# b-tudor/mpmcxx

Measured on AMD Instinct MI355X. Metric: energy-evals/sec (10k-atom LJ+Ewald+polar box); 1/2/4/8-GPU scaling, higher is better.
Workload: dtype f64

## Files before the change

mpmcxx_amd/csrc/context.h:

```cpp
#pragma once
#include <hip/hip_runtime.h>

#include <algorithm>
#include <atomic>
#include <chrono>
#include <mutex>
#include <cmath>
#include <cstdio>
#include <cstdlib>
#include <cstring>
#include <string>
#include <thread>
#include <vector>

#include "../../include/mpmc_energy.h"
#include "kernels.h"

using namespace mpmc;

namespace mpmc {
extern thread_local std::string g_create_error;
}

struct EvPair {
	hipEvent_t a, b;
	int cls;
};

#if defined(__SANITIZE_THREAD__)
extern "C" void AnnotateHappensBefore(const char *file, int line, const volatile void *tag);
extern "C" void AnnotateHappensAfter(const char *file, int line, const volatile void *tag);
inline char g_pinned_pool_tag;
#endif
template <class T>
inline hipError_t pinned_alloc(T **p, size_t bytes) {
	hipError_t e = hipHostMalloc((void **)p, bytes);
#if defined(__SANITIZE_THREAD__)
	AnnotateHappensAfter(__FILE__, __LINE__, &g_pinned_pool_tag);
#endif
	return e;
}
inline hipError_t pinned_free(void *p) {
#if defined(__SANITIZE_THREAD__)
	AnnotateHappensBefore(__FILE__, __LINE__, &g_pinned_pool_tag);
#endif
	return hipHostFree(p);
}

struct mpmc_ctx;
template <class T, bool kPinned = false>
struct DevBuf {
	T *p = nullptr;
	size_t cap = 0;
	DevBuf() = default;
	DevBuf(DevBuf &&o) noexcept : p(o.p), cap(o.cap) { o.p = nullptr, o.cap = 0; }
	DevBuf &operator=(DevBuf &&o) noexcept {
		std::swap(p, o.p), std::swap(cap, o.cap);
		return *this;
	}
	~DevBuf() { release(nullptr); }
	operator T *() const { return p; }
	void release(mpmc_ctx *c);
	int reserve(mpmc_ctx *c, size_t need, size_t grow_to = 0);
};
template <class T>
using PinnedBuf = DevBuf<T, true>;

struct mpmc_tuning {
	int stream_mode = -1;
	int pair_kernel = 0;
	int pair_waves = 0;
	int sort_grid = -1;
	int sort_nx = 0, sort_ny = 0;
	bool side_after_sweep = true;
	bool lazy_side_stream = true;
	bool poll_retire = true;
	bool poll_long = true;
	bool dense_symmetric = true;
	bool fast_geometry = true;
	int pair_split = -1;
	int pair_split_tail = -1;
	int sweep_order = 1;
	int sweep_lds_pad = 2048;
	bool use_panels = true;
	bool no_uniform = false;
	bool no_classes = false;
	bool single_launch = true;
	bool no_recip_tab = false;
	bool no_sort = false;
	bool no_order_carry = false;
	bool no_polar_delta = false;
	bool no_inline_move = false;
	int virtual_device = -1;
	int fail_next_wait = 0;
	bool trace_panel = false;
	bool dipoles_on_demand = true;
	long long tensor_budget_mb = 4096;
	long long direct_budget_mb = -1;
};

struct mpmc_kept {
	mpmc_tuning tune;
	bool prof = false;
	mpmc_timings tim{};
	long long n_poll_hits = 0, n_poll_timeouts = 0, n_stream_syncs = 0, n_poll_yields = 0;
	long long n_uploads_carried = 0, n_uploads_sorted = 0;
	bool tb_enabled = false, tb_mk = false;
	bool de_enabled = false;
	int de_flags = 0;
	bool pw_enabled = false;
	double pw_alpha = 0.0;
	bool palmo_enabled = false;
	bool on_demand = false;
};

struct mpmc_ctx {
	mpmc_kept kept;
	int device = 0;
	hipStream_t stream = nullptr;
	hipStream_t stream2 = nullptr;
	hipEvent_t ev_fork = nullptr, ev_join = nullptr;
	bool two_streams = true;
	int max_atoms = 0, max_pad = 0;
	int n = 0, n_pad = 0, n_tiles = 0, n_tile_pairs = 0, n_split = 1;
	int n_molecules = 0;
	double N_movable = 0;
	std::string err;

	std::vector<double> h_pos, h_q, h_alpha, h_eps, h_sigma, h_mass;
	std::vector<int32_t> h_mol, h_frozen, h_disp;

	std::vector<int32_t> perm, slot_of;
	int32_t *d_slot_of = nullptr, *d_perm = nullptr;
	bool atoms_dirty = true;

	DevBuf<char> d_atoms_blob;
	double4 *d_xyzq = nullptr;
	double2 *d_lj = nullptr;
	int2 *d_mf = nullptr;
	double *d_alpha = nullptr, *d_eps = nullptr, *d_inv_molmass = nullptr;

	DevBuf<int2> d_tile_pairs;
	DevBuf<double> d_block_part;
	DevBuf<int> d_block_cnt;
	DevBuf<int> d_cls;
	DevBuf<double> d_tile_bounds;
	DevBuf<double4> d_tp_shift;
	DevBuf<int4> d_panels;
	DevBuf<int> d_seg;
	DevBuf<double> d_gpart;
	DevBuf<long long> d_trace;
	int n_panel_entries = 0, seg_tiles = -1;
	bool panels_built = false;
	DevBuf<double2> d_erf_tab;
	DevBuf<int2> d_sweep_blocks;
	int n_sweep_blocks = 0, sweep_tiles = -1;
	DevBuf<int> d_generic_list;
	int n_generic = 0;
	std::vector<int> h_generic;
	int inflight_hint = 1;
	bool last_pair_was_sweep = false;
	FusedParams last_fp{};
	bool last_fp_valid = false;
	int debug_panel_replicas = 1;
	PinnedBuf<double4> h_xyzq;
	hipEvent_t ev_xyzq = nullptr;
	bool xyzq_in_flight = false;
	std::vector<double> h_pos_sorted;
	bool order_sorted = false;
	bool order_carried = false;
	bool atoms_dirty_order = false;
	int edits_since_sort = 0;
	double sort_origin_f[3] = {0, 0, 0};
	hipStream_t sync_stream = nullptr;
	std::vector<double> molmass_tmp;
	PinnedBuf<long long> static_cnt;
	PinnedBuf<char> h_kstage;
	hipEvent_t ev_kstage = nullptr;
	bool kstage_in_flight = false;
	int lvec_kmax = -1;
	PinnedBuf<char> h_stage;
	hipEvent_t ev_stage = nullptr;
	bool stage_in_flight = false;
	unsigned static_gen = 1, static_ride_gen = 0;

	bool static_dirty = true;
	double h_static[3] = {0, 0, 0};
	DevBuf<int> d_counter;
	bool scal_clean = false;
	int poll_budget_us = 1000;
	bool spin_on_post = false;
	bool last_was_single = false;
	double single_seq = 0;
	DevBuf<double> d_atom_part;
	DevBuf<double> d_scal;
	long long *d_cnt = nullptr;
	PinnedBuf<double> h_scal;
	long long *h_cnt = nullptr;
	DevBuf<int> d_flag;
	PinnedBuf<int> h_flag;

	int K = 0;
	DevBuf<double4> d_kvec, d_kw;
	DevBuf<double4> d_sf;
	DevBuf<int4> d_lvec;
	DevBuf<double4> d_sf_part;
	DevBuf<double> d_w_en;

	DevBuf<double> d_e_recip_part, d_part, d_e_static, d_mu[2], d_e_induced, d_rrms;
	DevBuf<double2> d_gs_blocks;
	DevBuf<double> d_gs_ul;
	int mu_cur = 0;
	DevBuf<double> d_dk_ring;
	enum { PEND_NONE = 0, PEND_OPEN = 1, PEND_DROPPED = 2 };
	int polar_pending = PEND_NONE;
	int pend_done = 0, pend_target = 0;
	DevBuf<double> d_arows;
	DevBuf<double> d_adense;
	DevBuf<double2> d_ab;
	int solver_used = MPMC_SOLVER_MATRIX_FREE;
	DevBuf<double> d_chol, d_chol_v, d_chol_info;
	PinnedBuf<double> h_chol_info;
	DevBuf<int> d_chol_list, d_chol_status;
	bool direct_ran = false;
	mpmc_direct_info direct{};

	Box box{};
	double box_in[20] = {0};
	bool box_in_has_recip = false;
	bool box_set = false, atoms_set = false, opts_set = false, k_dirty = true;
	mpmc_options opts{};
	double ewald_alpha = 0, polar_ewald_alpha = 0;

	bool pending = false;
	bool have_polar = false;
	int iters = 0, failed = 0;
	unsigned run_mask = 0;

	bool cache_valid = false;
	mpmc_result last_full{};
	mpmc_result trial_res{};
	int trial_last_kind = -1;
	bool trial_open = false, trial_evaluated = false, trial_was_full = false, trial_enqueued = false, trial_noop = false;
	mpmc_result trial_keep{};
	int trial_first = 0, trial_count = 0;
	std::vector<double> trial_new, trial_old;
	int *d_mv_slot = nullptr, *d_mv_orig = nullptr;
	double4 *d_mv_new = nullptr;
	DevBuf<int> d_moved_idx;
	DevBuf<double4> d_sf_trial;
	DevBuf<double> d_e_real, d_e_real_trial, d_dk_part;
	bool e_real_valid = false;
	bool trial_polar_delta = false;
	std::vector<int> store_dirty_tiles, trial_tiles;
	int touch_n = -1, touch[8] = {0};
	DevBuf<unsigned char> d_mv_blob;
	PinnedBuf<unsigned char> h_mv_blob;
	DevBuf<double> d_delta_out;
	PinnedBuf<double> h_delta_out;
	MvInline mv_inline{};
	bool trial_inline = false;
	double trial_seq = 0;
	long long *d_delta_cnt = nullptr, *h_delta_cnt = nullptr;

	bool tb_have = false;
	bool tb_dirty = false;
	std::vector<double> h_tb_au;
	DevBuf<double2> d_tb_au;
	DevBuf<double> d_tb_part;

	bool de_have = false;
	bool de_dirty = false;
	std::vector<double> h_de;
	std::vector<double> h_de_raw;
	bool de_lrc_valid = false;
	double de_lrc[2] = {0, 0}, de_lrc_volume = 0, de_lrc_cutoff = 0;
	int de_lrc_rd_lrc = 0;
	DevBuf<double4> d_de_co;
	DevBuf<double> d_de_t10;
	DevBuf<double> d_de_part;

	bool palmo_ran = false;
	double palmo_correction = 0.0;
	DevBuf<double> d_palmo_f, d_palmo_change;

	std::vector<EvPair> ev_free, ev_used;

	int64_t bytes_total = 0;
};

#define HIP_TRY(ctx, call)                                                                                        \
	do {                                                                                                          \
		hipError_t _e = (call);                                                                                   \
		if (_e != hipSuccess) {                                                                                   \
			(ctx)->err = std::string(#call) + ": " + hipGetErrorString(_e);                                       \
			return MPMC_ERR_HIP;                                                                                  \
		}                                                                                                         \
	} while (0)

template <class T, bool kPinned>
inline void DevBuf<T, kPinned>::release(mpmc_ctx *c) {
	if (p) (void)(kPinned ? pinned_free(p) : hipFree(p));
	if (p && c && !kPinned) c->bytes_total -= (int64_t)(cap * sizeof(T));
	p = nullptr, cap = 0;
}
template <class T, bool kPinned>
inline int DevBuf<T, kPinned>::reserve(mpmc_ctx *c, size_t need, size_t grow_to) {
	if (need <= cap) return MPMC_OK;
	release(c);
	const size_t count = std::max(need, grow_to), bytes = std::max<size_t>(count, 1) * sizeof(T);
	hipError_t e = kPinned ? pinned_alloc(&p, bytes) : hipMalloc((void **)&p, bytes);
	if (e != hipSuccess) p = nullptr;
	if (e == hipSuccess && !kPinned && (e = hipMemsetAsync(p, 0, bytes, c->stream)) == hipSuccess) e = hipStreamSynchronize(c->stream);
	if (e != hipSuccess) {
		release(nullptr);
		c->err = std::string(kPinned ? "pinned host" : "device") + " allocation of " + std::to_string(bytes) + " bytes: " + hipGetErrorString(e);
		return MPMC_ERR_HIP;
	}
	cap = count;
	if (!kPinned) c->bytes_total += (int64_t)(count * sizeof(T));
	return MPMC_OK;
}

namespace mpmc {

constexpr size_t kAtomRecordBytes = sizeof(double4) + sizeof(double2) + sizeof(int2) + 3 * sizeof(double) + 2 * sizeof(int32_t);
template <typename F>
inline void atom_block_layout(char *base, size_t P, F &&set) {
	double4 *xyzq = reinterpret_cast<double4 *>(base);
	double2 *lj = reinterpret_cast<double2 *>(xyzq + P);
	int2 *mf = reinterpret_cast<int2 *>(lj + P);
	double *al = reinterpret_cast<double *>(mf + P), *ep = al + P, *imm = ep + P;
	int32_t *perm = reinterpret_cast<int32_t *>(imm + P), *slot = perm + P;
	set(xyzq, lj, mf, al, ep, imm, perm, slot);
}
inline int mirror_guard(mpmc_ctx *c) {
	if (c->xyzq_in_flight) {
		HIP_TRY(c, hipEventSynchronize(c->ev_xyzq));
		c->xyzq_in_flight = false;
	}
	return MPMC_OK;
}

inline int fail(mpmc_ctx *c, int code, const std::string &msg) {
	if (c) c->err = msg;
	else g_create_error = msg;
	return code;
}

template <class Pred>
inline bool poll_posted(mpmc_ctx *c, Pred seen, std::chrono::microseconds budget) {
	const auto t0 = std::chrono::steady_clock::now();
	for (int spins = 0;; ++spins) {
		if (seen()) {
			std::atomic_thread_fence(std::memory_order_acquire);
			c->kept.n_poll_hits++;
			return true;
		}
		if ((spins & 255) == 255) {
			const auto dt = std::chrono::steady_clock::now() - t0;
			if (dt > budget) {
				c->kept.n_poll_timeouts++;
				return false;
			}
			if (dt > std::chrono::microseconds(50)) {
				c->kept.n_poll_yields++;
				std::this_thread::yield();
			}
		}
	}
}

inline void prof_begin(mpmc_ctx *c, int cls, int &cur, hipStream_t st) {
	cur = -1;
	if (!c->kept.prof) return;
	EvPair e;
	if (!c->ev_free.empty()) {
		e = c->ev_free.back();
		c->ev_free.pop_back();
	} else {
		if (hipEventCreate(&e.a) != hipSuccess || hipEventCreate(&e.b) != hipSuccess) return;
	}
	e.cls = cls;
	(void)hipEventRecord(e.a, st);
	c->ev_used.push_back(e);
	cur = (int)c->ev_used.size() - 1;
}
inline void prof_end(mpmc_ctx *c, int cur, hipStream_t st) {
	if (cur >= 0 && cur < (int)c->ev_used.size()) (void)hipEventRecord(c->ev_used[cur].b, st);
}
inline void prof_harvest(mpmc_ctx *c) {
	for (auto &e : c->ev_used) {
		float ms = 0;
		if (hipEventElapsedTime(&ms, e.a, e.b) == hipSuccess) {
			c->kept.tim.ms[e.cls] += ms;
			c->kept.tim.launches[e.cls] += 1;
		}
		c->ev_free.push_back(e);
	}
	c->ev_used.clear();
}
struct ProfScope {
	mpmc_ctx *c;
	int cur;
	hipStream_t st;
	ProfScope(mpmc_ctx *c_, int cls, hipStream_t st_ = nullptr) : c(c_), st(st_ ? st_ : c_->stream) { prof_begin(c, cls, cur, st); }
	~ProfScope() { prof_end(c, cur, st); }
};
inline hipStream_t fork_side(mpmc_ctx *c) {
	if (!c->two_streams) return c->stream;
	if (!c->stream2 && hipStreamCreateWithFlags(&c->stream2, hipStreamNonBlocking) != hipSuccess) {
		c->stream2 = nullptr;
		c->two_streams = false;
		return c->stream;
	}
	(void)hipEventRecord(c->ev_fork, c->stream);
	(void)hipStreamWaitEvent(c->stream2, c->ev_fork, 0);
	return c->stream2;
}
inline void join_side(mpmc_ctx *c) {
	if (!c->two_streams || !c->stream2) return;
	(void)hipEventRecord(c->ev_join, c->stream2);
	(void)hipStreamWaitEvent(c->stream, c->ev_join, 0);
}


enum : unsigned {
	RUN_PAIR = 1, RUN_PAIR_ES = 2, RUN_RECIP = 4, RUN_ATOMTERMS = 8, RUN_FIELD = 16, RUN_SOLVE = 32, RUN_WOLF = 64,
	RUN_STORE = 128,
	RUN_THREE_BODY = 256,
	RUN_DISP = 512
};
constexpr double kThreeBodyScale = 3.0 * (0.0032539449 / (3.166811429 * 0.000001));
int three_body_ready(mpmc_ctx *c);
int disp_ready(mpmc_ctx *c);
DispParams disp_params(const mpmc_ctx *c);
int prepare(mpmc_ctx *c, bool defer_static = false);
int enqueue(mpmc_ctx *c, unsigned mask, bool on_demand = false);
int wait_and_fill(mpmc_ctx *c, mpmc_result *out);
unsigned full_mask(const mpmc_ctx *c);
inline bool polar_moments_apply(const mpmc_ctx *c) {
	const mpmc_options &o = c->opts;
	return o.polarization && !o.rd_only && o.polar_iterative && o.polar_max_iter >= 1 && o.polar_max_iter <= kMomentsMaxIter && o.polar_gamma == 1.0 && o.polar_precision == 0.0 && !o.polar_rrms &&
	       !o.polar_gs;
}
inline int moments_half(int n) { return (n + 1) / 2; }
inline int reserve_dk_ring(mpmc_ctx *c) { return c->d_dk_ring.reserve(c, (size_t)(moments_half(c->opts.polar_max_iter) + 1) * 3 * (size_t)c->max_pad); }
int finish_pending_dipoles(mpmc_ctx *c);
inline void drop_pending_dipoles(mpmc_ctx *c) {
	if (c->polar_pending == mpmc_ctx::PEND_OPEN) c->polar_pending = mpmc_ctx::PEND_DROPPED;
}
inline bool direct_solve(const mpmc_ctx *c) { return c->opts.polarization && !c->opts.rd_only && !c->opts.polar_iterative; }
inline bool wolf_field_on(const mpmc_ctx *c) { return c->kept.pw_enabled && c->opts.polarization && !c->opts.rd_only && !c->opts.polar_ewald; }
void ext_params(const mpmc_ctx *c, FusedParams &fp, bool wolf_on);
AtomsDev atoms_view(const mpmc_ctx *c);
RecipDev recip_view(const mpmc_ctx *c);
int upload_atoms(mpmc_ctx *c);

}
```

mpmcxx_amd/csrc/evaluate.cpp:

```cpp
#include "context.h"


using namespace mpmc;

static int build_k_tables(mpmc_ctx *c) {
	const int kmax = c->opts.ewald_kmax;
	const double alpha = c->ewald_alpha, ea = c->polar_ewald_alpha;
	auto each_lvec = [kmax](auto &&visit) {
		int l[3];
		for (l[0] = 0; l[0] <= kmax; l[0]++)
			for (l[1] = (!l[0] ? 0 : -kmax); l[1] <= kmax; l[1]++)
				for (l[2] = ((!l[0] && !l[1]) ? 1 : -kmax); l[2] <= kmax; l[2]++)
					if (l[0] * l[0] + l[1] * l[1] + l[2] * l[2] <= kmax * kmax) visit(l);
	};
	int K = 0, rc;
	each_lvec([&K](const int *) { K++; });
	if ((size_t)K > c->d_lvec.cap) c->lvec_kmax = -1;
	if ((rc = c->d_kvec.reserve(c, (size_t)K)) != MPMC_OK) return rc;
	if ((rc = c->d_kw.reserve(c, (size_t)K)) != MPMC_OK) return rc;
	if ((rc = c->d_lvec.reserve(c, (size_t)K)) != MPMC_OK) return rc;
	if ((rc = c->d_w_en.reserve(c, (size_t)K)) != MPMC_OK) return rc;
	if ((rc = c->d_sf.reserve(c, (size_t)K)) != MPMC_OK) return rc;
	if (K > 0) {
		if (c->kstage_in_flight) {
			HIP_TRY(c, hipEventSynchronize(c->ev_kstage));
			c->kstage_in_flight = false;
		}
		if ((rc = c->h_kstage.reserve(c, (size_t)K * (2 * sizeof(double4) + sizeof(double) + sizeof(int4)))) != MPMC_OK) return rc;
		if (!c->ev_kstage) HIP_TRY(c, hipEventCreateWithFlags(&c->ev_kstage, hipEventDisableTiming));
		double4 *kvec = reinterpret_cast<double4 *>(c->h_kstage.p), *kw = kvec + K;
		int4 *lvec = reinterpret_cast<int4 *>(kw + K);
		double *wen = reinterpret_cast<double *>(lvec + K);
		int n = 0;
		each_lvec([&](const int *l) {
			double k[3];
			for (int p = 0; p < 3; p++) {
				k[p] = 0;
				for (int q = 0; q < 3; q++) k[p] += 2.0 * kPi * c->box.r[3 * p + q] * l[q];
			}
			const double k2 = k[0] * k[0] + k[1] * k[1] + k[2] * k[2];
			kvec[n] = make_double4(k[0], k[1], k[2], k2);
			lvec[n] = make_int4(l[0], l[1], l[2], 0);
			wen[n] = std::exp(-k2 / (4.0 * alpha * alpha)) / k2;
			const double g = std::exp(-k2 / (4.0 * ea * ea));
			kw[n] = make_double4(k[0] / k2 * g, k[1] / k2 * g, k[2] / k2 * g, 0.0);
			n++;
		});
		HIP_TRY(c, hipMemcpyAsync(c->d_kvec, kvec, K * sizeof(double4), hipMemcpyHostToDevice, c->stream));
		HIP_TRY(c, hipMemcpyAsync(c->d_kw, kw, K * sizeof(double4), hipMemcpyHostToDevice, c->stream));
		HIP_TRY(c, hipMemcpyAsync(c->d_w_en, wen, K * sizeof(double), hipMemcpyHostToDevice, c->stream));
		if (c->lvec_kmax != kmax) {
			HIP_TRY(c, hipMemcpyAsync(c->d_lvec, lvec, K * sizeof(int4), hipMemcpyHostToDevice, c->stream));
			c->lvec_kmax = kmax;
		}
		HIP_TRY(c, hipEventRecord(c->ev_kstage, c->stream));
		c->kstage_in_flight = true;
	}
	c->K = K;
	return MPMC_OK;
}

constexpr int kDenseChunks = 16;
constexpr int kOneStreamMinInflight = 4;
constexpr int kCheckEvery = 4;
constexpr int kSingleLaunchTiles = 32;

static int ensure_polar_buffers(mpmc_ctx *c) {
	const size_t np = (size_t)c->max_pad;
	int rc;
	if ((rc = c->d_e_static.reserve(c, 3 * np)) != MPMC_OK) return rc;
	if ((rc = c->d_mu[0].reserve(c, 3 * np)) != MPMC_OK) return rc;
	if ((rc = c->d_mu[1].reserve(c, 3 * np)) != MPMC_OK) return rc;
	if ((rc = c->d_e_induced.reserve(c, 3 * np)) != MPMC_OK) return rc;
	if ((rc = c->d_rrms.reserve(c, np)) != MPMC_OK) return rc;
	if ((rc = c->d_e_recip_part.reserve(c, recip_slices_capacity(np))) != MPMC_OK) return rc;
	if ((rc = c->d_e_real.reserve(c, 3 * np)) != MPMC_OK) return rc;
	if ((rc = c->d_e_real_trial.reserve(c, 3 * np)) != MPMC_OK) return rc;
	if ((rc = c->d_gs_ul.reserve(c, 6 * np)) != MPMC_OK) return rc;
	if ((rc = c->d_palmo_f.reserve(c, 3 * np)) != MPMC_OK) return rc;
	if ((rc = c->d_palmo_change.reserve(c, 3 * np)) != MPMC_OK) return rc;
	if (polar_moments_apply(c) && (rc = reserve_dk_ring(c)) != MPMC_OK) return rc;
	const size_t need = (size_t)std::max(c->n_tiles, kDenseChunks) * c->n_pad * 3;
	return c->d_part.reserve(c, need);
}

static int resolve_solver(mpmc_ctx *c) {
	const size_t need = (size_t)c->n_tile_pairs * (kTile * kTile);
	int want = c->opts.solver;
	if (direct_solve(c)) {
		c->solver_used = MPMC_SOLVER_MATRIX_FREE;
		return MPMC_OK;
	}
	if (c->opts.polar_gs) want = MPMC_SOLVER_MATRIX_FREE;
	if (want == MPMC_SOLVER_AUTO) {
		const size_t budget_mb = (size_t)c->kept.tune.tensor_budget_mb;
		want = (need * sizeof(double2) <= budget_mb * (size_t)1048576) ? MPMC_SOLVER_COMPACT : MPMC_SOLVER_MATRIX_FREE;
		if (c->opts.polar_precision == 0.0 && c->opts.polar_max_iter <= 3) want = MPMC_SOLVER_MATRIX_FREE;
	}
	if (want == MPMC_SOLVER_DENSE) {
		const int rc = c->d_adense.reserve(c, (size_t)3 * c->n_pad * (size_t)3 * c->n_pad);
		if (rc != MPMC_OK) return rc;
	}
	if (want == MPMC_SOLVER_COMPACT) {
		const int rc = c->d_ab.reserve(c, need);
		if (rc != MPMC_OK) {
			if (c->opts.solver == MPMC_SOLVER_COMPACT) return rc;
			(void)hipGetLastError();
			want = MPMC_SOLVER_MATRIX_FREE;
		}
	}
	c->solver_used = want;
	return MPMC_OK;
}

int mpmc::prepare(mpmc_ctx *c, bool defer_static) {
	if (!c->box_set) return fail(c, MPMC_ERR_BOX, "energy: no box set (mpmc_set_box)");
	if (!c->atoms_set) return fail(c, MPMC_ERR_INVALID_DATUM, "energy: no atoms set (mpmc_set_atoms)");
	HIP_TRY(c, hipSetDevice(c->device));
	if (c->opts.feynman_hibbs && c->h_mass.empty())
		return fail(c, MPMC_ERR_INVALID_DATUM, "energy: feynman_hibbs needs atom masses (mpmc_set_atoms was called without them)");
	if (c->atoms_dirty) {
		int rc = upload_atoms(c);
		if (rc != MPMC_OK) return rc;
	}
	if (c->k_dirty) {
		c->ewald_alpha = (c->opts.ewald_alpha > 0) ? c->opts.ewald_alpha : 3.5 / c->box.cutoff;
		c->polar_ewald_alpha = (c->opts.polar_ewald_alpha > 0) ? c->opts.polar_ewald_alpha : 3.5 / c->box.cutoff;
		int rc = build_k_tables(c);
		if (rc != MPMC_OK) return rc;
		c->k_dirty = false;
	}
	if (c->static_dirty && !defer_static) {
		c->scal_clean = false;
		launch_atom_terms(c->stream, atoms_view(c), c->box, c->ewald_alpha, c->opts.rd_lrc,  1, c->d_atom_part, c->d_scal);
		HIP_TRY(c, hipGetLastError());
		double tmp[S_COUNT];
		HIP_TRY(c, hipMemcpyAsync(tmp, c->d_scal, sizeof(tmp), hipMemcpyDeviceToHost, c->stream));
		HIP_TRY(c, hipStreamSynchronize(c->stream));
		c->h_static[0] = tmp[S_LRC_PAIR];
		c->h_static[1] = tmp[S_LRC_SELF];
		c->h_static[2] = tmp[S_ES_SELF];
		c->static_dirty = false;
	}
	return MPMC_OK;
}

AtomsDev mpmc::atoms_view(const mpmc_ctx *c) {
	AtomsDev a;
	a.xyzq = c->d_xyzq;
	a.lj = c->d_lj;
	a.mf = c->d_mf;
	a.alpha = c->d_alpha;
	a.eps = c->d_eps;
	a.inv_molmass = c->d_inv_molmass;
	a.n = c->n;
	a.n_pad = c->n_pad;
	return a;
}
RecipDev mpmc::recip_view(const mpmc_ctx *c) {
	RecipDev r;
	r.kvec = c->d_kvec;
	r.w_en = c->d_w_en;
	r.kw = c->d_kw;
	r.lvec = c->kept.tune.no_recip_tab ? nullptr : c->d_lvec;
	r.sf = c->d_sf;
	r.K = c->K;
	return r;
}

static inline const double4 *shift_view(const mpmc_ctx *c) { return (c->kept.tune.no_uniform || c->kept.tune.no_classes) ? nullptr : c->d_tp_shift.p; }

void mpmc::ext_params(const mpmc_ctx *c, FusedParams &fp, bool wolf_on) {
	const mpmc_options &o = c->opts;
	fp.wolf = wolf_on ? 1 : 0;
	fp.fh_order = o.feynman_hibbs ? ((o.feynman_hibbs_order == 4) ? 4 : 2) : 0;
	fp.fh_c2 = fp.fh_c4 = 0.0;
	if (fp.fh_order) {
		const double hBar2 = 1.11211999e-68, hBar4 = 1.23681087e-136, kB = 1.3806503e-23, kB2 = 1.90619525e-46, amu = 1.66053873e-27;
		fp.fh_c2 = 1.0e20 * (hBar2 / (24.0 * kB * o.temperature)) / amu;
		fp.fh_c4 = 1.0e40 * (hBar4 / (1152.0 * kB2 * o.temperature * o.temperature)) / (amu * amu);
	}
	fp.wolf_erfa_over_r = std::erf(c->ewald_alpha * c->box.cutoff) / c->box.cutoff;
	fp.wolf_inv_r2 = 1.0 / (c->box.cutoff * c->box.cutoff);
}

static inline int sweep_split_mode(const mpmc_ctx *c) { return c->kept.tune.pair_split < 0 ? 2 : (c->kept.tune.pair_split != 0 ? 1 : 0); }
static inline int sweep_split_tail(const mpmc_ctx *c) {
	const int permille = c->kept.tune.pair_split_tail >= 0 ? c->kept.tune.pair_split_tail : kSweepSplitTailPermille;
	return (int)((long long)c->n_sweep_blocks * permille / 1000);
}

static int enqueue_direct_solve(mpmc_ctx *c, const AtomsDev &at) {
	hipStream_t st = c->stream;
	int n_pol = 0;
	for (int i = 0; i < c->n; i++) n_pol += (c->h_alpha[i] != 0.0) ? 1 : 0;
	const int np = chol_padded(n_pol);
	const size_t elems = (size_t)np * (size_t)np, bytes = elems * sizeof(double);
	int rc;
	if ((rc = c->d_chol_status.reserve(c, 4)) != MPMC_OK) return rc;
	if ((rc = c->d_chol_info.reserve(c, 4)) != MPMC_OK) return rc;
	if ((rc = c->h_chol_info.reserve(c, 4)) != MPMC_OK) return rc;
	{
		size_t free_b = 0, total_b = 0;
		HIP_TRY(c, hipMemGetInfo(&free_b, &total_b));
		size_t avail = free_b + c->d_chol.cap * sizeof(double);
		if (c->kept.tune.direct_budget_mb >= 0) avail = std::min(avail, (size_t)c->kept.tune.direct_budget_mb * (size_t)1048576);
		if (bytes > avail) {
			char buf[256];
			std::snprintf(buf, sizeof buf, "direct dipole solve: the factor of %d unknowns needs %.1f MB (%d x %d doubles), %.1f MB are available", 3 * n_pol,
			              (double)bytes / 1048576.0, np, np, (double)avail / 1048576.0);
			return fail(c, MPMC_ERR_MEMORY, buf);
		}
	}
	if (c->d_chol.reserve(c, elems) != MPMC_OK) {
		(void)hipGetLastError();
		return fail(c, MPMC_ERR_MEMORY, "direct dipole solve: cannot allocate the factor (" + std::to_string(bytes) + " bytes): " + c->err);
	}
	if ((rc = c->d_chol_v.reserve(c, (size_t)2 * np, (size_t)2 * np + 1)) != MPMC_OK) return rc;
	if ((rc = c->d_chol_list.reserve(c, (size_t)n_pol, (size_t)c->max_pad)) != MPMC_OK) return rc;
	c->mu_cur = 0;
	double *mu = c->d_mu[0], *v0 = c->d_chol_v, *v1 = c->d_chol_v + np;
	HIP_TRY(c, hipMemsetAsync(c->d_chol_status, 0, sizeof(int), st));
	HIP_TRY(c, hipMemsetAsync(mu, 0, 3 * (size_t)at.n_pad * sizeof(double), st));
	if (n_pol > 0) {
		{
			ProfScope p(c, MPMC_K_TENSOR);
			launch_chol_build(st, at, c->box, c->opts.polar_damp, c->d_chol_list, n_pol, np, c->d_chol);
		}
		{
			ProfScope p(c, MPMC_K_DIPOLE_ITER);
			launch_chol_rhs(st, c->d_chol_list, n_pol, np, c->d_e_static, v0, c->d_chol_status);
			launch_chol_factor(st, c->d_chol, np, c->d_chol_status);
			launch_chol_solve(st, c->d_chol, np, v0, v1, c->d_chol_status);
			launch_chol_scatter(st, c->d_chol_list, n_pol, v0, mu, c->d_chol_status);
		}
	}
	{
		ProfScope p(c, MPMC_K_REDUCE);
		launch_dipole_iter_hybrid(st, at, c->box, mu, c->d_tile_pairs, c->d_cls, shift_view(c),
		                          c->n_tile_pairs, nullptr, c->d_part, c->opts.polar_damp, nullptr);
		launch_dipole_update(st, at, c->d_e_static, c->d_part, c->n_tiles, mu, c->d_mu[1], c->d_e_induced, 0, c->d_rrms, 0.0, nullptr, nullptr, 1);
		launch_chol_finish(st, at, mu, c->d_e_static, c->d_e_induced, c->d_chol_status, c->d_chol_info);
	}
	HIP_TRY(c, hipGetLastError());
	HIP_TRY(c, hipMemcpyAsync(c->h_chol_info, c->d_chol_info, 3 * sizeof(double), hipMemcpyDeviceToHost, st));
	c->direct.n_unknowns = 3 * (int64_t)n_pol;
	c->direct.factor_bytes = (int64_t)(c->d_chol.cap * sizeof(double));
	c->direct_ran = true;
	return MPMC_OK;
}


struct JacobiPlan {
	bool dense, dense_sym, compact;
	int iter_slots;
};
static JacobiPlan jacobi_plan(const mpmc_ctx *c) {
	JacobiPlan jp;
	jp.dense = (c->solver_used == MPMC_SOLVER_DENSE) && !c->opts.polar_gs;
	jp.dense_sym = jp.dense && c->kept.tune.dense_symmetric;
	jp.compact = c->solver_used == MPMC_SOLVER_COMPACT;
	jp.iter_slots = (jp.dense && !jp.dense_sym) ? kDenseChunks : c->n_tiles;
	return jp;
}
static void enqueue_jacobi_iteration(mpmc_ctx *c, const AtomsDev &at, const JacobiPlan &jp, int it, int want_rrms, double allowed, int *ctl, int *host_flag,
                                     double *dk) {
	hipStream_t st = c->stream;
	const mpmc_options &o = c->opts;
	const int *converged = ctl ? ctl + 1 : nullptr;
	if (jp.dense) {
		ProfScope p(c, MPMC_K_DIPOLE_ITER);
		if (jp.dense_sym) launch_dense_symv(st, c->d_adense, c->n_pad, c->d_mu[c->mu_cur], c->d_tile_pairs, c->n_tile_pairs, c->d_part);
		else launch_dense_matvec(st, c->d_adense, c->n_pad, c->d_mu[c->mu_cur], kDenseChunks, c->d_part);
	} else if (jp.compact) {
		ProfScope p(c, MPMC_K_DIPOLE_ITER);
		if (c->panels_built)
			launch_dipole_iter_panel(st, at, c->box, c->d_mu[c->mu_cur], c->d_tile_pairs, c->d_tp_shift, c->d_panels,
			                         c->n_panel_entries, c->d_ab, c->d_part, c->d_gpart, converged, c->d_trace);
		else
			launch_dipole_iter_hybrid(st, at, c->box, c->d_mu[c->mu_cur], c->d_tile_pairs, c->d_cls,
			                          shift_view(c), c->n_tile_pairs, c->d_ab, c->d_part, o.polar_damp,
			                          converged);
	} else {
		ProfScope p(c, MPMC_K_DIPOLE_ITER);
		launch_dipole_iter_hybrid(st, at, c->box, c->d_mu[c->mu_cur], c->d_tile_pairs, c->d_cls,
		                          shift_view(c), c->n_tile_pairs, nullptr, c->d_part, o.polar_damp,
		                          converged);
	}
	{
		ProfScope p(c, MPMC_K_REDUCE);
		if (jp.compact && c->panels_built && !jp.dense)
			launch_dipole_update_panel(st, at, c->d_e_static, c->d_part, c->d_gpart, c->d_seg, c->d_mu[c->mu_cur], c->d_mu[1 - c->mu_cur],
			                           c->d_e_induced, want_rrms, c->d_rrms, allowed, ctl, host_flag, it, dk);
		else
			launch_dipole_update(st, at, c->d_e_static, c->d_part, jp.iter_slots, c->d_mu[c->mu_cur], c->d_mu[1 - c->mu_cur], c->d_e_induced,
			                     want_rrms, c->d_rrms, allowed, ctl, host_flag, it, dk);
	}
	c->mu_cur = 1 - c->mu_cur;
}

int mpmc::finish_pending_dipoles(mpmc_ctx *c) {
	if (c->polar_pending == mpmc_ctx::PEND_NONE) return MPMC_OK;
	if (c->polar_pending == mpmc_ctx::PEND_DROPPED)
		return fail(c, MPMC_ERR_ARG, "the dipoles of the last evaluation were left to be computed on demand, and its positions, cell, options or buffers "
		                             "have been overwritten since: evaluate again (or mpmc_set_dipoles_on_demand(ctx, 0))");
	HIP_TRY(c, hipSetDevice(c->device));
	const AtomsDev at = atoms_view(c);
	const JacobiPlan jp = jacobi_plan(c);
	for (int it = c->pend_done + 1; it <= c->pend_target; it++) enqueue_jacobi_iteration(c, at, jp, it, 0, 0.0, nullptr, nullptr, nullptr);
	HIP_TRY(c, hipGetLastError());
	HIP_TRY(c, hipStreamSynchronize(c->stream));
	c->polar_pending = mpmc_ctx::PEND_NONE;
	c->pend_done = c->pend_target;
	if (!c->pending) prof_harvest(c);
	return MPMC_OK;
}

int mpmc::enqueue(mpmc_ctx *c, unsigned mask, bool on_demand) {
	if (c->pending) return fail(c, MPMC_ERR_ARG, "an evaluation of this context is still in flight (mpmc_energy_wait first)");
	drop_pending_dipoles(c);
	int rc = prepare(c, true);
	if (rc != MPMC_OK) return rc;
	if ((mask & RUN_THREE_BODY) && (rc = three_body_ready(c)) != MPMC_OK) return rc;
	if ((mask & RUN_DISP) && (rc = disp_ready(c)) != MPMC_OK) return rc;
	const bool static_ride = c->static_dirty;
	c->static_ride_gen = 0;
	const AtomsDev at = atoms_view(c);
	const RecipDev rcp = recip_view(c);
	const mpmc_options &o = c->opts;
	hipStream_t st = c->stream;
	c->run_mask = mask;
	c->have_polar = false;
	c->direct_ran = false;
	c->palmo_ran = false;
	c->iters = 0;
	c->failed = 0;

	c->last_was_single = false;
	c->spin_on_post = false;
	if (c->kept.tune.single_launch && mask == (RUN_PAIR | RUN_ATOMTERMS) && !o.feynman_hibbs && c->n_tiles <= kSingleLaunchTiles && !c->kept.prof && !static_ride) {
		FusedParams fp{};
		fp.rd_lrc = o.rd_lrc;
		c->single_seq += 1.0;
		launch_pair_lj_single(st, at, c->box, fp, c->d_tile_pairs, c->n_tile_pairs, c->d_block_part, c->d_block_cnt, c->d_counter, c->h_scal,
		                      c->single_seq);
		HIP_TRY(c, hipGetLastError());
		c->last_was_single = true;
		c->pending = true;
		return MPMC_OK;
	}
	if (!c->scal_clean) HIP_TRY(c, hipMemsetAsync(c->d_scal, 0, (S_COUNT + C_COUNT) * sizeof(double), st));
	c->scal_clean = false;
	if (static_ride) {
		launch_atom_terms(st, at, c->box, c->ewald_alpha, o.rd_lrc,  1, c->d_atom_part, c->d_scal);
		HIP_TRY(c, hipGetLastError());
		c->static_ride_gen = c->static_gen;
	}

	if (mask & (RUN_FIELD | RUN_SOLVE | RUN_STORE)) {
		if ((rc = ensure_polar_buffers(c)) != MPMC_OK) return rc;
		if ((rc = resolve_solver(c)) != MPMC_OK) return rc;
	}
	const bool compact = (mask & RUN_SOLVE) && c->solver_used == MPMC_SOLVER_COMPACT;

	const bool need_sf = (mask & RUN_RECIP) || ((mask & RUN_FIELD) && o.polar_ewald);
	const bool need_intra = (mask & RUN_PAIR) && (mask & RUN_PAIR_ES) && !(o.wolf && (mask & RUN_WOLF)) && (c->n_molecules != c->n);
	const bool side_work = need_sf || need_intra;
	c->two_streams = (c->kept.tune.stream_mode == 1) ||
	                 (c->kept.tune.stream_mode < 0 && c->n_tile_pairs > kOneStreamMaxPairs &&
	                  !((mask & RUN_SOLVE) && c->inflight_hint >= kOneStreamMinInflight));
	const bool side_fork = c->two_streams && (need_sf || need_intra);
	bool panel_side = false;
	int side_rc = MPMC_OK;
	auto enqueue_side_work = [&](hipStream_t s2) {
		if (need_intra) {
			ProfScope p(c, MPMC_K_PAIR, s2);
			launch_intra_terms(s2, at, c->d_slot_of, c->ewald_alpha, c->d_scal);
		}
		{
			ProfScope p(c, MPMC_K_RECIP, s2);
			if (need_sf) {
				const size_t need_part = (size_t)c->n_tiles * (size_t)c->K;
				if (rcp.lvec && o.ewald_kmax <= kRecipTabMaxK && (side_rc = c->d_sf_part.reserve(c, need_part)) != MPMC_OK) return;
				launch_recip_sf(s2, at, c->box, rcp, o.ewald_kmax, c->d_sf_part);
			}
			if (mask & RUN_RECIP) launch_recip_energy(s2, rcp, c->box, c->d_scal);
		}
		if ((mask & RUN_FIELD) && o.polar_ewald) {
			ProfScope p(c, MPMC_K_FIELD, s2);
			launch_field_recip(s2, at, c->box, rcp, o.ewald_kmax, c->d_e_recip_part);
		}
	};
	const bool side_deferred = side_work && side_fork && (mask & (RUN_PAIR | RUN_FIELD | RUN_STORE)) != 0 && c->kept.tune.side_after_sweep;
	if (side_work && !side_deferred) {
		enqueue_side_work(side_fork ? fork_side(c) : st);
		if (side_rc != MPMC_OK) return side_rc;
	}

	if (mask & (RUN_PAIR | RUN_FIELD | RUN_STORE)) {
		{
			ProfScope pc(c, MPMC_K_CLASSES);
			if (c->kept.tune.no_classes) HIP_TRY(c, hipMemsetAsync(c->d_cls, 0, (size_t)c->n_tile_pairs * sizeof(int), st));
			else launch_tile_classes(st, at, c->box, c->d_tile_pairs, c->n_tile_pairs, (o.polarization && !o.rd_only) ? o.polar_damp : 0.0,
			                         c->d_tile_bounds, c->d_cls, c->kept.tune.no_uniform ? nullptr : c->d_tp_shift, c->sort_origin_f, kTholeFarX);
		}
		FusedParams fp;
		fp.ewald_alpha = c->ewald_alpha;
		fp.polar_ewald_alpha = c->polar_ewald_alpha;
		fp.polar_damp = o.polar_damp;
		fp.rd_lrc = o.rd_lrc;
		fp.do_es = ((mask & RUN_PAIR_ES) || (mask & RUN_FIELD)) ? 1 : 0;
		fp.do_field = ((mask & RUN_FIELD) && !wolf_field_on(c)) ? (o.polar_ewald ? 1 : 2) : 0;
		fp.do_thole = compact ? 1 : 0;
		ext_params(c, fp, (o.wolf && (mask & RUN_WOLF)) != 0);
		fp.thole_far_x = kTholeFarX;
		fp.pair_waves = c->kept.tune.pair_waves ? c->kept.tune.pair_waves : (c->n_tile_pairs <= kPairSplitMax ? 4 : 1);
		fp.store_only = ((mask & RUN_STORE) && !(mask & (RUN_PAIR | RUN_FIELD))) ? 1 : 0;
		fp.touch_n = fp.store_only ? c->touch_n : -1;
		for (int k = 0; k < 8; k++) fp.touch[k] = c->touch[k];
		if (!fp.store_only && compact) c->store_dirty_tiles.clear();
		c->panels_built = false;
		if (compact && c->kept.tune.use_panels && !c->kept.tune.no_classes && !c->kept.tune.no_uniform && c->n_tiles >= 3) {
			if (c->seg_tiles != c->n_tiles) {
				std::vector<int> seg((size_t)c->n_tiles + 1, 0);
				for (int J = 0; J < c->n_tiles; J++) seg[J + 1] = seg[J] + panel_segment_entries(J);
				if ((rc = c->d_seg.reserve(c, seg.size())) != MPMC_OK) return rc;
				HIP_TRY(c, hipMemcpyAsync(c->d_seg, seg.data(), seg.size() * sizeof(int), hipMemcpyHostToDevice, st));
				HIP_TRY(c, hipStreamSynchronize(st));
				c->n_panel_entries = seg[c->n_tiles];
				c->seg_tiles = c->n_tiles;
			}
			const size_t need = (size_t)c->n_panel_entries;
			if ((rc = c->d_panels.reserve(c, need)) != MPMC_OK) return rc;
			if ((rc = c->d_gpart.reserve(c, need * kTile * 3)) != MPMC_OK) return rc;
			if (c->kept.tune.trace_panel && (rc = c->d_trace.reserve(c, need * 4)) != MPMC_OK) return rc;
			panel_side = c->two_streams;
			if (!panel_side) {
				ProfScope pc(c, MPMC_K_CLASSES, st);
				launch_build_panels(st, c->d_cls, c->n_tiles, c->d_seg, c->d_panels);
			}
			c->panels_built = true;
		}
		hipStream_t s_side = (side_deferred || panel_side) ? fork_side(c) : st;
		c->last_fp = fp;
		c->last_fp_valid = !fp.store_only;
		ProfScope p(c, MPMC_K_PAIR);
		const bool sweep = c->kept.tune.pair_kernel != 1 && c->d_sweep_blocks && (c->kept.tune.pair_kernel == 2 || c->n_tile_pairs > kSweepMinPairs) &&
		                   pair_sweep_covers(c->box, fp, c->ewald_alpha);
		c->last_pair_was_sweep = sweep;
		if (sweep) {
			launch_pair_sweep(st, at, c->box, fp, c->n_molecules != c->n, c->d_sweep_blocks, c->n_sweep_blocks, c->d_cls,
			                  shift_view(c), c->d_erf_tab, c->d_block_part, c->d_block_cnt, c->d_part,
			                  compact ? c->d_ab : nullptr, sweep_split_mode(c), sweep_split_tail(c), c->kept.tune.fast_geometry,
			                  (side_deferred || panel_side) ? c->kept.tune.sweep_lds_pad : 0);
			if (c->n_generic > 0)
				launch_pair_fused(st, at, c->box, fp, c->d_tile_pairs, c->d_cls, c->n_generic, c->d_block_part, c->d_block_cnt, c->d_part,
				                  compact ? c->d_ab : nullptr, c->d_generic_list);
		} else if (!(fp.store_only && !compact))
			launch_pair_fused(st, at, c->box, fp, c->d_tile_pairs, c->d_cls, c->n_tile_pairs, c->d_block_part, c->d_block_cnt, c->d_part,
			                  compact ? c->d_ab : nullptr);
		if (side_deferred) {
			enqueue_side_work(s_side);
			if (side_rc != MPMC_OK) return side_rc;
		}
		if (panel_side) {
			ProfScope pc(c, MPMC_K_CLASSES, s_side);
			launch_build_panels(s_side, c->d_cls, c->n_tiles, c->d_seg, c->d_panels);
		}
	}
	if ((side_work && side_fork) || panel_side) join_side(c);
	const bool reduce_in_tail = (mask & RUN_PAIR) && (mask & RUN_SOLVE);
	if ((mask & RUN_PAIR) && !reduce_in_tail) {
		ProfScope p(c, MPMC_K_REDUCE);
		launch_reduce_pairs(st, c->d_block_part, c->d_block_cnt, c->n_tile_pairs, c->d_scal, c->d_cnt);
	}

	if (mask & RUN_FIELD) {
		ProfScope p(c, MPMC_K_FIELD);
		c->mu_cur = 0;
		if (wolf_field_on(c))
			launch_wolf_field(st, at, c->box, wolf_field_params(c->kept.pw_alpha, c->box.cutoff), c->d_tile_pairs, c->d_cls, c->n_tile_pairs, c->d_part);
		launch_field_finalize(st, at, c->box, o.polar_ewald, c->d_e_recip_part, c->d_part, c->n_tiles, o.polar_gamma, c->d_e_static,
		                      c->d_mu[0], c->d_e_real, polar_moments_apply(c) ? c->d_dk_ring.p : nullptr);
		c->e_real_valid = (mask == full_mask(c));
	}

	if ((mask & RUN_SOLVE) && direct_solve(c)) {
		if ((rc = enqueue_direct_solve(c, at)) != MPMC_OK) return rc;
		{
			ProfScope p(c, MPMC_K_REDUCE);
			if (reduce_in_tail)
				launch_polar_energy_and_pairs(st, at, c->d_mu[c->mu_cur], c->d_e_static, nullptr, c->d_block_part, c->d_block_cnt, c->n_tile_pairs, c->d_scal,
				                              c->d_cnt);
			else launch_polar_energy(st, at, c->d_mu[c->mu_cur], c->d_e_static, nullptr, c->d_scal);
		}
		c->have_polar = true;
		c->polar_pending = mpmc_ctx::PEND_NONE;
	} else if (mask & RUN_SOLVE) {
		const bool by_precision = (o.polar_precision != 0.0);
		const int want_rrms = (o.polar_rrms || o.polar_precision > 0) ? 1 : 0;
		const double allowed = by_precision ? o.polar_precision * o.polar_precision * kDebye2SKA * kDebye2SKA : 0.0;
		const JacobiPlan jp = jacobi_plan(c);
		const bool dense = jp.dense, dense_sym = jp.dense_sym;
		const bool moments = polar_moments_apply(c);
		const int half = moments_half(o.polar_max_iter);
		const bool lazy = moments && on_demand && c->kept.tune.dipoles_on_demand && half < o.polar_max_iter;
		const int last_it = lazy ? half : o.polar_max_iter;
		const size_t dk_stride = 3 * (size_t)at.n_pad;
		if (dense) {
			ProfScope p(c, MPMC_K_TENSOR);
			launch_dense_build(st, at, c->box, o.polar_damp, c->d_adense, dense_sym);
		}
		int *ctl = (by_precision && !o.polar_gs) ? c->d_flag + 1 : nullptr;
		const int check_every = dense ? 1 : kCheckEvery;
		const int mu_start = c->mu_cur;
		int done_at = 0;
		int *host_flag = ctl ? c->h_flag + 2 : nullptr;
		if (ctl) {
			HIP_TRY(c, hipMemsetAsync(ctl, 0, 3 * sizeof(int), st));
			c->h_flag[2] = c->h_flag[3] = 0;
		}
		if (o.polar_gs) {
			if ((rc = c->d_gs_blocks.reserve(c, gs_block_store_elements(c->n_tiles))) != MPMC_OK) return rc;
			ProfScope p(c, MPMC_K_TENSOR);
			launch_gs_blocks(st, at, c->box, o.polar_damp, c->d_gs_blocks);
		}
		int it = 0;
		bool keep = true;
		while (keep) {
			it++;
			if (it >= kMaxIterationCount && by_precision) {
				launch_dipole_reset(st, at, c->d_e_static, c->d_mu[c->mu_cur]);
				c->failed = 1;
				break;
			}
			if (by_precision && o.polar_gs) HIP_TRY(c, hipMemsetAsync(c->d_flag, 0, sizeof(int), st));
			if (o.polar_gs) {
				double *mu = c->d_mu[c->mu_cur], *mu_old = c->d_mu[1 - c->mu_cur];
				if (want_rrms) HIP_TRY(c, hipMemcpyAsync(mu_old, mu, 3 * (size_t)at.n_pad * sizeof(double), hipMemcpyDeviceToDevice, st));
				{
					ProfScope p(c, MPMC_K_DIPOLE_ITER);
					launch_gs_sweep(st, at, c->box, o.polar_damp, c->d_e_static, mu, c->d_e_induced, c->d_part, c->d_tile_pairs, c->d_cls,
					                shift_view(c), c->n_tile_pairs, c->d_gs_ul, c->d_gs_ul + 3 * (size_t)c->max_pad, c->d_gs_blocks);
				}
				if (want_rrms) {
					ProfScope p(c, MPMC_K_REDUCE);
					launch_gs_finish(st, at, mu_old, mu, want_rrms, c->d_rrms, allowed, c->d_flag);
				}
				if (by_precision) {
					HIP_TRY(c, hipMemcpyAsync(c->h_flag, c->d_flag, sizeof(int), hipMemcpyDeviceToHost, st));
					HIP_TRY(c, hipStreamSynchronize(st));
					keep = (*c->h_flag != 0);
				} else {
					keep = (it != o.polar_max_iter);
				}
				continue;
			}
			enqueue_jacobi_iteration(c, at, jp, it, want_rrms, allowed, ctl, host_flag, (moments && it <= half) ? c->d_dk_ring + (size_t)it * dk_stride : nullptr);
			if (by_precision) {
				if (it % check_every == 0 || it + 1 >= kMaxIterationCount) {
					HIP_TRY(c, hipGetLastError());
					volatile const int *hf = host_flag;
					const bool seen = poll_posted(c, [&] { return hf[0] >= it || hf[1] != 0; }, std::chrono::microseconds(50000));
					if (seen) {
						done_at = hf[1];
					} else {
						c->kept.n_stream_syncs++;
						HIP_TRY(c, hipMemcpyAsync(c->h_flag, ctl + 1, sizeof(int), hipMemcpyDeviceToHost, st));
						HIP_TRY(c, hipStreamSynchronize(st));
						done_at = *c->h_flag;
					}
					keep = (done_at == 0);
				}
			} else {
				keep = (it != last_it);
			}
		}
		if (done_at > 0) {
			it = done_at;
			c->mu_cur = (mu_start + done_at) & 1;
		}
		c->iters = lazy ? o.polar_max_iter : it;
		c->polar_pending = lazy ? mpmc_ctx::PEND_OPEN : mpmc_ctx::PEND_NONE;
		c->pend_done = it, c->pend_target = o.polar_max_iter;
		if (moments) {
			ProfScope p(c, MPMC_K_REDUCE);
			if (reduce_in_tail)
				launch_polar_moments_and_pairs(st, at, c->d_dk_ring, c->d_e_static, o.polar_max_iter, c->d_block_part, c->d_block_cnt, c->n_tile_pairs, c->d_scal,
				                               c->d_cnt);
			else launch_polar_moments(st, at, c->d_dk_ring, c->d_e_static, o.polar_max_iter, c->d_scal);
		} else {
			ProfScope p(c, MPMC_K_REDUCE);
			if (reduce_in_tail)
				launch_polar_energy_and_pairs(st, at, c->d_mu[c->mu_cur], c->d_e_static, want_rrms ? c->d_rrms : nullptr, c->d_block_part, c->d_block_cnt,
				                              c->n_tile_pairs, c->d_scal, c->d_cnt);
			else launch_polar_energy(st, at, c->d_mu[c->mu_cur], c->d_e_static, want_rrms ? c->d_rrms : nullptr, c->d_scal);
		}
		if (c->kept.palmo_enabled && o.polar_gs && !c->failed) {
			double *mu = c->d_mu[c->mu_cur];
			{
				ProfScope p(c, MPMC_K_DIPOLE_ITER);
				launch_dipole_iter_hybrid(st, at, c->box, mu, c->d_tile_pairs, c->d_cls, shift_view(c),
				                          c->n_tile_pairs, nullptr, c->d_part, o.polar_damp, nullptr);
			}
			ProfScope p(c, MPMC_K_REDUCE);
			launch_dipole_update(st, at, c->d_e_static, c->d_part, c->n_tiles, mu, c->d_mu[1 - c->mu_cur], c->d_palmo_f, 0, c->d_rrms, 0.0, nullptr, nullptr, 1);
			launch_palmo_reduce(st, at, mu, c->d_palmo_f, c->d_e_induced, c->d_palmo_change, c->d_scal);
			c->palmo_ran = true;
		}
		c->have_polar = true;
	}
	if (mask & RUN_THREE_BODY) {
		ProfScope p(c, MPMC_K_THREE_BODY);
		launch_three_body(st, at, c->d_tb_au, c->box, kThreeBodyScale, c->d_tb_part, c->d_scal + S_THREE_BODY);
	}
	if (mask & RUN_DISP) {
		ProfScope p(c, MPMC_K_PAIR);
		launch_disp_expansion(st, at, c->d_de_co, c->d_de_t10, c->d_tile_pairs, c->n_tile_pairs, c->box, disp_params(c), c->de_lrc[0], c->de_lrc[1],
		                      c->d_de_part, c->d_scal + S_DISP);
	}
	HIP_TRY(c, hipGetLastError());
	c->single_seq += 1.0;
	launch_post_results(st, c->d_scal, c->h_scal, c->single_seq);
	HIP_TRY(c, hipGetLastError());
	c->scal_clean = true;
	c->spin_on_post = c->ev_used.empty() && (c->kept.tune.poll_long || c->n_tile_pairs <= kOneStreamMaxPairs);
	c->poll_budget_us = (c->n_tile_pairs <= kOneStreamMaxPairs) ? 1000 : 4000;
	c->pending = true;
	return MPMC_OK;
}


extern "C" int mpmc_debug_time_panel(mpmc_ctx *c, int reps, double *ms_per_launch) {
	if (!c || !ms_per_launch || reps <= 0) return MPMC_ERR_ARG;
	if (c->pending) return fail(c, MPMC_ERR_ARG, "mpmc_debug_time_panel: an evaluation is in flight");
	if (!c->have_polar || !c->panels_built || c->solver_used != MPMC_SOLVER_COMPACT)
		return fail(c, MPMC_ERR_ARG, "mpmc_debug_time_panel: the last evaluation did not run the panel kernel");
	HIP_TRY(c, hipSetDevice(c->device));
	{
		const int rc_f = finish_pending_dipoles(c);
		if (rc_f != MPMC_OK) return rc_f;
	}
	const AtomsDev at = atoms_view(c);
	hipEvent_t e0, e1;
	HIP_TRY(c, hipEventCreate(&e0));
	HIP_TRY(c, hipEventCreate(&e1));
	for (int r = 0; r < 3; r++)
		launch_dipole_iter_panel(c->stream, at, c->box, c->d_mu[c->mu_cur], c->d_tile_pairs, c->d_tp_shift, c->d_panels, c->n_panel_entries,
		                         c->d_ab, c->d_part, c->d_gpart);
	HIP_TRY(c, hipEventRecord(e0, c->stream));
	const int replicas = c->debug_panel_replicas;
	for (int r = 0; r < reps; r++)
		launch_dipole_iter_panel(c->stream, at, c->box, c->d_mu[c->mu_cur], c->d_tile_pairs, c->d_tp_shift, c->d_panels, c->n_panel_entries,
		                         c->d_ab, c->d_part, c->d_gpart, nullptr, nullptr, replicas);
	HIP_TRY(c, hipEventRecord(e1, c->stream));
	HIP_TRY(c, hipGetLastError());
	HIP_TRY(c, hipEventSynchronize(e1));
	float ms = 0;
	HIP_TRY(c, hipEventElapsedTime(&ms, e0, e1));
	(void)hipEventDestroy(e0);
	(void)hipEventDestroy(e1);
	*ms_per_launch = (double)ms / reps;
	return MPMC_OK;
}

extern "C" int mpmc_debug_time_pair(mpmc_ctx *c, int reps, double *ms_per_launch) {
	if (!c || !ms_per_launch || reps <= 0) return MPMC_ERR_ARG;
	if (c->pending) return fail(c, MPMC_ERR_ARG, "mpmc_debug_time_pair: an evaluation is in flight");
	if (!c->cache_valid || !c->last_fp_valid) return fail(c, MPMC_ERR_ARG, "mpmc_debug_time_pair: no complete evaluation has run");
	HIP_TRY(c, hipSetDevice(c->device));
	{
		const int rc_f = finish_pending_dipoles(c);
		if (rc_f != MPMC_OK) return rc_f;
	}
	const AtomsDev at = atoms_view(c);
	const FusedParams &fp = c->last_fp;
	const bool compact = c->solver_used == MPMC_SOLVER_COMPACT && fp.do_thole;
	bool timed = false;
	auto launch = [&] {
		if (c->last_pair_was_sweep) {
			launch_pair_sweep(c->stream, at, c->box, fp, c->n_molecules != c->n, c->d_sweep_blocks, c->n_sweep_blocks, c->d_cls,
			                  shift_view(c), c->d_erf_tab, c->d_block_part, c->d_block_cnt, c->d_part,
			                  compact ? c->d_ab : nullptr, sweep_split_mode(c), sweep_split_tail(c), c->kept.tune.fast_geometry,
			                  c->two_streams ? c->kept.tune.sweep_lds_pad : 0, timed ? c->debug_panel_replicas : 1);
			if (c->n_generic > 0)
				launch_pair_fused(c->stream, at, c->box, fp, c->d_tile_pairs, c->d_cls, c->n_generic, c->d_block_part, c->d_block_cnt, c->d_part,
				                  compact ? c->d_ab : nullptr, c->d_generic_list);
		} else {
			launch_pair_fused(c->stream, at, c->box, fp, c->d_tile_pairs, c->d_cls, c->n_tile_pairs, c->d_block_part, c->d_block_cnt, c->d_part,
			                  compact ? c->d_ab : nullptr);
		}
	};
	hipEvent_t e0, e1;
	HIP_TRY(c, hipEventCreate(&e0));
	HIP_TRY(c, hipEventCreate(&e1));
	for (int r = 0; r < 2; r++) launch();
	timed = true;
	HIP_TRY(c, hipEventRecord(e0, c->stream));
	for (int r = 0; r < reps; r++) launch();
	HIP_TRY(c, hipEventRecord(e1, c->stream));
	HIP_TRY(c, hipGetLastError());
	HIP_TRY(c, hipEventSynchronize(e1));
	float ms = 0;
	HIP_TRY(c, hipEventElapsedTime(&ms, e0, e1));
	(void)hipEventDestroy(e0);
	(void)hipEventDestroy(e1);
	*ms_per_launch = (double)ms / reps;
	return MPMC_OK;
}

int mpmc::wait_and_fill(mpmc_ctx *c, mpmc_result *out) {
	if (!c->pending) return fail(c, MPMC_ERR_ARG, "mpmc_energy_wait: nothing enqueued");
	auto abandon = [c](hipError_t e, const char *what) {
		(void)hipStreamSynchronize(c->stream);
		if (c->two_streams && c->stream2) (void)hipStreamSynchronize(c->stream2);
		c->sync_stream = nullptr;
		c->pending = false;
		c->scal_clean = false;
		c->static_ride_gen = 0;
		drop_pending_dipoles(c);
		return fail(c, MPMC_ERR_HIP, std::string(what) + ": " + hipGetErrorString(e));
	};
	hipError_t werr = c->kept.tune.fail_next_wait ? hipErrorUnknown : hipSetDevice(c->device);
	c->kept.tune.fail_next_wait = 0;
	if (werr != hipSuccess) return abandon(werr, "mpmc_energy_wait: hipSetDevice");
	bool seen = false;
	if (c->last_was_single || c->spin_on_post) {
		volatile const double *flag = c->h_scal + S_COUNT + C_COUNT;
		const double want = c->single_seq;
		seen = poll_posted(c, [&] { return *flag == want; }, std::chrono::microseconds(c->last_was_single ? 200 : c->poll_budget_us));
	}
	if (!seen) {
		c->kept.n_stream_syncs++;
		werr = hipStreamSynchronize(c->sync_stream ? c->sync_stream : c->stream);
		if (werr != hipSuccess) return abandon(werr, "mpmc_energy_wait: hipStreamSynchronize");
	} else if (c->kept.tune.poll_retire && c->n_tile_pairs > kOneStreamMaxPairs) {
		(void)hipStreamQuery(c->stream);
		if (c->two_streams && c->stream2) (void)hipStreamQuery(c->stream2);
	}
	c->sync_stream = nullptr;
	c->pending = false;
	prof_harvest(c);
	if (c->direct_ran) {
		c->direct.status = (int64_t)c->h_chol_info[0];
		c->direct.residual = (c->h_chol_info[2] > 0.0) ? c->h_chol_info[1] / c->h_chol_info[2] : 0.0;
		if (c->direct.status != 0) {
			c->failed = 1;
			c->err = "direct dipole solve: the matrix is not positive definite (pivot " + std::to_string((long long)c->direct.status) + " of " +
			         std::to_string((long long)c->direct.n_unknowns) + " is not positive): dipoles and polarization energy set to 0";
		}
	}
	if (!out) return MPMC_OK;
	std::memset(out, 0, sizeof(*out));
	const double *s = c->h_scal;
	if (c->static_ride_gen) {
		if (c->static_ride_gen == c->static_gen) {
			c->h_static[0] = s[S_LRC_PAIR];
			c->h_static[1] = s[S_LRC_SELF];
			c->h_static[2] = s[S_ES_SELF];
			c->static_dirty = false;
		}
		c->static_ride_gen = 0;
	}
	if (c->run_mask & RUN_DISP) {
		out->lj_pairs = s[S_DISP];
		out->lrc_pair = s[S_DISP_LRC_PAIR];
		out->lrc_self = s[S_DISP_LRC_SELF];
	} else {
		const bool lrc = (c->run_mask & RUN_ATOMTERMS) && c->opts.rd_lrc;
		out->lj_pairs = s[S_LJ];
		out->lrc_pair = lrc ? c->h_static[0] : 0.0;
		out->lrc_self = lrc ? c->h_static[1] : 0.0;
	}
	out->rd_energy = (out->lj_pairs + out->lrc_pair) + out->lrc_self;
	out->es_real = s[S_ES_REAL] - s[S_ES_INTRA];
	out->es_recip = s[S_ES_RECIP];
	out->es_self = (c->run_mask & RUN_RECIP) ? c->h_static[2] : 0.0;
	out->coulombic_energy = (out->es_real + out->es_recip) + out->es_self;
	out->polarization_energy = s[S_POLAR];
	if (c->run_mask & RUN_SOLVE) c->palmo_correction = c->palmo_ran ? s[S_PALMO] : 0.0;
	out->dipole_rrms = s[S_RRMS];
	out->three_body_energy = (c->run_mask & RUN_THREE_BODY) ? s[S_THREE_BODY] : 0.0;
	out->energy = out->rd_energy + out->coulombic_energy + out->polarization_energy + out->vdw_energy + out->three_body_energy;
	out->N = c->N_movable;
	out->NU = out->N * out->energy;
	out->n_pairs = (int64_t)c->n * (c->n - 1) / 2;
	out->n_lj_in_cutoff = c->h_cnt[C_LJ_IN];
	out->n_es_in_cutoff = c->h_cnt[C_ES_IN];
	out->n_intra = c->static_cnt[0];
	out->n_rd_excluded = c->static_cnt[1];
	out->n_es_excluded = c->static_cnt[2];
	out->n_frozen = c->static_cnt[3];
	out->polar_iterations = c->iters;
	out->iterator_failed = c->failed;
	if (c->run_mask == full_mask(c)) {
		c->last_full = *out;
		c->cache_valid = true;
	}
	return MPMC_OK;
}

unsigned mpmc::full_mask(const mpmc_ctx *c) {
	unsigned m = RUN_PAIR | RUN_ATOMTERMS;
	if (!c->opts.rd_only) {
		m |= RUN_PAIR_ES;
		m |= c->opts.wolf ? RUN_WOLF : RUN_RECIP;
		if (c->opts.polarization) m |= RUN_FIELD | RUN_SOLVE;
	}
	if (c->kept.tb_enabled) m |= RUN_THREE_BODY;
	if (c->kept.de_enabled) m |= RUN_DISP;
	return m;
}

extern "C" int mpmc_energy_async(mpmc_ctx *c) {
	if (!c) return MPMC_ERR_ARG;
	return enqueue(c, full_mask(c), c->kept.on_demand);
}
extern "C" int mpmc_set_dipoles_on_demand(mpmc_ctx *c, int enabled) {
	if (!c) return MPMC_ERR_ARG;
	c->kept.on_demand = enabled != 0;
	return MPMC_OK;
}
extern "C" int mpmc_hint_in_flight(mpmc_ctx *c, int n) {
	if (!c || n < 1) return MPMC_ERR_ARG;
	c->inflight_hint = n;
	return MPMC_OK;
}
extern "C" int mpmc_energy_wait(mpmc_ctx *c, mpmc_result *out) {
	if (!c) return MPMC_ERR_ARG;
	return wait_and_fill(c, out);
}
extern "C" int mpmc_energy(mpmc_ctx *c, mpmc_result *out) {
	if (!c || !out) return MPMC_ERR_ARG;
	c->inflight_hint = 1;
	int rc = enqueue(c, full_mask(c), c->kept.on_demand);
	if (rc != MPMC_OK) return rc;
	return wait_and_fill(c, out);
}


static int run_piece(mpmc_ctx *c, unsigned mask, mpmc_result *r) {
	if (!c) return MPMC_ERR_ARG;
	int rc = enqueue(c, mask);
	if (rc != MPMC_OK) return rc;
	return wait_and_fill(c, r);
}
extern "C" int mpmc_lj(mpmc_ctx *c, double *out) {
	mpmc_result r;
	int rc = run_piece(c, RUN_PAIR | RUN_ATOMTERMS, &r);
	if (rc == MPMC_OK && out) *out = r.rd_energy;
	return rc;
}
extern "C" int mpmc_coulombic_real(mpmc_ctx *c, double *out) {
	mpmc_result r;
	int rc = run_piece(c, RUN_PAIR | RUN_PAIR_ES, &r);
	if (rc == MPMC_OK && out) *out = r.es_real;
	return rc;
}
extern "C" int mpmc_coulombic_reciprocal(mpmc_ctx *c, double *out) {
	mpmc_result r;
	int rc = run_piece(c, RUN_RECIP, &r);
	if (rc == MPMC_OK && out) *out = r.es_recip;
	return rc;
}
extern "C" int mpmc_coulombic_self(mpmc_ctx *c, double *out) {
	mpmc_result r;
	int rc = run_piece(c, RUN_RECIP, &r);
	if (rc == MPMC_OK && out) *out = r.es_self;
	return rc;
}
extern "C" int mpmc_coulombic(mpmc_ctx *c, double *out) {
	if (!c) return MPMC_ERR_ARG;
	mpmc_result r;
	int rc = run_piece(c, RUN_PAIR | RUN_PAIR_ES | (c->opts.wolf ? RUN_WOLF : RUN_RECIP), &r);
	if (rc == MPMC_OK && out) *out = r.coulombic_energy;
	return rc;
}
extern "C" int mpmc_polar(mpmc_ctx *c, double *out) {
	if (!c) return MPMC_ERR_ARG;
	if (!c->opts.polarization) return fail(c, MPMC_ERR_INVALID_SETTING, "mpmc_polar: polarization is off");
	mpmc_result r;
	int rc = run_piece(c, RUN_FIELD | RUN_SOLVE, &r);
	if (rc == MPMC_OK && out) *out = r.polarization_energy;
	return rc;
}
extern "C" int mpmc_axilrod_teller(mpmc_ctx *c, double *out) {
	if (!c) return MPMC_ERR_ARG;
	if (!c->kept.tb_enabled) return fail(c, MPMC_ERR_INVALID_SETTING, "mpmc_axilrod_teller: the term is off (mpmc_set_axilrod_teller)");
	mpmc_result r;
	int rc = run_piece(c, RUN_THREE_BODY, &r);
	if (rc == MPMC_OK && out) *out = r.three_body_energy;
	return rc;
}
extern "C" int mpmc_disp_expansion(mpmc_ctx *c, double *out) {
	if (!c) return MPMC_ERR_ARG;
	if (!c->kept.de_enabled) return fail(c, MPMC_ERR_INVALID_SETTING, "mpmc_disp_expansion: the term is off (mpmc_set_disp_expansion)");
	mpmc_result r;
	int rc = run_piece(c, RUN_DISP, &r);
	if (rc == MPMC_OK && out) *out = r.rd_energy;
	return rc;
}
static int fetch_atoms3(mpmc_ctx *c, const double *d_src, double *out) {
	std::vector<double> tmp(3 * (size_t)c->n);
	HIP_TRY(c, hipMemcpyAsync(tmp.data(), d_src, tmp.size() * sizeof(double), hipMemcpyDeviceToHost, c->stream));
	HIP_TRY(c, hipStreamSynchronize(c->stream));
	for (int k = 0; k < c->n; k++) {
		const int i = c->perm[k];
		out[3 * (size_t)i] = tmp[3 * (size_t)k];
		out[3 * (size_t)i + 1] = tmp[3 * (size_t)k + 1];
		out[3 * (size_t)i + 2] = tmp[3 * (size_t)k + 2];
	}
	return MPMC_OK;
}

extern "C" int mpmc_thole_field(mpmc_ctx *c, double *ef_static) {
	if (!c) return MPMC_ERR_ARG;
	mpmc_result r;
	int rc = run_piece(c, RUN_FIELD, &r);
	if (rc != MPMC_OK) return rc;
	if (ef_static) return fetch_atoms3(c, c->d_e_static, ef_static);
	return MPMC_OK;
}

extern "C" int mpmc_thole_amatrix(mpmc_ctx *c, int row0, int nrows, double *a) {
	if (!c || !a || row0 < 0 || nrows <= 0) return MPMC_ERR_ARG;
	int rc = prepare(c);
	if (rc != MPMC_OK) return rc;
	if (row0 % 3 || nrows % 3 || row0 + nrows > 3 * c->n) return fail(c, MPMC_ERR_ARG, "mpmc_thole_amatrix: rows must cover whole atoms (multiples of 3) inside 3N");
	const size_t need = (size_t)nrows * 3 * c->n;
	if ((rc = c->d_arows.reserve(c, need)) != MPMC_OK) return rc;
	{
		ProfScope p(c, MPMC_K_TENSOR);
		launch_amatrix_rows(c->stream, atoms_view(c), c->d_slot_of, c->box, c->opts.polar_damp, row0, nrows, c->d_arows);
	}
	HIP_TRY(c, hipGetLastError());
	HIP_TRY(c, hipMemcpyAsync(a, c->d_arows, need * sizeof(double), hipMemcpyDeviceToHost, c->stream));
	HIP_TRY(c, hipStreamSynchronize(c->stream));
	prof_harvest(c);
	return MPMC_OK;
}

extern "C" int mpmc_polar_direct_info(mpmc_ctx *c, mpmc_direct_info *out) {
	if (!c || !out) return MPMC_ERR_ARG;
	if (c->pending) return fail(c, MPMC_ERR_ARG, "mpmc_polar_direct_info: an evaluation is in flight");
	*out = c->direct;
	return MPMC_OK;
}

extern "C" int mpmc_polar_palmo_info(mpmc_ctx *c, double *energy_correction, double *ef_induced_change) {
	if (!c) return MPMC_ERR_ARG;
	if (c->pending) return fail(c, MPMC_ERR_ARG, "mpmc_polar_palmo_info: an evaluation is in flight");
	if (energy_correction) *energy_correction = c->palmo_correction;
	if (ef_induced_change) {
		if (c->palmo_ran && c->d_palmo_change) {
			HIP_TRY(c, hipSetDevice(c->device));
			return fetch_atoms3(c, c->d_palmo_change, ef_induced_change);
		}
		std::fill(ef_induced_change, ef_induced_change + 3 * (size_t)c->n, 0.0);
	}
	return MPMC_OK;
}

extern "C" int mpmc_get_dipoles(mpmc_ctx *c, double *mu, double *ef_static, double *ef_induced) {
	if (!c) return MPMC_ERR_ARG;
	if (!c->d_e_static) return fail(c, MPMC_ERR_ARG, "mpmc_get_dipoles: no polarization evaluation has run");
	HIP_TRY(c, hipSetDevice(c->device));
	int rc = finish_pending_dipoles(c);
	if (rc != MPMC_OK) return rc;
	HIP_TRY(c, hipStreamSynchronize(c->stream));
	if (mu && rc == MPMC_OK) rc = fetch_atoms3(c, c->d_mu[c->mu_cur], mu);
	if (ef_static && rc == MPMC_OK) rc = fetch_atoms3(c, c->d_e_static, ef_static);
	if (ef_induced && rc == MPMC_OK) rc = fetch_atoms3(c, c->d_e_induced, ef_induced);
	return rc;
}

extern "C" int mpmc_update_com(mpmc_ctx *c, double *com, double *wrapped_com, double *wrapped_pos, int *n_molecules) {
	if (!c) return MPMC_ERR_ARG;
	if (!c->atoms_set || !c->box_set) return fail(c, MPMC_ERR_ARG, "mpmc_update_com: atoms and box must be set");
	if (c->h_mass.empty()) return fail(c, MPMC_ERR_ARG, "mpmc_update_com: mpmc_set_atoms was called without masses");
	if (n_molecules) *n_molecules = c->n_molecules;
	int m = 0;
	for (int i0 = 0; i0 < c->n;) {
		int i1 = i0;
		while (i1 + 1 < c->n && c->h_mol[i1 + 1] == c->h_mol[i0]) i1++;
		double cm[3] = {0, 0, 0}, mass = 0;
		for (int i = i0; i <= i1; i++) {
			mass += c->h_mass[i];
			for (int p = 0; p < 3; p++) cm[p] += c->h_mass[i] * c->h_pos[3 * i + p];
		}
		for (int p = 0; p < 3; p++) cm[p] /= mass;
		const bool mol_frozen = c->h_frozen[i1] != 0;
		double w[3] = {0, 0, 0};
		if (!mol_frozen) {
			double d[3];
			for (int p = 0; p < 3; p++) {
				d[p] = 0;
				for (int q = 0; q < 3; q++) d[p] += c->box.r[3 * q + p] * cm[q];
				d[p] = std::rint(d[p]);
			}
			for (int p = 0; p < 3; p++) {
				w[p] = 0;
				for (int q = 0; q < 3; q++) w[p] += c->box.b[3 * q + p] * d[q];
			}
		}
		if (com)
			for (int p = 0; p < 3; p++) com[3 * m + p] = cm[p];
		if (wrapped_com)
			for (int p = 0; p < 3; p++) wrapped_com[3 * m + p] = w[p];
		if (wrapped_pos)
			for (int i = i0; i <= i1; i++)
				for (int p = 0; p < 3; p++) wrapped_pos[3 * i + p] = mol_frozen ? c->h_pos[3 * i + p] : c->h_pos[3 * i + p] - w[p];
		m++;
		i0 = i1 + 1;
	}
	return MPMC_OK;
}
```

mpmcxx_amd/csrc/kernels.h:

```cpp
#pragma once

#include <hip/hip_runtime.h>
#include <stdint.h>

#include <algorithm>

#include "pair_math.h"

namespace mpmc {

constexpr int kTile = 64;
constexpr int kKSplit = 8;
constexpr int kKSplitMax = 64, kKSplitWaves = 1024;
inline int recip_ksplit(int n_pad) {
	const int nt = n_pad / kTile;
	int ks = kKSplit;
	while (ks < kKSplitMax && nt * ks < kKSplitWaves) ks *= 2;
	return ks;
}
inline size_t recip_slices_capacity(size_t max_pad) { return std::max((size_t)kKSplit * 3 * max_pad, (size_t)2 * kKSplitWaves * kTile * 3); }

struct AtomsDev {
	const double4 *xyzq;
	const double2 *lj;
	const int2 *mf;
	const double *alpha;
	const double *eps;
	const double *inv_molmass;
	int n, n_pad;
};

enum : int {
	S_LJ = 0, S_LRC_PAIR, S_ES_REAL, S_ES_INTRA,
	S_ES_RECIP, S_ES_SELF, S_LRC_SELF,
	S_POLAR, S_RRMS,
	S_THREE_BODY,
	S_DISP, S_DISP_LRC_PAIR, S_DISP_LRC_SELF,
	S_PALMO,
	S_COUNT = 16
};
enum : int { C_LJ_IN = 0, C_ES_IN, C_INTRA, C_RDX, C_ESX, C_FROZEN, C_COUNT = 8 };
enum : int {
	CLS_BEYOND_CUTOFF = 1,
	CLS_THOLE_FAR = 2,
	CLS_UNIFORM_X = 4,
	CLS_UNIFORM_Y = 8,
	CLS_UNIFORM_Z = 16
};
constexpr double kTholeFarX = 30.0;

struct RecipDev {
	const double4 *kvec;
	const double *w_en;
	const double4 *kw;
	const int4 *lvec;
	double4 *sf;
	int K;
};
constexpr int kRecipTabMaxK = 15;
void launch_recip_sf(hipStream_t st, const AtomsDev &at, const Box &bx, const RecipDev &rc, int kmax, double4 *sf_part);
constexpr size_t kAtomTermScratch = 64 * 34;
void launch_atom_terms(hipStream_t st, const AtomsDev &at, const Box &bx, double ewald_alpha, int rd_lrc, int do_es, double *part_scratch,
                       double *scal);

void launch_field_recip(hipStream_t st, const AtomsDev &at, const Box &bx, const RecipDev &rc, int kmax, double *e_recip );
void launch_field_finalize(hipStream_t st, const AtomsDev &at, const Box &bx, int polar_ewald, const double *e_recip,
                           const double *part, int n_split, double gamma, double *e_static, double *mu,
                           double *e_real_out = nullptr ,
                           double *mu_copy = nullptr );

void launch_dipole_update(hipStream_t st, const AtomsDev &at, const double *e_static, const double *part, int n_split,
                          const double *mu_old, double *mu_new, double *e_induced, int want_rrms, double *rrms_atom,
                          double allowed_sqerr, int *ctl, int *host_flag , int it,
                          double *dk = nullptr );
void launch_dipole_reset(hipStream_t st, const AtomsDev &at, const double *e_static, double *mu);
void launch_post_results(hipStream_t st, double *scal, double *out_host, double seq);
void launch_polar_energy(hipStream_t st, const AtomsDev &at, const double *mu, const double *e_static, const double *rrms_atom,
                         double *scal);
constexpr int kMomentsMaxIter = 64;
constexpr int kMomentsMaxHalf = (kMomentsMaxIter + 1) / 2;
void launch_polar_moments(hipStream_t st, const AtomsDev &at, const double *dk, const double *e_static, int n_iter, double *scal);
void launch_polar_moments_and_pairs(hipStream_t st, const AtomsDev &at, const double *dk, const double *e_static, int n_iter,
                                    const double *block_part, const int *block_cnt, int nb, double *scal, long long *cnt);

void launch_amatrix_rows(hipStream_t st, const AtomsDev &at, const int *slot_of, const Box &bx, double polar_damp, int row0, int nrows,
                         double *a );

struct FusedParams {
	double ewald_alpha, polar_ewald_alpha, polar_damp;
	int rd_lrc;
	int do_es;
	int do_field;
	int do_thole;
	int wolf;
	int fh_order;
	double fh_c2, fh_c4;
	double wolf_erfa_over_r, wolf_inv_r2;
	double thole_far_x;
	int store_only;
	int touch_n;
	int touch[8];
	int pair_waves;
};
constexpr int kOneStreamMaxPairs = 1536;
constexpr int kPairSplitMax = 8192;
void launch_pair_fused(hipStream_t st, const AtomsDev &at, const Box &bx, const FusedParams &fp, const int2 *tile_pairs,
                       const int *cls, int n_tile_pairs, double *block_part , int *block_cnt , double *fpart, double2 *ab,
                       const int *tp_list = nullptr);
struct PairSweepParams {
	double alpha_scaled_half, polar_damp_half, thole_far_x;
	int store;
	int nt;
	int have_shift;
	int split;
	int n_main;
	int fast;
};
constexpr int kSweepMinPairs = 2048;
constexpr int kSweepSplitTailPermille = 250;
constexpr int kErfTableDouble2 = 3 * 512;
void erfc_table_device_layout(double2 *out );
int pair_sweep_blocks(int n_tiles, int2 *out);
bool pair_sweep_covers(const Box &bx, const FusedParams &fp, double ewald_alpha);
void launch_pair_sweep(hipStream_t st, const AtomsDev &at, const Box &bx, const FusedParams &fp, bool intra ,
                       const int2 *blocks, int n_blocks, const int *cls, const double4 *tp_shift ,
                       const double2 *erf_tab, double *block_part, int *block_cnt, double *fpart, double2 *ab, int split_mode = 0 ,
                       int n_split_tail = 0 , bool fast_geometry = false, int lds_pad_bytes = 0 ,
                       int replicas = 1 );
void launch_reduce_pairs(hipStream_t st, const double *block_part, const int *block_cnt, int nb, double *scal, long long *cnt);
void launch_polar_energy_and_pairs(hipStream_t st, const AtomsDev &at, const double *mu, const double *e_static, const double *rrms_atom,
                                   const double *block_part, const int *block_cnt, int nb, double *scal, long long *cnt);
void launch_pair_lj_single(hipStream_t st, const AtomsDev &at, const Box &bx, const FusedParams &fp, const int2 *tile_pairs, int n_tile_pairs,
                           double *block_part, int *block_cnt, int *counter, double *out_host, double seq);
void launch_recip_energy(hipStream_t st, const RecipDev &rc, const Box &bx, double *scal);
void launch_static_counts(hipStream_t st, const AtomsDev &at, const int2 *tile_pairs, int n_tile_pairs, int *block_cnt ,
                          long long *cnt4);
void launch_intra_terms(hipStream_t st, const AtomsDev &at, const int *slot_of, double ewald_alpha, double *scal);
void launch_tile_classes(hipStream_t st, const AtomsDev &at, const Box &bx, const int2 *tile_pairs, int n_tile_pairs, double polar_damp,
                         double *tile_bounds , int *cls, double4 *tp_shift ,
                         const double origin_f[3] ,
                         double thole_far_x = kTholeFarX );
void launch_dipole_iter_hybrid(hipStream_t st, const AtomsDev &at, const Box &bx, const double *mu, const int2 *tile_pairs,
                               const int *cls, const double4 *tp_shift , int n_tile_pairs,
                               const double2 *ab ,
                               double *part, double polar_damp, const int *converged = nullptr);
int panel_segment_entries(int J);
void launch_build_panels(hipStream_t st, const int *cls, int n_tiles, const int *seg , int4 *panels);
void launch_dipole_iter_panel(hipStream_t st, const AtomsDev &at, const Box &bx, const double *mu, const int2 *tile_pairs,
                              const double4 *tp_shift, const int4 *panels, int n_entries, const double2 *ab, double *part, double *gpart,
                              const int *converged = nullptr, long long *trace = nullptr ,
                              int replicas = 1 );
void launch_dipole_update_panel(hipStream_t st, const AtomsDev &at, const double *e_static, const double *part, const double *gpart, const int *seg,
                                const double *mu_old, double *mu_new, double *e_induced, int want_rrms, double *rrms_atom, double allowed_sqerr,
                                int *ctl, int *host_flag, int it, double *dk = nullptr );
void launch_rot_selftest(hipStream_t st, int *out);

void launch_dense_build(hipStream_t st, const AtomsDev &at, const Box &bx, double polar_damp, double *a, bool upper_only = false);
void launch_dense_symv(hipStream_t st, const double *a, int n_pad, const double *x, const int2 *tile_pairs, int n_tile_pairs, double *part);
void launch_dense_matvec(hipStream_t st, const double *a, int n_pad, const double *x, int n_chunks, double *part);

constexpr int kCholNB = 64;
constexpr int kCholPanel = 192;
inline int chol_padded(int n_pol) { return (3 * n_pol + kCholPanel - 1) / kCholPanel * kCholPanel; }
void launch_chol_build(hipStream_t st, const AtomsDev &at, const Box &bx, double polar_damp, int *pol_list, int n_pol, int np, double *m);
void launch_chol_rhs(hipStream_t st, const int *pol_list, int n_pol, int np, const double *e_static, double *b, int *status);
void launch_chol_factor(hipStream_t st, double *m, int np, int *status);
void launch_chol_solve(hipStream_t st, const double *m, int np, double *v0, double *v1, const int *status);
void launch_chol_scatter(hipStream_t st, const int *pol_list, int n_pol, const double *x, double *mu , const int *status);
void launch_chol_finish(hipStream_t st, const AtomsDev &at, const double *mu, const double *e_static, double *e_induced, const int *status,
                        double *info);

size_t gs_block_store_elements(int n_tiles);
void launch_gs_blocks(hipStream_t st, const AtomsDev &at, const Box &bx, double polar_damp, double2 *blocks);
void launch_gs_sweep(hipStream_t st, const AtomsDev &at, const Box &bx, double polar_damp, const double *e_static, double *mu, double *e_induced,
                     double *part, const int2 *tile_pairs, const int *cls, const double4 *tp_shift, int n_tile_pairs, double *U, double *L,
                     const double2 *blocks);
void launch_gs_finish(hipStream_t st, const AtomsDev &at, const double *mu_old, const double *mu_new, int want_rrms, double *rrms_atom,
                      double allowed_sqerr, int *not_done_flag);

constexpr int kMvInline = 8;
struct MvInline {
	double nw[kMvInline][4];
	int slot[kMvInline], orig[kMvInline];
};
void launch_commit_positions_inline(hipStream_t st, double4 *xyzq, const MvInline &inl, int m);
void launch_delta(hipStream_t st, const AtomsDev &at, const int *slot_of, const Box &bx, const RecipDev &rc,
                  const FusedParams &fp , int do_es,
                  const int *mv_slot, const int *orig_of_mv, const double4 *mv_new, int m, int *moved_idx, double4 *sf_trial,
                  double *block_part, int *block_cnt, double *out4, long long *dcnt2,
                  double *host_out , double seq,
                  const MvInline *inl = nullptr );
void launch_commit_positions(hipStream_t st, double4 *xyzq, const int *mv_slot, const double4 *mv_new, int m);
void launch_delta_field(hipStream_t st, const AtomsDev &at, const Box &bx, double polar_ewald_alpha, int polar_ewald, const int *mv_slot,
                        const double4 *mv_new, int m, int *moved_idx, const double *e_real, double *e_real_trial, double *dk_part);
void launch_swap_positions(hipStream_t st, double4 *xyzq, const int *mv_slot, double4 *mv_new, int m);

constexpr int kThreeBodyBlocks = 8192;
long long three_body_tile_triples(int n_tiles);
int three_body_grid(long long work_items);
void launch_three_body(hipStream_t st, const AtomsDev &at, const double2 *au, const Box &bx, double scale, double *part, double *out);
void launch_three_body_delta(hipStream_t st, const AtomsDev &at, const double2 *au, const Box &bx, double scale, const int *mv_slot, const double4 *mv_new,
                             int m, int *moved_idx, double *part, double *out);

constexpr int kDispBlocks = 16384;
struct DispParams {
	int damp, schmidt;
};
int disp_grid(long long work_items);
void launch_disp_expansion(hipStream_t st, const AtomsDev &at, const double4 *co, const double *t10, const int2 *tile_pairs, int n_tile_pairs,
                           const Box &bx, const DispParams &dp, double lrc_pair, double lrc_self, double *part, double *out);
void launch_disp_expansion_delta(hipStream_t st, const AtomsDev &at, const double4 *co, const double *t10, const Box &bx, const DispParams &dp,
                                 const int *mv_slot, const double4 *mv_new, int m, int *moved_idx, double *part, double *out);

struct WolfFieldParams {
	double a;
	double c_gauss;
	double cutoff_term;
};
WolfFieldParams wolf_field_params(double polar_wolf_alpha, double cutoff);
void launch_wolf_field(hipStream_t st, const AtomsDev &at, const Box &bx, const WolfFieldParams &wp, const int2 *tile_pairs, const int *cls,
                       int n_tile_pairs, double *fpart);
void launch_wolf_field_delta(hipStream_t st, const AtomsDev &at, const Box &bx, const WolfFieldParams &wp, const int *mv_slot, const double4 *mv_new, int m,
                             int *moved_idx, const double *e_real, double *e_real_trial, double *dk_part);
void launch_palmo_reduce(hipStream_t st, const AtomsDev &at, const double *mu, const double *f_new, const double *e_induced, double *change, double *scal);

void launch_set_positions(hipStream_t st, const double *pos_dev, const int *perm, double4 *xyzq, int n);

}
```

mpmcxx_amd/csrc/kernels.hip:

```cpp
#include "kernels.h"

namespace mpmc {

__device__ __forceinline__ double wave_sum(double v) {
#pragma unroll
	for (int off = 32; off > 0; off >>= 1) v += __shfl_down(v, off, 64);
	return v;
}
__device__ __forceinline__ int wave_sum_i(int v) {
#pragma unroll
	for (int off = 32; off > 0; off >>= 1) v += __shfl_down(v, off, 64);
	return v;
}
__device__ __forceinline__ double block_sum_256(double v, double *sh) {
	v = wave_sum(v);
	__syncthreads();
	if ((threadIdx.x & 63) == 0) sh[threadIdx.x >> 6] = v;
	__syncthreads();
	return ((sh[0] + sh[1]) + sh[2]) + sh[3];
}

__device__ __forceinline__ void reduce_pairs_block(const double *__restrict__ block_part, const int *__restrict__ block_cnt, int nb,
                                                   double *__restrict__ scal, long long *__restrict__ cnt) {
	__shared__ double sh[4];
	__shared__ long long shc[256];
	double s0 = 0, s1 = 0;
	long long c0 = 0, c1 = 0;
#pragma unroll 4
	for (int b = threadIdx.x; b < nb; b += 256) {
		s0 += block_part[2 * (size_t)b];
		s1 += block_part[2 * (size_t)b + 1];
		c0 += block_cnt[2 * (size_t)b];
		c1 += block_cnt[2 * (size_t)b + 1];
	}
	s0 = block_sum_256(s0, sh);
	s1 = block_sum_256(s1, sh);
	if (threadIdx.x == 0) {
		scal[S_LJ] = s0;
		scal[S_ES_REAL] = s1;
	}
	for (int k = 0; k < 2; ++k) {
		__syncthreads();
		shc[threadIdx.x] = k ? c1 : c0;
		__syncthreads();
		for (int off = 128; off > 0; off >>= 1) {
			if (threadIdx.x < off) shc[threadIdx.x] += shc[threadIdx.x + off];
			__syncthreads();
		}
		if (threadIdx.x == 0) cnt[k ? C_ES_IN : C_LJ_IN] = shc[0];
	}
}
__global__ __launch_bounds__(256) void k_reduce_pairs(const double *__restrict__ block_part, const int *__restrict__ block_cnt, int nb,
                                                      double *__restrict__ scal, long long *__restrict__ cnt) {
	reduce_pairs_block(block_part, block_cnt, nb, scal, cnt);
}

__global__ __launch_bounds__(64) void k_static_counts(AtomsDev at, const int2 *__restrict__ tile_pairs, int *__restrict__ block_cnt) {
	__shared__ int2 s_mf[kTile];
	const int lane = threadIdx.x;
	const int2 IJ = tile_pairs[blockIdx.x];
	const int2 mi = at.mf[IJ.x * kTile + lane];
	s_mf[lane] = at.mf[IJ.y * kTile + lane];
	__syncthreads();
	int n_intra = 0, n_rdx = 0, n_esx = 0, n_fr = 0;
	const bool diag = (IJ.x == IJ.y);
	for (int jj = 0; jj < kTile; ++jj) {
		const int2 mj = s_mf[jj];
		if ((mi.y & AF_PAD) || (mj.y & AF_PAD) || (diag && jj <= lane)) continue;
		const PairFlags f = pair_flags(mi.x, mi.y, mj.x, mj.y);
		n_intra += f.intra;
		n_rdx += f.rd_excluded;
		n_esx += f.es_excluded;
		n_fr += f.frozen;
	}
	n_intra = wave_sum_i(n_intra);
	n_rdx = wave_sum_i(n_rdx);
	n_esx = wave_sum_i(n_esx);
	n_fr = wave_sum_i(n_fr);
	if (lane == 0) {
		int *bc = block_cnt + 4 * (size_t)blockIdx.x;
		bc[0] = n_intra;
		bc[1] = n_rdx;
		bc[2] = n_esx;
		bc[3] = n_fr;
	}
}
__global__ __launch_bounds__(256) void k_reduce_counts4(const int *__restrict__ block_cnt, int nb, long long *__restrict__ cnt4) {
	__shared__ long long shc[256];
	long long c[4] = {0, 0, 0, 0};
#pragma unroll 4
	for (int b = threadIdx.x; b < nb; b += 256)
		for (int k = 0; k < 4; ++k) c[k] += block_cnt[4 * (size_t)b + k];
	for (int k = 0; k < 4; ++k) {
		__syncthreads();
		shc[threadIdx.x] = c[k];
		__syncthreads();
		for (int off = 128; off > 0; off >>= 1) {
			if (threadIdx.x < off) shc[threadIdx.x] += shc[threadIdx.x + off];
			__syncthreads();
		}
		if (threadIdx.x == 0) cnt4[k] = shc[0];
	}
}
void launch_static_counts(hipStream_t st, const AtomsDev &at, const int2 *tile_pairs, int n_tile_pairs, int *block_cnt, long long *cnt4) {
	hipLaunchKernelGGL(k_static_counts, dim3(n_tile_pairs), dim3(kTile), 0, st, at, tile_pairs, block_cnt);
	hipLaunchKernelGGL(k_reduce_counts4, dim3(1), dim3(256), 0, st, block_cnt, n_tile_pairs, cnt4);
}

void launch_reduce_pairs(hipStream_t st, const double *block_part, const int *block_cnt, int nb, double *scal, long long *cnt) {
	hipLaunchKernelGGL(k_reduce_pairs, dim3(1), dim3(256), 0, st, block_part, block_cnt, nb, scal, cnt);
}

__global__ __launch_bounds__(256) void k_recip_sf(AtomsDev at, RecipDev rc) {
	__shared__ double sh[4];
	const double4 kv = rc.kvec[blockIdx.x];
	double re = 0, im = 0, C = 0, S = 0;
	for (int a = threadIdx.x; a < at.n; a += 256) {
		const double4 p = at.xyzq[a];
		const int fl = at.mf[a].y;
		const double ph = ((kv.x * p.x) + kv.y * p.y) + kv.z * p.z;
		double s, c;
		sincos(ph, &s, &c);
		const double qc = p.w * c, qs = p.w * s;
		C += qc;
		S += qs;
		if (!(fl & (AF_FROZEN | AF_ZERO_Q))) {
			re += qc;
			im += qs;
		}
	}
	re = block_sum_256(re, sh);
	im = block_sum_256(im, sh);
	C = block_sum_256(C, sh);
	S = block_sum_256(S, sh);
	if (threadIdx.x == 0) rc.sf[blockIdx.x] = make_double4(re, im, C, S);
}

__device__ const double kBinom6[7] = {1, 6, 15, 20, 15, 6, 1};
__device__ const double kBinom12[13] = {1, 12, 66, 220, 495, 792, 924, 792, 495, 220, 66, 12, 1};

constexpr int kAtomTermSums = 34, kAtomTermBlocks = 64;
static_assert((size_t)kAtomTermSums * kAtomTermBlocks <= kAtomTermScratch, "scratch of launch_atom_terms");
__global__ __launch_bounds__(256) void k_atom_terms_part(AtomsDev at, Box bx, double ewald_alpha, int rd_lrc, int do_es,
                                                         double *__restrict__ part ) {
	double self = 0, lrc = 0;
	double m[13], mf[13], d6 = 0, d12 = 0, df6 = 0, df12 = 0, na = 0, nfa = 0;
	for (int k = 0; k < 13; ++k) m[k] = mf[k] = 0;
	for (int a = blockIdx.x * 256 + threadIdx.x; a < at.n; a += gridDim.x * 256) {
		const int fl = at.mf[a].y;
		const double2 l = at.lj[a];
		if (rd_lrc && !(fl & (AF_NULL_RD | AF_NEG_SIGMA))) {
			double pw = l.y;
			const bool fr = (fl & AF_FROZEN) != 0;
			for (int k = 0; k < 13; ++k) {
				m[k] += pw;
				if (fr) mf[k] += pw;
				pw *= l.x;
			}
			const double t2 = 2.0 * l.x, t6 = (t2 * t2 * t2) * (t2 * t2 * t2), e2 = l.y * l.y;
			d6 += e2 * t6;
			d12 += e2 * t6 * t6;
			na += 1.0;
			if (fr) {
				df6 += e2 * t6;
				df12 += e2 * t6 * t6;
				nfa += 1.0;
			}
		}
		if (fl & AF_FROZEN) continue;
		const double q = at.xyzq[a].w;
		if (do_es) self -= ewald_alpha * q * q / sqrt(kPi);
		if (rd_lrc && !(fl & AF_NULL_RD)) lrc += lrc_term(l.x, at.eps[a], bx.cutoff, bx.volume);
	}
	__shared__ double s_w[4][kAtomTermSums];
	const int lane = threadIdx.x & 63, w = threadIdx.x >> 6;
	auto put = [&](int slot, double v) {
		v = wave_sum(v);
		if (lane == 0) s_w[w][slot] = v;
	};
	put(0, self);
	put(1, lrc);
	for (int k = 0; k < 13; ++k) {
		put(2 + k, m[k]);
		put(15 + k, mf[k]);
	}
	put(28, d6);
	put(29, d12);
	put(30, df6);
	put(31, df12);
	put(32, na);
	put(33, nfa);
	__syncthreads();
	if (threadIdx.x < kAtomTermSums)
		part[(size_t)blockIdx.x * kAtomTermSums + threadIdx.x] = ((s_w[0][threadIdx.x] + s_w[1][threadIdx.x]) + s_w[2][threadIdx.x]) + s_w[3][threadIdx.x];
}
__global__ __launch_bounds__(64) void k_atom_terms_finish(const double *__restrict__ part, int nb, Box bx, int rd_lrc, double *__restrict__ scal) {
	__shared__ double s[kAtomTermSums];
	if (threadIdx.x < kAtomTermSums) {
		double v = 0;
#pragma unroll 8
		for (int b = 0; b < nb; ++b) v += part[(size_t)b * kAtomTermSums + threadIdx.x];
		s[threadIdx.x] = v;
	}
	__syncthreads();
	if (threadIdx.x == 0) {
		const double *m = s + 2, *mf = s + 15;
		const double d6 = s[28], d12 = s[29], df6 = s[30], df12 = s[31];
		double s6 = 0, s12 = 0, f6 = 0, f12 = 0;
		for (int k = 0; k <= 6; ++k) {
			s6 += kBinom6[k] * m[k] * m[6 - k];
			f6 += kBinom6[k] * mf[k] * mf[6 - k];
		}
		for (int k = 0; k <= 12; ++k) {
			s12 += kBinom12[k] * m[k] * m[12 - k];
			f12 += kBinom12[k] * mf[k] * mf[12 - k];
		}
		const double p6 = (0.5 * (s6 - d6) - 0.5 * (f6 - df6)) / 64.0;
		const double p12 = (0.5 * (s12 - d12) - 0.5 * (f12 - df12)) / 4096.0;
		const double rc3 = bx.cutoff * bx.cutoff * bx.cutoff, rc9 = rc3 * rc3 * rc3;
		const bool no_pair = s[32] * (s[32] - 1.0) == s[33] * (s[33] - 1.0);
		scal[S_LRC_PAIR] = (rd_lrc && !no_pair) ? (16.0 / 3.0) * kPi * (p12 / (3.0 * rc9) - p6 / rc3) / bx.volume : 0.0;
		scal[S_ES_SELF] = s[0];
		scal[S_LRC_SELF] = s[1];
	}
}

__device__ __forceinline__ double2 cmul(double2 a, double2 b) { return make_double2(a.x * b.x - a.y * b.y, a.x * b.y + a.y * b.x); }
__device__ __forceinline__ double2 phase_base(const Box &bx, const double4 &p, int q) {
	const double g = (bx.r[q] * p.x + bx.r[3 + q] * p.y) + bx.r[6 + q] * p.z;
	double s, c;
	sincos(2.0 * kPi * g, &s, &c);
	return make_double2(c, s);
}

__global__ __launch_bounds__(256) void k_recip_sf_tab(AtomsDev at, Box bx, RecipDev rc, int kmax, double4 *__restrict__ part) {
	extern __shared__ double2 tab[];
	__shared__ double s_q[kTile], s_qe[kTile];
	const int KM1 = kmax + 1;
	const int tile = blockIdx.x, tid = threadIdx.x;
	for (int idx = tid; idx < 3 * kTile; idx += 256) {
		const int a = idx & 63, q = idx >> 6;
		const double2 base = phase_base(bx, at.xyzq[tile * kTile + a], q);
		double2 *row = tab + (size_t)(q * kTile + a) * KM1;
		double2 v = make_double2(1.0, 0.0);
		row[0] = v;
		for (int m = 1; m <= kmax; ++m) {
			v = cmul(v, base);
			row[m] = v;
		}
	}
	if (tid < kTile) {
		const int i = tile * kTile + tid;
		const int fl = at.mf[i].y;
		const double q = (fl & AF_PAD) ? 0.0 : at.xyzq[i].w;
		s_q[tid] = q;
		s_qe[tid] = (fl & (AF_FROZEN | AF_ZERO_Q | AF_PAD)) ? 0.0 : q;
	}
	__syncthreads();
	const int k = blockIdx.y * 256 + tid;
	if (k >= rc.K) return;
	const int4 l = rc.lvec[k];
	const int ay = abs(l.y), az = abs(l.z);
	const double sy = (l.y < 0) ? -1.0 : 1.0, sz = (l.z < 0) ? -1.0 : 1.0;
	double re = 0, im = 0, C = 0, S = 0;
	for (int a = 0; a < kTile; ++a) {
		const double2 ex = tab[(size_t)a * KM1 + l.x];
		double2 ey = tab[(size_t)(kTile + a) * KM1 + ay];
		double2 ez = tab[(size_t)(2 * kTile + a) * KM1 + az];
		ey.y *= sy;
		ez.y *= sz;
		const double2 e = cmul(cmul(ex, ey), ez);
		const double q = s_q[a], qe = s_qe[a];
		C += q * e.x;
		S += q * e.y;
		re += qe * e.x;
		im += qe * e.y;
	}
	part[(size_t)tile * rc.K + k] = make_double4(re, im, C, S);
}
__global__ __launch_bounds__(256) void k_recip_sf_reduce(RecipDev rc, const double4 *__restrict__ part, int n_tiles) {
	__shared__ double4 sh[16][16];
	const int kk = threadIdx.x & 15, g = threadIdx.x >> 4;
	const int k = blockIdx.x * 16 + kk;
	double4 acc = make_double4(0, 0, 0, 0);
	if (k < rc.K)
		for (int t = g; t < n_tiles; t += 16) {
			const double4 v = part[(size_t)t * rc.K + k];
			acc.x += v.x;
			acc.y += v.y;
			acc.z += v.z;
			acc.w += v.w;
		}
	sh[g][kk] = acc;
	__syncthreads();
	if (g == 0 && k < rc.K) {
		double4 r = sh[0][kk];
		for (int j = 1; j < 16; ++j) {
			r.x += sh[j][kk].x;
			r.y += sh[j][kk].y;
			r.z += sh[j][kk].z;
			r.w += sh[j][kk].w;
		}
		rc.sf[k] = r;
	}
}

void launch_recip_sf(hipStream_t st, const AtomsDev &at, const Box &bx, const RecipDev &rc, int kmax, double4 *sf_part) {
	if (rc.K <= 0) return;
	if (sf_part && rc.lvec && kmax <= kRecipTabMaxK) {
		const int nt = at.n_pad / kTile;
		const size_t lds = (size_t)3 * kTile * (kmax + 1) * sizeof(double2);
		hipLaunchKernelGGL(k_recip_sf_tab, dim3(nt, (rc.K + 255) / 256), dim3(256), lds, st, at, bx, rc, kmax, sf_part);
		hipLaunchKernelGGL(k_recip_sf_reduce, dim3((rc.K + 15) / 16), dim3(256), 0, st, rc, sf_part, nt);
		return;
	}
	hipLaunchKernelGGL(k_recip_sf, dim3(rc.K), dim3(256), 0, st, at, rc);
}
void launch_atom_terms(hipStream_t st, const AtomsDev &at, const Box &bx, double ewald_alpha, int rd_lrc, int do_es, double *part_scratch,
                       double *scal) {
	const int nb = std::max(1, std::min(kAtomTermBlocks, (at.n + 255) / 256));
	hipLaunchKernelGGL(k_atom_terms_part, dim3(nb), dim3(256), 0, st, at, bx, ewald_alpha, rd_lrc, do_es, part_scratch);
	hipLaunchKernelGGL(k_atom_terms_finish, dim3(1), dim3(64), 0, st, part_scratch, nb, bx, rd_lrc, scal);
}

__global__ __launch_bounds__(256) void k_recip_energy(RecipDev rc, Box bx, double *__restrict__ scal) {
	__shared__ double sh[4];
	double e = 0;
	for (int k = threadIdx.x; k < rc.K; k += 256) {
		const double4 sf = rc.sf[k];
		e += rc.w_en[k] * (sf.x * sf.x + sf.y * sf.y);
	}
	e = block_sum_256(e, sh);
	if (threadIdx.x == 0) scal[S_ES_RECIP] = e * (4.0 * kPi / bx.volume);
}
void launch_recip_energy(hipStream_t st, const RecipDev &rc, const Box &bx, double *scal) {
	hipLaunchKernelGGL(k_recip_energy, dim3(1), dim3(256), 0, st, rc, bx, scal);
}


__global__ __launch_bounds__(64) void k_field_recip(AtomsDev at, RecipDev rc, double *__restrict__ e_part ) {
	const int i = blockIdx.x * kTile + threadIdx.x;
	const int per = (rc.K + (int)gridDim.y - 1) / (int)gridDim.y;
	const int k0 = blockIdx.y * per, k1 = min(rc.K, k0 + per);
	const double4 p = at.xyzq[i];
	double ex = 0, ey = 0, ez = 0;
	for (int k = k0; k < k1; ++k) {
		const double4 kv = rc.kvec[k];
		const double4 sf = rc.sf[k];
		const double4 kw = rc.kw[k];
		const double ph = ((kv.x * p.x) + kv.y * p.y) + kv.z * p.z;
		double s, c;
		sincos(ph, &s, &c);
		const double g = s * sf.z - c * sf.w;
		ex += kw.x * g;
		ey += kw.y * g;
		ez += kw.z * g;
	}
	double *o = e_part + ((size_t)blockIdx.y * at.n_pad + i) * 3;
	o[0] = ex;
	o[1] = ey;
	o[2] = ez;
}

constexpr int kSlotGroups = 8;
__device__ __forceinline__ void slot_sum_64(const double *__restrict__ part, int n_slots, int n_pad, int i, int a, int g,
                                            double (*sh)[kTile][3], double out[3]) {
	double f[3] = {0, 0, 0};
	const int gs = __builtin_amdgcn_readfirstlane(g);
	const size_t tile0 = (size_t)__builtin_amdgcn_readfirstlane(i - a);
	const unsigned lane3 = 3u * (unsigned)a;
#pragma unroll 4
	for (int t = gs; t < n_slots; t += kSlotGroups) {
		const double *__restrict__ q = part + ((size_t)t * n_pad + tile0) * 3;
		f[0] += q[lane3];
		f[1] += q[lane3 + 1];
		f[2] += q[lane3 + 2];
	}
	sh[g][a][0] = f[0];
	sh[g][a][1] = f[1];
	sh[g][a][2] = f[2];
	__syncthreads();
	if (g == 0) {
		for (int p = 0; p < 3; ++p) {
			double v = sh[0][a][p];
			for (int k = 1; k < kSlotGroups; ++k) v += sh[k][a][p];
			out[p] = v;
		}
	}
}

__global__ __launch_bounds__(512) void k_field_finalize(AtomsDev at, Box bx, int polar_ewald, const double *__restrict__ e_recip_part,
                                                        const double *__restrict__ part, int n_split, double gamma,
                                                        double *__restrict__ e_static, double *__restrict__ mu, double *__restrict__ e_real_out, int n_kslices,
                                                        double *__restrict__ mu_copy) {
	__shared__ double sh[kSlotGroups][kTile][3];
	__shared__ double shk[kSlotGroups][kTile][3];
	const int a = threadIdx.x & 63, g = threadIdx.x >> 6;
	const int i = blockIdx.x * kTile + a;
	double real[3];
	double e[3] = {0, 0, 0};
	if (polar_ewald) slot_sum_64(e_recip_part, n_kslices, at.n_pad, i, a, g, shk, e);
	slot_sum_64(part, n_split, at.n_pad, i, a, g, sh, real);
	if (g != 0) return;
	if (e_real_out)
		for (int p = 0; p < 3; ++p) e_real_out[3 * (size_t)i + p] = real[p];
	if (polar_ewald) {
		const double sc = 8.0 * kPi / bx.volume;
		for (int p = 0; p < 3; ++p) e[p] *= sc;
	}
	for (int p = 0; p < 3; ++p) e[p] += real[p];
	const double al = at.alpha[i];
	for (int p = 0; p < 3; ++p) {
		e_static[3 * (size_t)i + p] = e[p];
		const double m0 = (al * e[p]) * gamma;
		mu[3 * (size_t)i + p] = m0;
		if (mu_copy) mu_copy[3 * (size_t)i + p] = m0;
	}
}

constexpr int kFieldRecipWaves = 4;
__global__ __launch_bounds__(64 * kFieldRecipWaves) void k_field_recip_tab(AtomsDev at, Box bx, RecipDev rc, int kmax, double *__restrict__ e_part) {
	extern __shared__ double2 tab[];
	__shared__ double s_e[kFieldRecipWaves][3][kTile];
	const int KM1 = kmax + 1;
	const int lane = threadIdx.x & 63, w = __builtin_amdgcn_readfirstlane(threadIdx.x >> 6), i = blockIdx.x * kTile + lane;
	if (w < 3) {
		const double2 base = phase_base(bx, at.xyzq[i], w);
		double2 v = make_double2(1.0, 0.0);
		tab[(size_t)(w * KM1) * kTile + lane] = v;
		for (int m = 1; m <= kmax; ++m) {
			v = cmul(v, base);
			tab[(size_t)(w * KM1 + m) * kTile + lane] = v;
		}
	}
	__syncthreads();
	const int per = (rc.K + (int)gridDim.y - 1) / (int)gridDim.y;
	const int s0 = blockIdx.y * per, s1 = min(rc.K, s0 + per);
	const int quarter = (s1 - s0 + kFieldRecipWaves - 1) / kFieldRecipWaves;
	const int k0 = min(s1, s0 + w * quarter), k1 = min(s1, k0 + quarter);
	double ex = 0, ey = 0, ez = 0;
#pragma unroll 8
	for (int k = k0; k < k1; ++k) {
		const int4 l = rc.lvec[k];
		const double4 sf = rc.sf[k];
		const double4 kw = rc.kw[k];
		const double2 a = tab[(size_t)l.x * kTile + lane];
		double2 b = tab[(size_t)(KM1 + abs(l.y)) * kTile + lane];
		double2 c = tab[(size_t)(2 * KM1 + abs(l.z)) * kTile + lane];
		if (l.y < 0) b.y = -b.y;
		if (l.z < 0) c.y = -c.y;
		const double2 e = cmul(cmul(a, b), c);
		const double g = e.y * sf.z - e.x * sf.w;
		ex += kw.x * g;
		ey += kw.y * g;
		ez += kw.z * g;
	}
	s_e[w][0][lane] = ex;
	s_e[w][1][lane] = ey;
	s_e[w][2][lane] = ez;
	__syncthreads();
	if (w == 0) {
		double *o = e_part + ((size_t)blockIdx.y * at.n_pad + i) * 3;
#pragma unroll
		for (int d = 0; d < 3; ++d) o[d] = ((s_e[0][d][lane] + s_e[1][d][lane]) + s_e[2][d][lane]) + s_e[3][d][lane];
	}
}

__global__ __launch_bounds__(64) void k_post_results(double *__restrict__ scal, double *__restrict__ out_host, double seq) {
	static_assert(S_COUNT + C_COUNT <= 64, "one wave posts the scalar block");
	const int t = threadIdx.x;
	if (t < S_COUNT + C_COUNT) {
		const double v = scal[t];
		out_host[t] = v;
		scal[t] = 0.0;
	}
	__threadfence_system();
	if (t == 0) __hip_atomic_store(out_host + S_COUNT + C_COUNT, seq, __ATOMIC_RELEASE, __HIP_MEMORY_SCOPE_SYSTEM);
}
void launch_post_results(hipStream_t st, double *scal, double *out_host, double seq) {
	hipLaunchKernelGGL(k_post_results, dim3(1), dim3(64), 0, st, scal, out_host, seq);
}

void launch_field_recip(hipStream_t st, const AtomsDev &at, const Box &bx, const RecipDev &rc, int kmax, double *e_recip_part) {
	if (rc.lvec && kmax <= kRecipTabMaxK) {
		const size_t lds = (size_t)3 * kTile * (kmax + 1) * sizeof(double2);
		hipLaunchKernelGGL(k_field_recip_tab, dim3(at.n_pad / kTile, recip_ksplit(at.n_pad)), dim3(kTile * kFieldRecipWaves), lds, st, at, bx, rc, kmax, e_recip_part);
		return;
	}
	hipLaunchKernelGGL(k_field_recip, dim3(at.n_pad / kTile, recip_ksplit(at.n_pad)), dim3(kTile), 0, st, at, rc, e_recip_part);
}

void launch_field_finalize(hipStream_t st, const AtomsDev &at, const Box &bx, int polar_ewald, const double *e_recip_part, const double *part,
                           int n_split, double gamma, double *e_static, double *mu, double *e_real_out, double *mu_copy) {
	hipLaunchKernelGGL(k_field_finalize, dim3(at.n_pad / kTile), dim3(kTile * kSlotGroups), 0, st, at, bx, polar_ewald, e_recip_part, part, n_split,
	                   gamma, e_static, mu, e_real_out, recip_ksplit(at.n_pad), mu_copy);
}

__device__ __forceinline__ void iteration_verdict(int *__restrict__ ctl, int *__restrict__ host_flag, int it, bool lane_broke) {
	const bool wave_broke = __any(lane_broke);
	if ((threadIdx.x & 63) != 0) return;
	if (wave_broke) atomicOr(&ctl[0], 1);
	__threadfence();
	const int ticket = atomicAdd(&ctl[2], 1);
	if (ticket != (int)gridDim.x - 1) return;
	__threadfence();
	const int broke = atomicOr(&ctl[0], 0);
	if (!broke) ctl[1] = it;
	ctl[0] = 0;
	ctl[2] = 0;
	if (host_flag) {
		__hip_atomic_store(host_flag + 1, broke ? 0 : it, __ATOMIC_RELAXED, __HIP_MEMORY_SCOPE_SYSTEM);
		__hip_atomic_store(host_flag, it, __ATOMIC_RELEASE, __HIP_MEMORY_SCOPE_SYSTEM);
	}
}

__device__ __forceinline__ void dipole_update_block(const AtomsDev &at, const double *__restrict__ e_static, const double *__restrict__ part,
                                                    int n_split, const double *__restrict__ mu_old, double *__restrict__ mu_new,
                                                    double *__restrict__ e_induced, int want_rrms, double *__restrict__ rrms_atom,
                                                    double allowed_sqerr, int *__restrict__ ctl, int *__restrict__ host_flag, int it,
                                                    double *__restrict__ dk) {
	__shared__ double sh[kSlotGroups][kTile][3];
	if (ctl && ctl[1] != 0) return;
	const int a = threadIdx.x & 63, g = threadIdx.x >> 6;
	const int i = blockIdx.x * kTile + a;
	double fsum[3];
	slot_sum_64(part, n_split, at.n_pad, i, a, g, sh, fsum);
	if (g != 0) return;
	const double al = at.alpha[i];
	const bool live = (i < at.n) && (al != 0.0);
	double f[3] = {0, 0, 0}, nm[3] = {0, 0, 0};
	if (live) {
		for (int p = 0; p < 3; ++p) {
			f[p] = fsum[p];
			nm[p] = al * (e_static[3 * (size_t)i + p] + f[p]);
		}
	}
	bool broke = false;
	double acc = 0, nn = 0;
	for (int p = 0; p < 3; ++p) {
		const double d = nm[p] - mu_old[3 * (size_t)i + p];
		acc += d * d;
		nn += nm[p] * nm[p];
		if (d * d > allowed_sqerr) broke = true;
		mu_new[3 * (size_t)i + p] = nm[p];
		e_induced[3 * (size_t)i + p] = f[p];
		if (dk) dk[3 * (size_t)i + p] = d;
	}
	if (want_rrms) {
		double r = sqrt(acc / nn);
		if (!isfinite(r)) r = 0.0;
		rrms_atom[i] = (i < at.n) ? r : 0.0;
	}
	if (ctl) iteration_verdict(ctl, host_flag, it, allowed_sqerr > 0.0 && broke && i < at.n);
}
__global__ __launch_bounds__(512) void k_dipole_update(AtomsDev at, const double *__restrict__ e_static, const double *__restrict__ part,
                                                       int n_split, const double *__restrict__ mu_old, double *__restrict__ mu_new,
                                                       double *__restrict__ e_induced, int want_rrms, double *__restrict__ rrms_atom,
                                                       double allowed_sqerr, int *__restrict__ ctl, int *__restrict__ host_flag, int it,
                                                       double *__restrict__ dk) {
	dipole_update_block(at, e_static, part, n_split, mu_old, mu_new, e_induced, want_rrms, rrms_atom, allowed_sqerr, ctl, host_flag, it, dk);
}

__global__ __launch_bounds__(256) void k_dipole_reset(AtomsDev at, const double *__restrict__ e_static, double *__restrict__ mu) {
	const int i = blockIdx.x * 256 + threadIdx.x;
	if (i >= at.n_pad) return;
	const double a = at.alpha[i];
	for (int p = 0; p < 3; ++p) mu[3 * (size_t)i + p] = a * e_static[3 * (size_t)i + p];
}

__device__ __forceinline__ void polar_energy_block(const AtomsDev &at, const double *__restrict__ mu, const double *__restrict__ e_static,
                                                   const double *__restrict__ rrms_atom, double *__restrict__ scal) {
	__shared__ double sh[4];
	double u = 0, rr = 0;
#pragma unroll 4
	for (int i = threadIdx.x; i < at.n; i += 256) {
		const size_t b = 3 * (size_t)i;
		u += ((mu[b] * e_static[b]) + mu[b + 1] * e_static[b + 1]) + mu[b + 2] * e_static[b + 2];
		if (rrms_atom) {
			const double r = rrms_atom[i];
			if (isfinite(r)) rr += r;
		}
	}
	u = block_sum_256(u, sh);
	rr = block_sum_256(rr, sh);
	if (threadIdx.x == 0) {
		scal[S_POLAR] = -0.5 * u;
		scal[S_RRMS] = rr / (double)at.n;
	}
}
__global__ __launch_bounds__(256) void k_polar_energy(AtomsDev at, const double *__restrict__ mu, const double *__restrict__ e_static,
                                                      const double *__restrict__ rrms_atom, double *__restrict__ scal) {
	polar_energy_block(at, mu, e_static, rrms_atom, scal);
}

constexpr int kMomentsMax = 2 * (kMomentsMaxHalf + 1);
constexpr int kMomentsOnePassHalf = 5;
template <int H>
__device__ __forceinline__ void polar_moments_one_pass(const AtomsDev &at, const double *__restrict__ dk, const double *__restrict__ e_static,
                                                       double *__restrict__ sh, double *__restrict__ s_m) {
	const size_t stride = 3 * (size_t)at.n_pad;
	double acc[2 * H + 1] = {};
#pragma unroll 2
	for (int i = threadIdx.x; i < at.n; i += 256) {
		const size_t b = 3 * (size_t)i;
		const double al = at.alpha[i];
		double d[H + 1][3], w[3];
#pragma unroll
		for (int a = 0; a <= H; ++a) {
			const double *__restrict__ q = dk + (size_t)a * stride + b;
			d[a][0] = q[0], d[a][1] = q[1], d[a][2] = q[2];
		}
		w[0] = e_static[b], w[1] = e_static[b + 1], w[2] = e_static[b + 2];
		const double inv = (al != 0.0) ? 1.0 / al : 0.0;
#pragma unroll
		for (int a = 0; a <= H; ++a) {
			if (a > 0) w[0] = d[a][0] * inv, w[1] = d[a][1] * inv, w[2] = d[a][2] * inv;
			acc[2 * a] += ((w[0] * d[a][0]) + w[1] * d[a][1]) + w[2] * d[a][2];
			if (a < H) acc[2 * a + 1] += ((w[0] * d[a + 1][0]) + w[1] * d[a + 1][1]) + w[2] * d[a + 1][2];
		}
	}
#pragma unroll
	for (int k = 0; k <= 2 * H; ++k) {
		const double v = block_sum_256(acc[k], sh);
		if (threadIdx.x == 0) s_m[k] = v;
	}
}
__device__ __forceinline__ void polar_moments_block(const AtomsDev &at, const double *__restrict__ dk, const double *__restrict__ e_static, int n_iter,
                                                    double *__restrict__ scal) {
	__shared__ double sh[4];
	__shared__ double s_m[kMomentsMax];
	const size_t stride = 3 * (size_t)at.n_pad;
	const int half = (n_iter + 1) / 2;
	switch (half <= kMomentsOnePassHalf ? half : 0) {
	case 1: polar_moments_one_pass<1>(at, dk, e_static, sh, s_m); break;
	case 2: polar_moments_one_pass<2>(at, dk, e_static, sh, s_m); break;
	case 3: polar_moments_one_pass<3>(at, dk, e_static, sh, s_m); break;
	case 4: polar_moments_one_pass<4>(at, dk, e_static, sh, s_m); break;
	case 5: polar_moments_one_pass<5>(at, dk, e_static, sh, s_m); break;
	default: break;
	}
	for (int a = 0; a <= (half <= kMomentsOnePassHalf ? -1 : half); ++a) {
		const double *__restrict__ da = dk + (size_t)a * stride;
		const bool odd = 2 * a + 1 <= n_iter;
		const double *__restrict__ db = odd ? da + stride : da;
		double m0 = 0, m1 = 0;
		if (a == 0) {
#pragma unroll 4
			for (int i = threadIdx.x; i < at.n; i += 256) {
				const size_t b = 3 * (size_t)i;
				const double w0 = e_static[b], w1 = e_static[b + 1], w2 = e_static[b + 2];
				m0 += ((w0 * da[b]) + w1 * da[b + 1]) + w2 * da[b + 2];
				m1 += ((w0 * db[b]) + w1 * db[b + 1]) + w2 * db[b + 2];
			}
		} else {
#pragma unroll 4
			for (int i = threadIdx.x; i < at.n; i += 256) {
				const size_t b = 3 * (size_t)i;
				const double al = at.alpha[i];
				const double inv = (al != 0.0) ? 1.0 / al : 0.0;
				const double w0 = da[b] * inv, w1 = da[b + 1] * inv, w2 = da[b + 2] * inv;
				m0 += ((w0 * da[b]) + w1 * da[b + 1]) + w2 * da[b + 2];
				m1 += ((w0 * db[b]) + w1 * db[b + 1]) + w2 * db[b + 2];
			}
		}
		m0 = block_sum_256(m0, sh);
		m1 = block_sum_256(m1, sh);
		if (threadIdx.x == 0) {
			s_m[2 * a] = m0;
			s_m[2 * a + 1] = odd ? m1 : 0.0;
		}
	}
	if (threadIdx.x == 0) {
		double u = 0;
		for (int k = 0; k <= n_iter; ++k) u += s_m[k];
		scal[S_POLAR] = -0.5 * u;
		scal[S_RRMS] = 0.0;
	}
}
__global__ __launch_bounds__(256) void k_polar_moments(AtomsDev at, const double *__restrict__ dk, const double *__restrict__ e_static, int n_iter,
                                                       double *__restrict__ scal) {
	polar_moments_block(at, dk, e_static, n_iter, scal);
}
__global__ __launch_bounds__(256) void k_polar_moments_and_pairs(AtomsDev at, const double *__restrict__ dk, const double *__restrict__ e_static, int n_iter,
                                                                 const double *__restrict__ block_part, const int *__restrict__ block_cnt, int nb,
                                                                 double *__restrict__ scal, long long *__restrict__ cnt) {
	if (blockIdx.x == 0) polar_moments_block(at, dk, e_static, n_iter, scal);
	else reduce_pairs_block(block_part, block_cnt, nb, scal, cnt);
}
void launch_polar_moments(hipStream_t st, const AtomsDev &at, const double *dk, const double *e_static, int n_iter, double *scal) {
	hipLaunchKernelGGL(k_polar_moments, dim3(1), dim3(256), 0, st, at, dk, e_static, n_iter, scal);
}
void launch_polar_moments_and_pairs(hipStream_t st, const AtomsDev &at, const double *dk, const double *e_static, int n_iter, const double *block_part,
                                    const int *block_cnt, int nb, double *scal, long long *cnt) {
	hipLaunchKernelGGL(k_polar_moments_and_pairs, dim3(2), dim3(256), 0, st, at, dk, e_static, n_iter, block_part, block_cnt, nb, scal, cnt);
}

__global__ __launch_bounds__(256) void k_polar_energy_and_pairs(AtomsDev at, const double *__restrict__ mu, const double *__restrict__ e_static,
                                                                const double *__restrict__ rrms_atom, const double *__restrict__ block_part,
                                                                const int *__restrict__ block_cnt, int nb, double *__restrict__ scal,
                                                                long long *__restrict__ cnt) {
	if (blockIdx.x == 0) polar_energy_block(at, mu, e_static, rrms_atom, scal);
	else reduce_pairs_block(block_part, block_cnt, nb, scal, cnt);
}

void launch_dipole_update(hipStream_t st, const AtomsDev &at, const double *e_static, const double *part, int n_split, const double *mu_old,
                          double *mu_new, double *e_induced, int want_rrms, double *rrms_atom, double allowed_sqerr, int *ctl, int *host_flag, int it,
                          double *dk) {
	hipLaunchKernelGGL(k_dipole_update, dim3(at.n_pad / kTile), dim3(kTile * kSlotGroups), 0, st, at, e_static, part, n_split, mu_old, mu_new,
	                   e_induced, want_rrms, rrms_atom, allowed_sqerr, ctl, host_flag, it, dk);
}
void launch_dipole_reset(hipStream_t st, const AtomsDev &at, const double *e_static, double *mu) {
	hipLaunchKernelGGL(k_dipole_reset, dim3((at.n_pad + 255) / 256), dim3(256), 0, st, at, e_static, mu);
}
void launch_polar_energy(hipStream_t st, const AtomsDev &at, const double *mu, const double *e_static, const double *rrms_atom, double *scal) {
	hipLaunchKernelGGL(k_polar_energy, dim3(1), dim3(256), 0, st, at, mu, e_static, rrms_atom, scal);
}
void launch_polar_energy_and_pairs(hipStream_t st, const AtomsDev &at, const double *mu, const double *e_static, const double *rrms_atom,
                                   const double *block_part, const int *block_cnt, int nb, double *scal, long long *cnt) {
	hipLaunchKernelGGL(k_polar_energy_and_pairs, dim3(2), dim3(256), 0, st, at, mu, e_static, rrms_atom, block_part, block_cnt, nb, scal, cnt);
}

template <bool ORTHO>
__global__ __launch_bounds__(256) void k_amatrix_rows(AtomsDev at, const int *__restrict__ slot_of, Box bx, double lambda, int atom0,
                                                      int natoms_rows, double *__restrict__ a) {
	const int j = blockIdx.x * 256 + threadIdx.x;
	const int ir = blockIdx.y;
	if (j >= at.n || ir >= natoms_rows) return;
	const int i = atom0 + ir;
	const size_t ld = 3 * (size_t)at.n;
	double *blk = a + (3 * (size_t)ir) * ld + 3 * (size_t)j;
	if (i == j) {
		const double al = at.alpha[slot_of[i]];
		for (int p = 0; p < 3; ++p)
			for (int q = 0; q < 3; ++q) blk[p * ld + q] = (p == q) ? ((al != 0.0) ? 1.0 / al : kMaxValue) : 0.0;
		return;
	}
	const int lo = min(i, j), hi = max(i, j);
	const double4 pl = at.xyzq[slot_of[lo]], ph = at.xyzq[slot_of[hi]];
	double d[3];
	const double r = min_image<ORTHO>(bx, pl.x - ph.x, pl.y - ph.y, pl.z - ph.z, d[0], d[1], d[2]);
	double ir3, ir5;
	if (r == 0.0)
		ir3 = ir5 = kMaxValue;
	else {
		const double inv = 1.0 / r;
		ir3 = inv * inv * inv;
		ir5 = ir3 * inv * inv;
	}
	const double r2 = r * r, l2 = lambda * lambda, l3 = l2 * lambda;
	const double explr = exp(-lambda * r);
	const double damp1 = 1.0 - explr * (0.5 * l2 * r2 + lambda * r + 1.0);
	const double damp2 = damp1 - explr * (l3 * r2 * r / 6.0);
	for (int p = 0; p < 3; ++p)
		for (int q = 0; q < 3; ++q) {
			double v = -3.0 * d[p] * d[q] * damp2 * ir5;
			if (p == q) v += damp1 * ir3;
			blk[p * ld + q] = v;
		}
}

void launch_amatrix_rows(hipStream_t st, const AtomsDev &at, const int *slot_of, const Box &bx, double polar_damp, int row0, int nrows, double *a) {
	const int atom0 = row0 / 3, nat = nrows / 3;
	dim3 grid((at.n + 255) / 256, nat), block(256);
	if (bx.ortho)
		hipLaunchKernelGGL(k_amatrix_rows<true>, grid, block, 0, st, at, slot_of, bx, polar_damp, atom0, nat, a);
	else
		hipLaunchKernelGGL(k_amatrix_rows<false>, grid, block, 0, st, at, slot_of, bx, polar_damp, atom0, nat, a);
}

__global__ __launch_bounds__(256) void k_set_positions(const double *__restrict__ pos, const int *__restrict__ perm, double4 *__restrict__ xyzq, int n) {
	const int k = blockIdx.x * 256 + threadIdx.x;
	if (k >= n) return;
	const int i = perm[k];
	double4 v = xyzq[k];
	v.x = pos[3 * (size_t)i + 0];
	v.y = pos[3 * (size_t)i + 1];
	v.z = pos[3 * (size_t)i + 2];
	xyzq[k] = v;
}
void launch_set_positions(hipStream_t st, const double *pos_dev, const int *perm, double4 *xyzq, int n) {
	if (n > 0) hipLaunchKernelGGL(k_set_positions, dim3((n + 255) / 256), dim3(256), 0, st, pos_dev, perm, xyzq, n);
}

}
```

mpmcxx_amd/csrc/kernels_panel.hip:

```cpp
#include "kernels.h"
#include "device_math.h"

namespace mpmc {

int panel_segment_entries(int J) { return J / 2 + 3; }
constexpr int kPanFar = 8, kPanDiag = 16;
#ifndef MPMC_PANEL_WAVES
#define MPMC_PANEL_WAVES 2
#endif
constexpr int kPanelWaves = MPMC_PANEL_WAVES;
#ifndef MPMC_PANEL_PIPE
#define MPMC_PANEL_PIPE 4
#endif
constexpr double kFarSumScale = 0.125;

__device__ __forceinline__ int tp_index(int I, int J, int nt) { return I * nt - (I * (I - 1)) / 2 + (J - I); }

__global__ __launch_bounds__(64) void k_build_panels(const int *__restrict__ cls, int nt, const int *__restrict__ seg, int4 *__restrict__ panels) {
	__shared__ int s_odd[16][33];
	const int J = blockIdx.x, lane = threadIdx.x;
	if (J >= nt) return;
	int4 *out = panels + seg[J];
	const int cap = seg[J + 1] - seg[J];
	int n = 0;
	if (lane == 0) out[0] = make_int4(tp_index(J, J, nt), -1, ((cls[tp_index(J, J, nt)] / CLS_UNIFORM_X) & 7) | kPanDiag, J);
	n = 1;
	int pend[16];
#pragma unroll
	for (int k = 0; k < 16; ++k) pend[k] = -1;
	const unsigned long long lt = (lane == 0) ? 0ull : (~0ull >> (64 - lane));
	for (int I0 = 0; I0 < J; I0 += 64) {
		const int I = I0 + lane;
		const bool live = I < J;
		const int tp = live ? tp_index(I, J, nt) : -1;
		const int c = live ? cls[tp] : 0;
		const int key = ((c & CLS_THOLE_FAR) ? 8 : 0) | ((c / CLS_UNIFORM_X) & 7);
#pragma unroll
		for (int k = 0; k < 16; ++k) {
			const unsigned long long mask = __ballot(live && key == k);
			if (mask == 0ull) continue;
			const int cnt = __popcll(mask);
			const bool mine = live && key == k;
			const int shift = (pend[k] >= 0) ? 1 : 0;
			const int rank = __popcll(mask & lt) + shift;
			const int total = cnt + shift;
			if (mine && (rank & 1)) s_odd[k][rank >> 1] = tp;
			__builtin_amdgcn_fence(__ATOMIC_RELEASE, "wavefront");
			__builtin_amdgcn_wave_barrier();
			if (mine && !(rank & 1) && rank + 1 < total) out[n + (rank >> 1)] = make_int4(tp, s_odd[k][rank >> 1], k, J);
			if (shift && lane == 0) out[n] = make_int4(pend[k], s_odd[k][0], k, J);
			int np = -1;
			if (total & 1) {
				const int top = 63 - __clzll(mask);
				np = __shfl(tp, top, 64);
			}
			n += total >> 1;
			pend[k] = np;
			__builtin_amdgcn_wave_barrier();
		}
	}
	if (lane == 0) {
		for (int far = 0; far < 2; ++far) {
			int prev = -1, prev_um = 0;
#pragma unroll
			for (int um = 7; um >= 0; --um) {
				const int p = pend[far * 8 + um];
				if (p < 0) continue;
				if (prev >= 0) {
					out[n++] = make_int4(prev, p, (prev_um & um) | (far ? kPanFar : 0), J);
					prev = -1;
				} else {
					prev = p;
					prev_um = um;
				}
			}
			if (prev >= 0) out[n++] = make_int4(prev, -1, prev_um | (far ? kPanFar : 0), J);
		}
		for (; n < cap; ++n) out[n] = make_int4(-1, -1, 0, J);
	}
}

template <int NI>
struct PanAcc {
	double f[NI][3];
	double g[3];
};

template <bool FAR, int NU, int NI, bool ROT, bool PAD, bool TRI>
__device__ __forceinline__ void pan_step(const Box &bx, const double2 *__restrict__ s_xy, const double2 *__restrict__ s_zm, const double2 *__restrict__ s_mm,
                                         const double *__restrict__ s_valid, const int jl, const int src4, const double (&L)[3],
                                         const double (&iL)[3], const double (&q)[NI][3], const double (&m)[NI][3], const double2 (&t)[NI],
                                         PanAcc<NI> &A) {
	const double2 xy = s_xy[jl], zm = s_zm[jl], mm = s_mm[jl];
	const double xj = xy.x, yj = xy.y, zj = zm.x, mjx = zm.y, mjy = mm.x, mjz = mm.y;
	double vj = 1.0;
	if (FAR && PAD) vj = s_valid[jl];
#pragma unroll
	for (int k = 0; k < NI; ++k) {
		double ox = q[k][0] - xj, oy = q[k][1] - yj, oz = q[k][2] - zj;
		if (TRI) {
			const double dx = ox, dy = oy, dz = oz;
			if (NU & 1) {
				const double n0 = rint(fma(bx.r[6], dz, fma(bx.r[3], dy, bx.r[0] * dx)));
				ox = fma(-n0, bx.b[0], ox), oy = fma(-n0, bx.b[1], oy), oz = fma(-n0, bx.b[2], oz);
			}
			if (NU & 2) {
				const double n1 = rint(fma(bx.r[7], dz, fma(bx.r[4], dy, bx.r[1] * dx)));
				ox = fma(-n1, bx.b[3], ox), oy = fma(-n1, bx.b[4], oy), oz = fma(-n1, bx.b[5], oz);
			}
			if (NU & 4) {
				const double n2 = rint(fma(bx.r[8], dz, fma(bx.r[5], dy, bx.r[2] * dx)));
				ox = fma(-n2, bx.b[6], ox), oy = fma(-n2, bx.b[7], oy), oz = fma(-n2, bx.b[8], oz);
			}
		} else {
			if (NU > 0) ox = fma(-L[0], rint(iL[0] * ox), ox);
			if (NU > 1) oy = fma(-L[1], rint(iL[1] * oy), oy);
			if (NU > 2) oz = fma(-L[2], rint(iL[2] * oz), oz);
		}
		double ta, tb;
		if (FAR) {
			const double r2 = fma(oz, oz, fma(oy, oy, ox * ox));
			const double y0 = __builtin_amdgcn_rsq(r2);
			const double y2 = y0 * fma(-(r2 * y0), y0, 3.0);
			const double i4 = y2 * y2;
			ta = i4 * y2;
			if (PAD) ta *= vj;
			tb = 0.75 * i4;
			const double sj = tb * fma(oz, mjz, fma(oy, mjy, ox * mjx));
			const double si = tb * fma(oz, m[k][2], fma(oy, m[k][1], ox * m[k][0]));
			A.f[k][0] = fma(ta, fma(sj, ox, -mjx), A.f[k][0]);
			A.f[k][1] = fma(ta, fma(sj, oy, -mjy), A.f[k][1]);
			A.f[k][2] = fma(ta, fma(sj, oz, -mjz), A.f[k][2]);
			A.g[0] = fma(ta, fma(si, ox, -m[k][0]), A.g[0]);
			A.g[1] = fma(ta, fma(si, oy, -m[k][1]), A.g[1]);
			A.g[2] = fma(ta, fma(si, oz, -m[k][2]), A.g[2]);
		} else {
			ta = t[k].x;
			tb = t[k].y;
			const double dj = tb * fma(oz, mjz, fma(oy, mjy, ox * mjx));
			const double di = tb * fma(oz, m[k][2], fma(oy, m[k][1], ox * m[k][0]));
			A.f[k][0] = fma(-ta, mjx, fma(dj, ox, A.f[k][0]));
			A.f[k][1] = fma(-ta, mjy, fma(dj, oy, A.f[k][1]));
			A.f[k][2] = fma(-ta, mjz, fma(dj, oz, A.f[k][2]));
			A.g[0] = fma(-ta, m[k][0], fma(di, ox, A.g[0]));
			A.g[1] = fma(-ta, m[k][1], fma(di, oy, A.g[1]));
			A.g[2] = fma(-ta, m[k][2], fma(di, oz, A.g[2]));
		}
	}
	if (ROT) {
		A.g[0] = rot_from_next(A.g[0]);
		A.g[1] = rot_from_next(A.g[1]);
		A.g[2] = rot_from_next(A.g[2]);
	}
}

template <bool FAR, int NU, int NI, int PIPE, bool TRI>
__device__ __forceinline__ void pan_walk(const Box &bx, const double2 *__restrict__ s_xy, const double2 *__restrict__ s_zm, const double2 *__restrict__ s_mm,
                                         const double *__restrict__ s_valid, const bool pad, const int lane, const int src4,
                                         const double (&L)[3], const double (&iL)[3], const double (&q)[NI][3], const double (&m)[NI][3],
                                         const double2 *__restrict__ ab, const size_t (&ab_tile)[NI], const int s_first, const int n_steps,
                                         PanAcc<NI> &A) {
	int jb = lane + s_first;
	if (FAR) {
		const double2 none[NI] = {};
#define MPMC_FAR_LOOP(P)                                                                                                               \
	for (int kc = 0; kc < n_steps - 4; kc += 4, jb += 4) {                                                                             \
		_Pragma("unroll") for (int u = 0; u < 4; ++u)                                                                                  \
		    pan_step<true, NU, NI, true, P, TRI>(bx, s_xy, s_zm, s_mm, s_valid, jb + u, src4, L, iL, q, m, none, A);                      \
	}                                                                                                                                  \
	_Pragma("unroll") for (int u = 0; u < 3; ++u) pan_step<true, NU, NI, true, P, TRI>(bx, s_xy, s_zm, s_mm, s_valid, jb + u, src4, L, iL, q, m, none, A); \
	pan_step<true, NU, NI, false, P, TRI>(bx, s_xy, s_zm, s_mm, s_valid, jb + 3, src4, L, iL, q, m, none, A);
		if (pad) {
			MPMC_FAR_LOOP(true)
		} else {
			MPMC_FAR_LOOP(false)
		}
#undef MPMC_FAR_LOOP
		return;
	}
	double2 buf[NI][PIPE];
	int voff = s_first * kTile + lane;
#pragma unroll
	for (int k = 0; k < NI; ++k) {
#pragma unroll
		for (int u = 0; u < PIPE; ++u) buf[k][u] = ld_stream<true>(ab + ab_tile[k] + voff + u * kTile);
	}
	for (int kc = 0; kc < n_steps - PIPE; kc += PIPE, jb += PIPE) {
		voff += PIPE * kTile;
#pragma unroll
		for (int u = 0; u < PIPE; ++u) {
			double2 t[NI];
#pragma unroll
			for (int k = 0; k < NI; ++k) t[k] = buf[k][u];
			pan_step<false, NU, NI, true, false, TRI>(bx, s_xy, s_zm, s_mm, s_valid, jb + u, src4, L, iL, q, m, t, A);
#pragma unroll
			for (int k = 0; k < NI; ++k) buf[k][u] = ld_stream<true>(ab + ab_tile[k] + voff + u * kTile);
			__builtin_amdgcn_sched_barrier(0);
		}
	}
#pragma unroll
	for (int u = 0; u < PIPE; ++u) {
		double2 t[NI];
#pragma unroll
		for (int k = 0; k < NI; ++k) t[k] = buf[k][u];
		if (u != PIPE - 1) pan_step<false, NU, NI, true, false, TRI>(bx, s_xy, s_zm, s_mm, s_valid, jb + u, src4, L, iL, q, m, t, A);
		else pan_step<false, NU, NI, false, false, TRI>(bx, s_xy, s_zm, s_mm, s_valid, jb + u, src4, L, iL, q, m, t, A);
		__builtin_amdgcn_sched_barrier(0);
	}
}

template <int PIPE, int NI, bool ORTHO>
__device__ __forceinline__ void panel_block(const AtomsDev &at, const Box &bx, const double *__restrict__ mu, const int2 *__restrict__ tile_pairs,
                                            const double4 *__restrict__ tp_shift, const double2 *__restrict__ ab, double *__restrict__ part,
                                            double *__restrict__ gslot, const int tpA, const int tpB, const int flags, const int J,
                                            double2 *__restrict__ s_xy, double2 *__restrict__ s_zm, double2 *__restrict__ s_mm,
                                            double *__restrict__ s_valid, double (*__restrict__ s_F)[2][3][kTile], double (*__restrict__ s_G)[3][kTile]) {
	const int lane = threadIdx.x & 63, w = threadIdx.x >> 6;
	const int src4 = ((lane + 1) & 63) * 4;
	const int tps[2] = {tpA, tpB};
	const int um = flags & 7;
	const bool far = (flags & kPanFar) != 0, diag = (flags & kPanDiag) != 0;
	const int j0 = J * kTile;
	const int nonuni = (~um) & 7;
	const int nu = __popc(nonuni);
	unsigned packed = 0x24;
	switch (ORTHO ? nonuni : 7) {
	case 2: packed = 0x21; break;
	case 4: packed = 0x12; break;
	case 5: packed = 0x18; break;
	case 6: packed = 0x09; break;
	default: break;
	}
	const int p0 = packed & 3, p1 = (packed >> 2) & 3, p2 = (packed >> 4) & 3;
	auto pick = [](const double x, const double y, const double z, const int p) { return p == 0 ? x : (p == 1 ? y : z); };
	const double L[3] = {pick(bx.b[0], bx.b[4], bx.b[8], p0), pick(bx.b[0], bx.b[4], bx.b[8], p1), pick(bx.b[0], bx.b[4], bx.b[8], p2)};
	const double iL[3] = {pick(bx.r[0], bx.r[4], bx.r[8], p0), pick(bx.r[0], bx.r[4], bx.r[8], p1), pick(bx.r[0], bx.r[4], bx.r[8], p2)};

	const double *__restrict__ xyz = reinterpret_cast<const double *>(at.xyzq);
	const double *__restrict__ xp[3] = {xyz + p0, xyz + p1, xyz + p2}, *__restrict__ mp[3] = {mu + p0, mu + p1, mu + p2};
	if (w == 0) {
		const unsigned a4 = 4u * (unsigned)(j0 + lane), a3 = 3u * (unsigned)(j0 + lane);
		const double2 xy = make_double2(xp[0][a4], xp[1][a4]);
		const double2 zm = make_double2(xp[2][a4], mp[0][a3]);
		const double2 mm = make_double2(mp[1][a3], mp[2][a3]);
		s_xy[lane] = s_xy[lane + kTile] = xy;
		s_zm[lane] = s_zm[lane + kTile] = zm;
		s_mm[lane] = s_mm[lane + kTile] = mm;
		s_valid[lane] = s_valid[lane + kTile] = (at.mf[j0 + lane].y & AF_PAD) ? 0.0 : 1.0;
	}
	double q[NI][3], m[NI][3];
	size_t ab_tile[NI];
	int Is[NI];
#pragma unroll
	for (int k = 0; k < NI; ++k) {
		const int I = tile_pairs[tps[k]].x;
		Is[k] = I;
		const unsigned a4 = 4u * (unsigned)(I * kTile + lane), a3 = 3u * (unsigned)(I * kTile + lane);
		const double4 sh = tp_shift[tps[k]];
		const bool whole = !ORTHO;
		const double sx = (whole || (um & 1)) ? sh.x : 0.0, sy = (whole || (um & 2)) ? sh.y : 0.0, sz = (whole || (um & 4)) ? sh.z : 0.0;
		q[k][0] = xp[0][a4] - pick(sx, sy, sz, p0);
		q[k][1] = xp[1][a4] - pick(sx, sy, sz, p1);
		q[k][2] = xp[2][a4] - pick(sx, sy, sz, p2);
		m[k][0] = mp[0][a3];
		m[k][1] = mp[1][a3];
		m[k][2] = mp[2][a3];
		ab_tile[k] = (size_t)tps[k] * (kTile * kTile);
	}
	__syncthreads();
	const bool pad = (at.n != at.n_pad) && (J == at.n_pad / kTile - 1);
	const int n_steps = (diag ? 32 : 64) / kPanelWaves, s_first = (diag ? 1 : 0) + w * n_steps;
	PanAcc<NI> A = {};
#define MPMC_PWALK(F, N) pan_walk<F, N, NI, PIPE, false>(bx, s_xy, s_zm, s_mm, s_valid, pad, lane, src4, L, iL, q, m, ab, ab_tile, s_first, n_steps, A)
#define MPMC_PWALK_TRI(F, M) pan_walk<F, M, NI, PIPE, true>(bx, s_xy, s_zm, s_mm, s_valid, pad, lane, src4, L, iL, q, m, ab, ab_tile, s_first, n_steps, A)
	if (!ORTHO && nu > 0) {
		if (far) {
			switch (nonuni) {
			case 1: MPMC_PWALK_TRI(true, 1); break;
			case 2: MPMC_PWALK_TRI(true, 2); break;
			case 3: MPMC_PWALK_TRI(true, 3); break;
			case 4: MPMC_PWALK_TRI(true, 4); break;
			case 5: MPMC_PWALK_TRI(true, 5); break;
			case 6: MPMC_PWALK_TRI(true, 6); break;
			default: MPMC_PWALK_TRI(true, 7); break;
			}
		} else MPMC_PWALK_TRI(false, 7);
	} else if (!ORTHO) {
		if (far) MPMC_PWALK(true, 0);
		else MPMC_PWALK(false, 0);
	} else if (far) {
		switch (nu) {
		case 0: MPMC_PWALK(true, 0); break;
		case 1: MPMC_PWALK(true, 1); break;
		case 2: MPMC_PWALK(true, 2); break;
		default: MPMC_PWALK(true, 3); break;
		}
	} else {
		switch (nu) {
		case 0: MPMC_PWALK(false, 0); break;
		case 1: MPMC_PWALK(false, 1); break;
		case 2: MPMC_PWALK(false, 2); break;
		default: MPMC_PWALK(false, 3); break;
		}
	}
#undef MPMC_PWALK
#undef MPMC_PWALK_TRI
	if (far) {
#pragma unroll
		for (int d = 0; d < 3; ++d) {
#pragma unroll
			for (int k = 0; k < NI; ++k) A.f[k][d] *= kFarSumScale;
			A.g[d] *= kFarSumScale;
		}
	}
	{
		const int jl_last = (lane + s_first + n_steps - 1) & 63;
#pragma unroll
		for (int d = 0; d < 3; ++d) {
#pragma unroll
			for (int k = 0; k < NI; ++k) s_F[w][k][d][lane] = A.f[k][d];
			s_G[w][d][jl_last] = A.g[d];
		}
	}
	__syncthreads();
	if (w != 0) return;
	const int nt_pad3 = at.n_pad * 3;
	double g[3];
#pragma unroll
	for (int d = 0; d < 3; ++d) {
		g[d] = s_G[0][d][lane];
#pragma unroll
		for (int v = 1; v < kPanelWaves; ++v) g[d] += s_G[v][d][lane];
	}
#pragma unroll
	for (int k = 0; k < NI; ++k) {
		double f[3];
#pragma unroll
		for (int d = 0; d < 3; ++d) {
			f[d] = s_F[0][k][d][lane];
#pragma unroll
			for (int v = 1; v < kPanelWaves; ++v) f[d] += s_F[v][k][d][lane];
		}
		if (NI == 1 && diag) {
#pragma unroll
			for (int d = 0; d < 3; ++d) {
				f[d] += g[d];
				g[d] = 0.0;
			}
		}
		double *oi = part + (size_t)J * nt_pad3 + 3 * (size_t)(Is[k] * kTile) + lane;
		oi[p0 * kTile] = f[0];
		oi[p1 * kTile] = f[1];
		oi[p2 * kTile] = f[2];
	}
	*(gslot + p0 * kTile + lane) = g[0];
	*(gslot + p1 * kTile + lane) = g[1];
	*(gslot + p2 * kTile + lane) = g[2];
}

constexpr int kUpdGroups = 16;
constexpr int kUpdWaves = 4;
constexpr int kUpdRounds = 2;
struct PanelUpdate {
	const double *e_static;
	const int *seg;
	double *mu_new, *e_induced , *rrms_atom, *dk ;
	double allowed_sqerr;
	int *ctl, *host_flag;
	int nt, it, want_rrms;
};

__device__ __forceinline__ void panel_update_tile(const AtomsDev &at, const PanelUpdate &u, const double *__restrict__ part, const double *__restrict__ gpart,
                                                  const double *__restrict__ mu_old, const int X, double (*__restrict__ sh)[kTile][3]) {
	constexpr int GW = kUpdGroups / kUpdWaves;
	const int a = threadIdx.x & 63, w = __builtin_amdgcn_readfirstlane(threadIdx.x >> 6);
	const int i = X * kTile + a;
	const int nF = u.nt - X, wg0 = u.seg[X], nG = u.seg[X + 1] - wg0;
	double al = 0.0, es[3] = {0, 0, 0}, mo[3] = {0, 0, 0};
	if (w == 0) {
		al = at.alpha[i];
		for (int p = 0; p < 3; ++p) {
			es[p] = u.e_static[3 * (size_t)i + p];
			mo[p] = mu_old[3 * (size_t)i + p];
		}
	}
	double f[GW][3] = {};
	const size_t n_pad = (size_t)at.n_pad;
	const int T = nF + nG;
	const double *__restrict__ pX = part + ((size_t)X * n_pad + (size_t)X * kTile) * 3 + a;
	const double *__restrict__ gX = gpart + (size_t)wg0 * (kTile * 3) + a;
	for (int t0 = 0; t0 < T; t0 += kUpdRounds * kUpdGroups) {
		double v[kUpdRounds][GW][3];
#pragma unroll
		for (int r = 0; r < kUpdRounds; ++r) {
#pragma unroll
			for (int c = 0; c < GW; ++c) {
				const int t = t0 + r * kUpdGroups + w * GW + c;
				const int tc = t < T ? t : T - 1;
				const double *__restrict__ q = tc < nF ? pX + (size_t)tc * n_pad * 3 : gX + (size_t)(tc - nF) * (kTile * 3);
				v[r][c][0] = q[0];
				v[r][c][1] = q[kTile];
				v[r][c][2] = q[2 * kTile];
			}
		}
#pragma unroll
		for (int r = 0; r < kUpdRounds; ++r) {
#pragma unroll
			for (int c = 0; c < GW; ++c) {
				const bool ok = t0 + r * kUpdGroups + w * GW + c < T;
#pragma unroll
				for (int p = 0; p < 3; ++p) f[c][p] += ok ? v[r][c][p] : 0.0;
			}
		}
	}
#pragma unroll
	for (int c = 0; c < GW; ++c) {
		sh[w * GW + c][a][0] = f[c][0];
		sh[w * GW + c][a][1] = f[c][1];
		sh[w * GW + c][a][2] = f[c][2];
	}
	__syncthreads();
	if (w != 0) return;
	double fsum[3];
	for (int p = 0; p < 3; ++p) {
		double v = sh[0][a][p];
		for (int k = 1; k < kUpdGroups; ++k) v += sh[k][a][p];
		fsum[p] = v;
	}
	const bool live = (i < at.n) && (al != 0.0);
	double fo[3] = {0, 0, 0}, nm[3] = {0, 0, 0};
	if (live) {
		for (int p = 0; p < 3; ++p) {
			fo[p] = fsum[p];
			nm[p] = al * (es[p] + fo[p]);
		}
	}
	bool broke = false;
	double acc = 0, nn = 0;
	for (int p = 0; p < 3; ++p) {
		const double d = nm[p] - mo[p];
		acc += d * d;
		nn += nm[p] * nm[p];
		if (d * d > u.allowed_sqerr) broke = true;
		u.mu_new[3 * (size_t)i + p] = nm[p];
		if (u.e_induced) u.e_induced[3 * (size_t)i + p] = fo[p];
		if (u.dk) u.dk[3 * (size_t)i + p] = d;
	}
	if (u.want_rrms) {
		double r = sqrt(acc / nn);
		if (!isfinite(r)) r = 0.0;
		u.rrms_atom[i] = (i < at.n) ? r : 0.0;
	}
	if (u.ctl) {
		int *ctl = u.ctl;
		const bool wave_broke = __any(u.allowed_sqerr > 0.0 && broke && i < at.n);
		if (a != 0) return;
		if (wave_broke) atomicOr(&ctl[0], 1);
		__threadfence();
		const int ticket = atomicAdd(&ctl[2], 1);
		if (ticket != u.nt - 1) return;
		__threadfence();
		const int any_broke = atomicOr(&ctl[0], 0);
		if (!any_broke) ctl[1] = u.it;
		ctl[0] = 0;
		ctl[2] = 0;
		if (u.host_flag) {
			__hip_atomic_store(u.host_flag + 1, any_broke ? 0 : u.it, __ATOMIC_RELAXED, __HIP_MEMORY_SCOPE_SYSTEM);
			__hip_atomic_store(u.host_flag, u.it, __ATOMIC_RELEASE, __HIP_MEMORY_SCOPE_SYSTEM);
		}
	}
}

constexpr int kPanelLdsDouble2 = 6 * kTile + kTile + (kPanelWaves * 2 * 3 * kTile + kPanelWaves * 3 * kTile) / 2;
template <int PIPE, bool ORTHO>
__global__ __launch_bounds__(64 * kPanelWaves) void k_dipole_iter_panel(AtomsDev at, Box bx, const double *__restrict__ mu,
                                                                        const int2 *__restrict__ tile_pairs, const double4 *__restrict__ tp_shift,
                                                                        const int4 *__restrict__ panels, const double2 *__restrict__ ab,
                                                                        double *__restrict__ part, double *__restrict__ gpart ,
                                                                        const int *__restrict__ converged ,
                                                                        long long *__restrict__ trace ) {
	long long t_start = 0;
	if (trace) t_start = wall_clock64();
	__shared__ double2 s_all[kPanelLdsDouble2];
	if (converged && *converged != 0) return;
	double2 *s_xy = s_all, *s_zm = s_all + 2 * kTile, *s_mm = s_all + 4 * kTile;
	double *s_valid = reinterpret_cast<double *>(s_all + 6 * kTile);
	double(*s_F)[2][3][kTile] = reinterpret_cast<double(*)[2][3][kTile]>(s_all + 7 * kTile);
	double(*s_G)[3][kTile] = reinterpret_cast<double(*)[3][kTile]>(s_all + 7 * kTile + kPanelWaves * 2 * 3 * kTile / 2);
	const int ent = (int)gridDim.x - 1 - (int)blockIdx.x;
	const int4 e = panels[ent];
	const int tpA = __builtin_amdgcn_readfirstlane(e.x), tpB = __builtin_amdgcn_readfirstlane(e.y);
	const int flags = __builtin_amdgcn_readfirstlane(e.z), J = __builtin_amdgcn_readfirstlane(e.w);
	double *gslot = gpart + (size_t)ent * kTile * 3;
	if (tpA < 0) {
		if (threadIdx.x < kTile) {
			*(gslot + threadIdx.x) = 0.0;
			*(gslot + kTile + threadIdx.x) = 0.0;
			*(gslot + 2 * kTile + threadIdx.x) = 0.0;
		}
		if (trace && threadIdx.x == 0) trace[4 * (size_t)ent + 1] = 0;
		return;
	}
	if (tpB >= 0) panel_block<PIPE, 2, ORTHO>(at, bx, mu, tile_pairs, tp_shift, ab, part, gslot, tpA, tpB, flags, J, s_xy, s_zm, s_mm, s_valid, s_F, s_G);
	else panel_block<PIPE, 1, ORTHO>(at, bx, mu, tile_pairs, tp_shift, ab, part, gslot, tpA, tpB, flags, J, s_xy, s_zm, s_mm, s_valid, s_F, s_G);
	if (trace && threadIdx.x == 0) {
		long long *o = trace + 4 * (size_t)ent;
		o[0] = t_start;
		o[1] = wall_clock64();
		o[2] = __builtin_amdgcn_s_getreg((4 ) | (0 << 6) | (31 << 11));
		o[3] = __builtin_amdgcn_s_getreg((20 ) | (0 << 6) | (3 << 11));
	}
}

__global__ __launch_bounds__(64 * kUpdWaves) void k_dipole_update_panel(AtomsDev at, const double *__restrict__ part, const double *__restrict__ gpart,
                                                                        const double *__restrict__ mu_old, const PanelUpdate u) {
	__shared__ double sh[kUpdGroups][kTile][3];
	if (u.ctl && u.ctl[1] != 0) return;
	panel_update_tile(at, u, part, gpart, mu_old, blockIdx.x, sh);
}

void launch_build_panels(hipStream_t st, const int *cls, int n_tiles, const int *seg, int4 *panels) {
	hipLaunchKernelGGL(k_build_panels, dim3(n_tiles), dim3(64), 0, st, cls, n_tiles, seg, panels);
}

void launch_dipole_iter_panel(hipStream_t st, const AtomsDev &at, const Box &bx, const double *mu, const int2 *tile_pairs,
                              const double4 *tp_shift, const int4 *panels, int n_entries, const double2 *ab, double *part, double *gpart,
                              const int *converged, long long *trace, int replicas) {
	if (n_entries <= 0) return;
	dim3 grid(n_entries, replicas > 1 ? replicas : 1), block(kTile * kPanelWaves);
	if (bx.ortho)
		hipLaunchKernelGGL((k_dipole_iter_panel<MPMC_PANEL_PIPE, true>), grid, block, 0, st, at, bx, mu, tile_pairs, tp_shift, panels, ab, part, gpart, converged, trace);
	else
		hipLaunchKernelGGL((k_dipole_iter_panel<MPMC_PANEL_PIPE, false>), grid, block, 0, st, at, bx, mu, tile_pairs, tp_shift, panels, ab, part, gpart, converged, trace);
}

void launch_dipole_update_panel(hipStream_t st, const AtomsDev &at, const double *e_static, const double *part, const double *gpart, const int *seg,
                                const double *mu_old, double *mu_new, double *e_induced, int want_rrms, double *rrms_atom, double allowed_sqerr,
                                int *ctl, int *host_flag, int it, double *dk) {
	PanelUpdate u{};
	u.dk = dk;
	u.e_static = e_static, u.seg = seg, u.mu_new = mu_new, u.e_induced = e_induced, u.rrms_atom = rrms_atom, u.allowed_sqerr = allowed_sqerr;
	u.ctl = ctl, u.host_flag = host_flag, u.nt = at.n_pad / kTile, u.it = it, u.want_rrms = want_rrms;
	hipLaunchKernelGGL(k_dipole_update_panel, dim3(at.n_pad / kTile), dim3(kTile * kUpdWaves), 0, st, at, part, gpart, mu_old, u);
}

}
```

mpmcxx_amd/csrc/trial.cpp:

```cpp
#include <atomic>
#include <chrono>

#include "context.h"


using namespace mpmc;

constexpr size_t kMvBlobBytes = MPMC_TRIAL_MAX_ATOMS * (2 * sizeof(int) + sizeof(double4));
static int ensure_trial_buffers(mpmc_ctx *c) {
	int rc;
	if (!c->h_mv_blob) {
		if ((rc = c->d_mv_blob.reserve(c, kMvBlobBytes)) != MPMC_OK) return rc;
		c->d_mv_new = reinterpret_cast<double4 *>(c->d_mv_blob.p);
		c->d_mv_slot = reinterpret_cast<int *>(c->d_mv_blob + MPMC_TRIAL_MAX_ATOMS * sizeof(double4));
		c->d_mv_orig = c->d_mv_slot + MPMC_TRIAL_MAX_ATOMS;
		if ((rc = c->d_moved_idx.reserve(c, (size_t)c->max_pad)) != MPMC_OK) return rc;
		if ((rc = c->d_delta_out.reserve(c, 9)) != MPMC_OK) return rc;
		c->d_delta_cnt = reinterpret_cast<long long *>(c->d_delta_out + 5);
		HIP_TRY(c, hipMemsetAsync(c->d_moved_idx, 0xff, (size_t)c->max_pad * sizeof(int), c->stream));
		if ((rc = c->h_delta_out.reserve(c, 10)) != MPMC_OK) return rc;
		c->h_delta_out[8] = c->h_delta_out[9] = 0.0;
		c->h_delta_cnt = reinterpret_cast<long long *>(c->h_delta_out + 5);
		if ((rc = c->h_mv_blob.reserve(c, kMvBlobBytes)) != MPMC_OK) return rc;
	}
	return c->d_sf_trial.reserve(c, (size_t)c->K);
}

extern "C" int mpmc_trial_begin(mpmc_ctx *c, int first, int count, const double *new_pos) {
	if (!c || !new_pos || first < 0 || count <= 0) return MPMC_ERR_ARG;
	if (!c->atoms_set || first + count > c->n) return fail(c, MPMC_ERR_ARG, "mpmc_trial_begin: range outside the atom list");
	if (c->trial_open) return fail(c, MPMC_ERR_ARG, "mpmc_trial_begin: a trial move is already open (accept or reject it first)");
	if (!c->cache_valid) return fail(c, MPMC_ERR_ARG, "mpmc_trial_begin: no accepted configuration (call mpmc_energy first)");
	for (int t = 0; t < 3 * count; t++)
		if (!std::isfinite(new_pos[t])) return fail(c, MPMC_ERR_INVALID_DATUM, "mpmc_trial_begin: non-finite position");
	c->trial_first = first;
	c->trial_count = count;
	c->trial_new.assign(new_pos, new_pos + 3 * (size_t)count);
	c->trial_old.assign(c->h_pos.begin() + 3 * (size_t)first, c->h_pos.begin() + 3 * (size_t)(first + count));
	c->trial_open = true;
	c->trial_evaluated = false;
	c->trial_enqueued = false;
	c->trial_noop = (std::memcmp(new_pos, c->h_pos.data() + 3 * (size_t)first, 3 * (size_t)count * sizeof(double)) == 0);
	return MPMC_OK;
}

extern "C" int mpmc_trial_energy_async(mpmc_ctx *c) {
	if (!c) return MPMC_ERR_ARG;
	if (!c->trial_open) return fail(c, MPMC_ERR_ARG, "mpmc_trial_energy: no trial move is open");
	if (c->trial_enqueued) return fail(c, MPMC_ERR_ARG, "mpmc_trial_energy_async: already enqueued");
	if (c->trial_noop) {
		c->trial_was_full = false;
		c->trial_enqueued = true;
		return MPMC_OK;
	}
	const mpmc_options &o = c->opts;
	const bool polar = o.polarization && !o.rd_only;
	const int m = c->trial_count;
	c->trial_polar_delta = false;
	const bool no_polar_delta = c->kept.tune.no_polar_delta;
	const bool polar_delta = polar && c->e_real_valid && !no_polar_delta && m <= MPMC_TRIAL_MAX_ATOMS && !o.wolf && !direct_solve(c);
	if ((polar && !polar_delta) || m > MPMC_TRIAL_MAX_ATOMS) {
		c->trial_keep = c->last_full;
		int rc = mpmc_update_positions(c, c->trial_first, m, c->trial_new.data());
		if (rc != MPMC_OK) return rc;
		if ((rc = enqueue(c, full_mask(c))) != MPMC_OK) return rc;
		c->trial_was_full = true;
		c->trial_last_kind = 1;
		c->trial_enqueued = true;
		return MPMC_OK;
	}
	drop_pending_dipoles(c);
	int rc = prepare(c);
	if (rc != MPMC_OK) return rc;
	if ((rc = ensure_trial_buffers(c)) != MPMC_OK) return rc;
	hipStream_t st = c->stream;
	const bool no_inline = c->kept.tune.no_inline_move;
	c->trial_inline = !polar_delta && m <= kMvInline && !no_inline && !c->kept.tb_enabled && !c->kept.de_enabled;
	if (c->trial_inline) {
		for (int t = 0; t < m; t++) {
			const int i = c->trial_first + t;
			c->mv_inline.orig[t] = i;
			c->mv_inline.slot[t] = c->slot_of[i];
			for (int d = 0; d < 3; d++) c->mv_inline.nw[t][d] = c->trial_new[3 * t + d];
			c->mv_inline.nw[t][3] = c->h_q[i];
		}
		for (int t = m; t < kMvInline; t++) {
			c->mv_inline.orig[t] = c->mv_inline.slot[t] = 0;
			for (int d = 0; d < 4; d++) c->mv_inline.nw[t][d] = 0.0;
		}
	} else {
		double4 *nw = reinterpret_cast<double4 *>(c->h_mv_blob.p);
		int *slots = reinterpret_cast<int *>(c->h_mv_blob + MPMC_TRIAL_MAX_ATOMS * sizeof(double4));
		int *origs = slots + MPMC_TRIAL_MAX_ATOMS;
		for (int t = 0; t < m; t++) {
			const int i = c->trial_first + t;
			origs[t] = i;
			slots[t] = c->slot_of[i];
			nw[t] = make_double4(c->trial_new[3 * t], c->trial_new[3 * t + 1], c->trial_new[3 * t + 2], c->h_q[i]);
		}
		HIP_TRY(c, hipMemcpyAsync(c->d_mv_blob, c->h_mv_blob, kMvBlobBytes, hipMemcpyHostToDevice, st));
	}
	const int do_es = o.rd_only ? 0 : 1;
	if (c->kept.tb_enabled) {
		if ((rc = three_body_ready(c)) != MPMC_OK) return rc;
		ProfScope p(c, MPMC_K_THREE_BODY);
		launch_three_body_delta(st, atoms_view(c), c->d_tb_au, c->box, kThreeBodyScale, c->d_mv_slot, c->d_mv_new, m, c->d_moved_idx, c->d_tb_part,
		                        c->d_delta_out + 7);
	}
	if (c->kept.de_enabled) {
		if ((rc = disp_ready(c)) != MPMC_OK) return rc;
		ProfScope p(c, MPMC_K_PAIR);
		launch_disp_expansion_delta(st, atoms_view(c), c->d_de_co, c->d_de_t10, c->box, disp_params(c), c->d_mv_slot, c->d_mv_new, m, c->d_moved_idx,
		                            c->d_de_part, c->d_delta_out + 8);
	}
	{
		FusedParams fp{};
		fp.ewald_alpha = c->ewald_alpha;
		ext_params(c, fp, o.wolf && do_es);
		ProfScope p(c, MPMC_K_PAIR);
		launch_delta(st, atoms_view(c), c->d_slot_of, c->box, recip_view(c), fp, do_es, c->d_mv_slot, c->d_mv_orig, c->d_mv_new, m,
		             c->d_moved_idx, c->d_sf_trial, c->d_block_part, c->d_block_cnt, c->d_delta_out, c->d_delta_cnt, c->h_delta_out,
		             (c->trial_seq += 1.0), c->trial_inline ? &c->mv_inline : nullptr);
	}
	HIP_TRY(c, hipGetLastError());
	c->trial_was_full = false;
	c->trial_last_kind = 0;
	if (polar_delta) {
		if ((rc = c->d_dk_part.reserve(c, (size_t)c->n_tiles * (size_t)m * 3, (size_t)c->n_tiles * MPMC_TRIAL_MAX_ATOMS * 3)) != MPMC_OK) return rc;
		const AtomsDev at = atoms_view(c);
		{
			ProfScope p(c, MPMC_K_FIELD);
			if (wolf_field_on(c))
				launch_wolf_field_delta(st, at, c->box, wolf_field_params(c->kept.pw_alpha, c->box.cutoff), c->d_mv_slot, c->d_mv_new, m, c->d_moved_idx, c->d_e_real,
				                        c->d_e_real_trial, c->d_dk_part);
			else
				launch_delta_field(st, at, c->box, c->polar_ewald_alpha, o.polar_ewald, c->d_mv_slot, c->d_mv_new, m, c->d_moved_idx, c->d_e_real,
				                   c->d_e_real_trial, c->d_dk_part);
			launch_swap_positions(st, c->d_xyzq, c->d_mv_slot, c->d_mv_new, m);
			if (o.polar_ewald) {
				RecipDev rt = recip_view(c);
				rt.sf = c->d_sf_trial;
				launch_field_recip(st, at, c->box, rt, o.ewald_kmax, c->d_e_recip_part);
			}
			c->mu_cur = 0;
			if (polar_moments_apply(c) && (rc = reserve_dk_ring(c)) != MPMC_OK) return rc;
			launch_field_finalize(st, at, c->box, o.polar_ewald, c->d_e_recip_part, c->d_e_real_trial, 1, o.polar_gamma, c->d_e_static, c->d_mu[0], nullptr,
			                      polar_moments_apply(c) ? c->d_dk_ring.p : nullptr);
		}
		HIP_TRY(c, hipGetLastError());
		c->trial_polar_delta = true;
		c->trial_tiles.clear();
		for (int t = 0; t < m; t++) {
			const int tile = c->slot_of[c->trial_first + t] / kTile;
			if (std::find(c->trial_tiles.begin(), c->trial_tiles.end(), tile) == c->trial_tiles.end()) c->trial_tiles.push_back(tile);
		}
		std::vector<int> touch = c->trial_tiles;
		for (int tile : c->store_dirty_tiles)
			if (std::find(touch.begin(), touch.end(), tile) == touch.end()) touch.push_back(tile);
		c->touch_n = (touch.size() <= 8) ? (int)touch.size() : -1;
		for (int k = 0; k < c->touch_n; k++) c->touch[k] = touch[k];
		rc = enqueue(c, RUN_STORE | RUN_SOLVE);
		c->touch_n = -1;
		if (rc != MPMC_OK) return rc;
		c->store_dirty_tiles = c->trial_tiles;
	}
	c->trial_enqueued = true;
	return MPMC_OK;
}

extern "C" int mpmc_trial_energy_wait(mpmc_ctx *c, mpmc_result *out) {
	if (!c || !out) return MPMC_ERR_ARG;
	if (!c->trial_open || !c->trial_enqueued) return fail(c, MPMC_ERR_ARG, "mpmc_trial_energy_wait: nothing enqueued");
	c->trial_enqueued = false;
	if (c->trial_noop) {
		c->trial_res = c->last_full;
		c->trial_evaluated = true;
		*out = c->trial_res;
		return MPMC_OK;
	}
	if (c->trial_was_full) {
		int rc = mpmc_energy_wait(c, out);
		if (rc != MPMC_OK) return rc;
		c->trial_res = *out;
		c->last_full = c->trial_keep;
		c->trial_evaluated = true;
		return MPMC_OK;
	}
	HIP_TRY(c, hipSetDevice(c->device));
	mpmc_result solved{};
	if (c->trial_polar_delta) {
		const mpmc_result keep = c->last_full;
		int rc = wait_and_fill(c, &solved);
		c->last_full = keep;
		if (rc != MPMC_OK) return rc;
	} else {
		bool seen = false;
		if (c->ev_used.empty()) {
			volatile const double *flag = c->h_delta_out + 8;
			const double want = c->trial_seq;
			seen = poll_posted(c, [&] { return *flag == want; }, std::chrono::microseconds(1000));
		}
		if (!seen) {
			c->kept.n_stream_syncs++;
			HIP_TRY(c, hipStreamSynchronize(c->stream));
		}
		prof_harvest(c);
	}
	const int do_es = c->opts.rd_only ? 0 : 1;
	const mpmc_result &a = c->last_full;
	mpmc_result r = a;
	r.lj_pairs = a.lj_pairs + (c->kept.de_enabled ? c->h_delta_out[9] : c->h_delta_out[0]);
	r.rd_energy = (r.lj_pairs + r.lrc_pair) + r.lrc_self;
	r.n_lj_in_cutoff = a.n_lj_in_cutoff + c->h_delta_cnt[0];
	if (do_es) {
		r.es_real = a.es_real + (c->h_delta_out[1] - c->h_delta_out[2]);
		r.es_recip = c->h_delta_out[3];
		r.coulombic_energy = (r.es_real + r.es_recip) + r.es_self;
		r.n_es_in_cutoff = a.n_es_in_cutoff + c->h_delta_cnt[1];
	}
	if (c->trial_polar_delta) {
		r.polarization_energy = solved.polarization_energy;
		r.dipole_rrms = solved.dipole_rrms;
		r.polar_iterations = solved.polar_iterations;
		r.iterator_failed = solved.iterator_failed;
	}
	if (c->kept.tb_enabled) r.three_body_energy = a.three_body_energy + c->h_delta_out[7];
	r.energy = r.rd_energy + r.coulombic_energy + r.polarization_energy + r.vdw_energy + r.three_body_energy;
	r.NU = r.N * r.energy;
	c->trial_res = r;
	c->trial_evaluated = true;
	*out = r;
	return MPMC_OK;
}

extern "C" int mpmc_trial_energy(mpmc_ctx *c, mpmc_result *out) {
	if (!c || !out) return MPMC_ERR_ARG;
	int rc = mpmc_trial_energy_async(c);
	if (rc != MPMC_OK) return rc;
	return mpmc_trial_energy_wait(c, out);
}

extern "C" int mpmc_trial_accept(mpmc_ctx *c) {
	if (!c) return MPMC_ERR_ARG;
	if (!c->trial_open || !c->trial_evaluated) return fail(c, MPMC_ERR_ARG, "mpmc_trial_accept: no evaluated trial move");
	HIP_TRY(c, hipSetDevice(c->device));
	const int m = c->trial_count;
	if (c->trial_noop) {
		c->trial_open = false;
		return MPMC_OK;
	}
	if (!c->trial_was_full) {
		if (c->trial_polar_delta) {
			std::swap(c->d_e_real, c->d_e_real_trial);
			c->store_dirty_tiles.clear();
		} else {
			if (c->trial_inline) launch_commit_positions_inline(c->stream, c->d_xyzq, c->mv_inline, m);
			else launch_commit_positions(c->stream, c->d_xyzq, c->d_mv_slot, c->d_mv_new, m);
		}
		HIP_TRY(c, hipGetLastError());
		std::swap(c->d_sf, c->d_sf_trial);
		for (int t = 0; t < 3 * m; t++) c->h_pos[3 * (size_t)c->trial_first + t] = c->trial_new[t];
		{
			const int rc_g = mirror_guard(c);
			if (rc_g != MPMC_OK) return rc_g;
		}
		for (int t = 0; t < m; t++) {
			double4 &v = c->h_xyzq[c->slot_of[c->trial_first + t]];
			v.x = c->trial_new[3 * t], v.y = c->trial_new[3 * t + 1], v.z = c->trial_new[3 * t + 2];
		}
	}
	c->last_full = c->trial_res;
	c->cache_valid = true;
	c->trial_open = false;
	c->trial_polar_delta = false;
	return MPMC_OK;
}

extern "C" int mpmc_trial_reject(mpmc_ctx *c) {
	if (!c) return MPMC_ERR_ARG;
	if (!c->trial_open) return fail(c, MPMC_ERR_ARG, "mpmc_trial_reject: no trial move is open");
	if (c->trial_enqueued) {
		mpmc_result drop;
		int rc = mpmc_trial_energy_wait(c, &drop);
		if (rc != MPMC_OK) return rc;
	}
	c->trial_open = false;
	if (c->trial_polar_delta) {
		HIP_TRY(c, hipSetDevice(c->device));
		launch_swap_positions(c->stream, c->d_xyzq, c->d_mv_slot, c->d_mv_new, c->trial_count);
		HIP_TRY(c, hipGetLastError());
		c->trial_polar_delta = false;
		return MPMC_OK;
	}
	if (c->trial_evaluated && c->trial_was_full) {
		const mpmc_result keep = c->last_full;
		int rc = mpmc_update_positions(c, c->trial_first, c->trial_count, c->trial_old.data());
		if (rc != MPMC_OK) return rc;
		c->last_full = keep;
		c->cache_valid = true;
		c->e_real_valid = false;
		const bool polar = c->opts.polarization && !c->opts.rd_only;
		if (!polar && !c->opts.wolf) {
			mpmc_result tmp;
			if ((rc = mpmc_energy(c, &tmp)) != MPMC_OK) return rc;
		}
	}
	return MPMC_OK;
}
```

Before: 1953.

## Compute polarization moments per tile inside update kernels and fuse tail with result posting

Each Jacobi dipole-update kernel (and the field-finalize kernel) now reduces its tile's moment terms in-wave and writes per-tile partials. A single tail kernel then folds those partials, reduces the pair blocks, and posts results to the host. This replaces a single-block pass that re-read the whole dk ring over all atoms, and drops a separate post-results launch. Field finalize also moves to a four-wave slot sum. The cost is extra loads and shuffles in each update kernel, plus a new per-tile buffer.

```diff
diff --git a/mpmcxx_amd/csrc/context.h b/mpmcxx_amd/csrc/context.h
--- a/mpmcxx_amd/csrc/context.h
+++ b/mpmcxx_amd/csrc/context.h
@@ -212,6 +212,7 @@
 	DevBuf<double> d_gs_ul;
 	int mu_cur = 0;
 	DevBuf<double> d_dk_ring;
+	DevBuf<double> d_moment_part;
 	enum { PEND_NONE = 0, PEND_OPEN = 1, PEND_DROPPED = 2 };
 	int polar_pending = PEND_NONE;
 	int pend_done = 0, pend_target = 0;
@@ -445,7 +446,11 @@
 	       !o.polar_gs;
 }
 inline int moments_half(int n) { return (n + 1) / 2; }
-inline int reserve_dk_ring(mpmc_ctx *c) { return c->d_dk_ring.reserve(c, (size_t)(moments_half(c->opts.polar_max_iter) + 1) * 3 * (size_t)c->max_pad); }
+inline int reserve_dk_ring(mpmc_ctx *c) {
+	const int rc = c->d_moment_part.reserve(c, (size_t)(c->max_pad / kTile) * kMomentsMax);
+	if (rc != MPMC_OK) return rc;
+	return c->d_dk_ring.reserve(c, (size_t)(moments_half(c->opts.polar_max_iter) + 1) * 3 * (size_t)c->max_pad);
+}
 int finish_pending_dipoles(mpmc_ctx *c);
 inline void drop_pending_dipoles(mpmc_ctx *c) {
 	if (c->polar_pending == mpmc_ctx::PEND_OPEN) c->polar_pending = mpmc_ctx::PEND_DROPPED;
diff --git a/mpmcxx_amd/csrc/evaluate.cpp b/mpmcxx_amd/csrc/evaluate.cpp
--- a/mpmcxx_amd/csrc/evaluate.cpp
+++ b/mpmcxx_amd/csrc/evaluate.cpp
@@ -264,7 +264,7 @@
 	return jp;
 }
 static void enqueue_jacobi_iteration(mpmc_ctx *c, const AtomsDev &at, const JacobiPlan &jp, int it, int want_rrms, double allowed, int *ctl, int *host_flag,
-                                     double *dk) {
+                                     double *dk, const MomentOut &mo = MomentOut()) {
 	hipStream_t st = c->stream;
 	const mpmc_options &o = c->opts;
 	const int *converged = ctl ? ctl + 1 : nullptr;
@@ -291,10 +291,10 @@
 		ProfScope p(c, MPMC_K_REDUCE);
 		if (jp.compact && c->panels_built && !jp.dense)
 			launch_dipole_update_panel(st, at, c->d_e_static, c->d_part, c->d_gpart, c->d_seg, c->d_mu[c->mu_cur], c->d_mu[1 - c->mu_cur],
-			                           c->d_e_induced, want_rrms, c->d_rrms, allowed, ctl, host_flag, it, dk);
+			                           c->d_e_induced, want_rrms, c->d_rrms, allowed, ctl, host_flag, it, dk, mo);
 		else
 			launch_dipole_update(st, at, c->d_e_static, c->d_part, jp.iter_slots, c->d_mu[c->mu_cur], c->d_mu[1 - c->mu_cur], c->d_e_induced,
-			                     want_rrms, c->d_rrms, allowed, ctl, host_flag, it, dk);
+			                     want_rrms, c->d_rrms, allowed, ctl, host_flag, it, dk, mo);
 	}
 	c->mu_cur = 1 - c->mu_cur;
 }
@@ -470,6 +470,7 @@
 	}
 	if ((side_work && side_fork) || panel_side) join_side(c);
 	const bool reduce_in_tail = (mask & RUN_PAIR) && (mask & RUN_SOLVE);
+	bool posted = false;
 	if ((mask & RUN_PAIR) && !reduce_in_tail) {
 		ProfScope p(c, MPMC_K_REDUCE);
 		launch_reduce_pairs(st, c->d_block_part, c->d_block_cnt, c->n_tile_pairs, c->d_scal, c->d_cnt);
@@ -481,7 +482,7 @@
 		if (wolf_field_on(c))
 			launch_wolf_field(st, at, c->box, wolf_field_params(c->kept.pw_alpha, c->box.cutoff), c->d_tile_pairs, c->d_cls, c->n_tile_pairs, c->d_part);
 		launch_field_finalize(st, at, c->box, o.polar_ewald, c->d_e_recip_part, c->d_part, c->n_tiles, o.polar_gamma, c->d_e_static,
-		                      c->d_mu[0], c->d_e_real, polar_moments_apply(c) ? c->d_dk_ring.p : nullptr);
+		                      c->d_mu[0], c->d_e_real, polar_moments_apply(c) ? c->d_dk_ring.p : nullptr, polar_moments_apply(c) ? c->d_moment_part.p : nullptr);
 		c->e_real_valid = (mask == full_mask(c));
 	}
 
@@ -556,7 +557,9 @@
 				}
 				continue;
 			}
-			enqueue_jacobi_iteration(c, at, jp, it, want_rrms, allowed, ctl, host_flag, (moments && it <= half) ? c->d_dk_ring + (size_t)it * dk_stride : nullptr);
+			MomentOut mo;
+			if (moments && it <= half) mo.part = c->d_moment_part, mo.d_prev = c->d_dk_ring + (size_t)(it - 1) * dk_stride, mo.k = it, mo.n_iter = o.polar_max_iter;
+			enqueue_jacobi_iteration(c, at, jp, it, want_rrms, allowed, ctl, host_flag, (moments && it <= half) ? c->d_dk_ring + (size_t)it * dk_stride : nullptr, mo);
 			if (by_precision) {
 				if (it % check_every == 0 || it + 1 >= kMaxIterationCount) {
 					HIP_TRY(c, hipGetLastError());
@@ -585,10 +588,10 @@
 		c->pend_done = it, c->pend_target = o.polar_max_iter;
 		if (moments) {
 			ProfScope p(c, MPMC_K_REDUCE);
-			if (reduce_in_tail)
-				launch_polar_moments_and_pairs(st, at, c->d_dk_ring, c->d_e_static, o.polar_max_iter, c->d_block_part, c->d_block_cnt, c->n_tile_pairs, c->d_scal,
-				                               c->d_cnt);
-			else launch_polar_moments(st, at, c->d_dk_ring, c->d_e_static, o.polar_max_iter, c->d_scal);
+			posted = !(mask & (RUN_THREE_BODY | RUN_DISP));
+			if (posted) c->single_seq += 1.0;
+			launch_moments_tail(st, c->d_moment_part, c->n_tiles, o.polar_max_iter, reduce_in_tail ? c->d_block_part.p : nullptr, c->d_block_cnt, c->n_tile_pairs,
+			                    c->d_scal, posted ? c->h_scal.p : nullptr, c->single_seq);
 		} else {
 			ProfScope p(c, MPMC_K_REDUCE);
 			if (reduce_in_tail)
@@ -620,8 +623,10 @@
 		                      c->d_de_part, c->d_scal + S_DISP);
 	}
 	HIP_TRY(c, hipGetLastError());
-	c->single_seq += 1.0;
-	launch_post_results(st, c->d_scal, c->h_scal, c->single_seq);
+	if (!posted) {
+		c->single_seq += 1.0;
+		launch_post_results(st, c->d_scal, c->h_scal, c->single_seq);
+	}
 	HIP_TRY(c, hipGetLastError());
 	c->scal_clean = true;
 	c->spin_on_post = c->ev_used.empty() && (c->kept.tune.poll_long || c->n_tile_pairs <= kOneStreamMaxPairs);
diff --git a/mpmcxx_amd/csrc/kernels.h b/mpmcxx_amd/csrc/kernels.h
--- a/mpmcxx_amd/csrc/kernels.h
+++ b/mpmcxx_amd/csrc/kernels.h
@@ -67,21 +67,57 @@
 void launch_field_finalize(hipStream_t st, const AtomsDev &at, const Box &bx, int polar_ewald, const double *e_recip,
                            const double *part, int n_split, double gamma, double *e_static, double *mu,
                            double *e_real_out = nullptr ,
-                           double *mu_copy = nullptr );
-
-void launch_dipole_update(hipStream_t st, const AtomsDev &at, const double *e_static, const double *part, int n_split,
-                          const double *mu_old, double *mu_new, double *e_induced, int want_rrms, double *rrms_atom,
-                          double allowed_sqerr, int *ctl, int *host_flag , int it,
-                          double *dk = nullptr );
+                           double *mu_copy = nullptr ,
+                           double *moment_part = nullptr );
+
 void launch_dipole_reset(hipStream_t st, const AtomsDev &at, const double *e_static, double *mu);
 void launch_post_results(hipStream_t st, double *scal, double *out_host, double seq);
 void launch_polar_energy(hipStream_t st, const AtomsDev &at, const double *mu, const double *e_static, const double *rrms_atom,
                          double *scal);
 constexpr int kMomentsMaxIter = 64;
 constexpr int kMomentsMaxHalf = (kMomentsMaxIter + 1) / 2;
-void launch_polar_moments(hipStream_t st, const AtomsDev &at, const double *dk, const double *e_static, int n_iter, double *scal);
-void launch_polar_moments_and_pairs(hipStream_t st, const AtomsDev &at, const double *dk, const double *e_static, int n_iter,
-                                    const double *block_part, const int *block_cnt, int nb, double *scal, long long *cnt);
+constexpr int kMomentsMax = 2 * (kMomentsMaxHalf + 1);
+struct MomentOut {
+	double *part = nullptr;
+	const double *d_prev = nullptr;
+	int k = 0, n_iter = 0;
+};
+__device__ __forceinline__ double moment_term(bool live, const double w[3], const double d[3]) {
+	return live ? ((w[0] * d[0]) + w[1] * d[1]) + w[2] * d[2] : 0.0;
+}
+__device__ __forceinline__ double moment_lane_sum(double v) {
+#pragma unroll
+	for (int off = 32; off > 0; off >>= 1) v += __shfl_down(v, off, 64);
+	return v;
+}
+__device__ __forceinline__ void moment_pair_store(const MomentOut &mo, bool live, double al, const double es[3], const double dp[3],
+                                                  const double dn[3], int lane, int tile) {
+	const double inv = (al != 0.0) ? 1.0 / al : 0.0;
+	const bool even = 2 * mo.k <= mo.n_iter;
+	double w[3], wn[3];
+	for (int p = 0; p < 3; ++p) {
+		w[p] = (mo.k == 1) ? es[p] : dp[p] * inv;
+		wn[p] = dn[p] * inv;
+	}
+	double m_odd = moment_term(live, w, dn), m_even = even ? moment_term(live, wn, dn) : 0.0;
+#pragma unroll
+	for (int off = 32; off > 0; off >>= 1) {
+		m_odd += __shfl_down(m_odd, off, 64);
+		m_even += __shfl_down(m_even, off, 64);
+	}
+	if (lane == 0) {
+		double *o = mo.part + (size_t)tile * kMomentsMax + 2 * mo.k - 1;
+		o[0] = m_odd;
+		if (even) o[1] = m_even;
+	}
+}
+void launch_dipole_update(hipStream_t st, const AtomsDev &at, const double *e_static, const double *part, int n_split,
+                          const double *mu_old, double *mu_new, double *e_induced, int want_rrms, double *rrms_atom,
+                          double allowed_sqerr, int *ctl, int *host_flag , int it,
+                          double *dk = nullptr ,
+                          const MomentOut &mo = MomentOut() );
+void launch_moments_tail(hipStream_t st, const double *moment_part, int n_tiles, int n_iter, const double *block_part, const int *block_cnt, int nb,
+                         double *scal, double *out_host, double seq);
 
 void launch_amatrix_rows(hipStream_t st, const AtomsDev &at, const int *slot_of, const Box &bx, double polar_damp, int row0, int nrows,
                          double *a );
@@ -152,7 +188,8 @@
                               int replicas = 1 );
 void launch_dipole_update_panel(hipStream_t st, const AtomsDev &at, const double *e_static, const double *part, const double *gpart, const int *seg,
                                 const double *mu_old, double *mu_new, double *e_induced, int want_rrms, double *rrms_atom, double allowed_sqerr,
-                                int *ctl, int *host_flag, int it, double *dk = nullptr );
+                                int *ctl, int *host_flag, int it, double *dk = nullptr ,
+                                const MomentOut &mo = MomentOut() );
 void launch_rot_selftest(hipStream_t st, int *out);
 
 void launch_dense_build(hipStream_t st, const AtomsDev &at, const Box &bx, double polar_damp, double *a, bool upper_only = false);
diff --git a/mpmcxx_amd/csrc/kernels.hip b/mpmcxx_amd/csrc/kernels.hip
--- a/mpmcxx_amd/csrc/kernels.hip
+++ b/mpmcxx_amd/csrc/kernels.hip
@@ -389,19 +389,63 @@
 	}
 }
 
-__global__ __launch_bounds__(512) void k_field_finalize(AtomsDev at, Box bx, int polar_ewald, const double *__restrict__ e_recip_part,
-                                                        const double *__restrict__ part, int n_split, double gamma,
-                                                        double *__restrict__ e_static, double *__restrict__ mu, double *__restrict__ e_real_out, int n_kslices,
-                                                        double *__restrict__ mu_copy) {
+constexpr int kSlotWaves = 4;
+__device__ __forceinline__ void slot_sum_64_four_waves(const double *__restrict__ part, int n_slots, int n_pad, int i, int a, int w,
+                                                       double (*sh)[kTile][3], double out[3]) {
+	constexpr int GW = kSlotGroups / kSlotWaves;
+	static_assert(GW == 2, "the walk below is written for two groups per wave");
+	double f[GW][3] = {};
+	const int g0 = __builtin_amdgcn_readfirstlane(w) * GW;
+	const size_t tile0 = (size_t)__builtin_amdgcn_readfirstlane(i - a);
+	const unsigned lane3 = 3u * (unsigned)a;
+	const size_t slot = (size_t)n_pad * 3;
+	int t = g0;
+#pragma unroll 4
+	for (; t + 1 < n_slots; t += kSlotGroups) {
+		const double *__restrict__ q = part + ((size_t)t * n_pad + tile0) * 3;
+		f[0][0] += q[lane3];
+		f[0][1] += q[lane3 + 1];
+		f[0][2] += q[lane3 + 2];
+		f[1][0] += q[slot + lane3];
+		f[1][1] += q[slot + lane3 + 1];
+		f[1][2] += q[slot + lane3 + 2];
+	}
+	if (t < n_slots) {
+		const double *__restrict__ q = part + ((size_t)t * n_pad + tile0) * 3;
+		f[0][0] += q[lane3];
+		f[0][1] += q[lane3 + 1];
+		f[0][2] += q[lane3 + 2];
+	}
+#pragma unroll
+	for (int c = 0; c < GW; ++c) {
+		sh[g0 + c][a][0] = f[c][0];
+		sh[g0 + c][a][1] = f[c][1];
+		sh[g0 + c][a][2] = f[c][2];
+	}
+	__syncthreads();
+	if (w == 0) {
+		for (int p = 0; p < 3; ++p) {
+			double v = sh[0][a][p];
+			for (int k = 1; k < kSlotGroups; ++k) v += sh[k][a][p];
+			out[p] = v;
+		}
+	}
+}
+
+__global__ __launch_bounds__(64 * kSlotWaves) void k_field_finalize(AtomsDev at, Box bx, int polar_ewald, const double *__restrict__ e_recip_part,
+                                                                    const double *__restrict__ part, int n_split, double gamma,
+                                                                    double *__restrict__ e_static, double *__restrict__ mu, double *__restrict__ e_real_out, int n_kslices,
+                                                                    double *__restrict__ mu_copy, double *__restrict__ moment_part) {
 	__shared__ double sh[kSlotGroups][kTile][3];
 	__shared__ double shk[kSlotGroups][kTile][3];
-	const int a = threadIdx.x & 63, g = threadIdx.x >> 6;
+	const int a = threadIdx.x & 63, w = threadIdx.x >> 6;
 	const int i = blockIdx.x * kTile + a;
 	double real[3];
 	double e[3] = {0, 0, 0};
-	if (polar_ewald) slot_sum_64(e_recip_part, n_kslices, at.n_pad, i, a, g, shk, e);
-	slot_sum_64(part, n_split, at.n_pad, i, a, g, sh, real);
-	if (g != 0) return;
+	const double al = (w == 0) ? at.alpha[i] : 0.0;
+	if (polar_ewald) slot_sum_64_four_waves(e_recip_part, n_kslices, at.n_pad, i, a, w, shk, e);
+	slot_sum_64_four_waves(part, n_split, at.n_pad, i, a, w, sh, real);
+	if (w != 0) return;
 	if (e_real_out)
 		for (int p = 0; p < 3; ++p) e_real_out[3 * (size_t)i + p] = real[p];
 	if (polar_ewald) {
@@ -409,12 +453,17 @@
 		for (int p = 0; p < 3; ++p) e[p] *= sc;
 	}
 	for (int p = 0; p < 3; ++p) e[p] += real[p];
-	const double al = at.alpha[i];
+	double d0[3];
 	for (int p = 0; p < 3; ++p) {
 		e_static[3 * (size_t)i + p] = e[p];
 		const double m0 = (al * e[p]) * gamma;
 		mu[3 * (size_t)i + p] = m0;
 		if (mu_copy) mu_copy[3 * (size_t)i + p] = m0;
+		d0[p] = m0;
+	}
+	if (moment_part) {
+		const double m = moment_lane_sum(moment_term(i < at.n && al != 0.0, e, d0));
+		if (a == 0) moment_part[(size_t)blockIdx.x * kMomentsMax] = m;
 	}
 }
 
@@ -466,7 +515,7 @@
 	}
 }
 
-__global__ __launch_bounds__(64) void k_post_results(double *__restrict__ scal, double *__restrict__ out_host, double seq) {
+__device__ __forceinline__ void post_results_wave(double *scal, double *out_host, double seq) {
 	static_assert(S_COUNT + C_COUNT <= 64, "one wave posts the scalar block");
 	const int t = threadIdx.x;
 	if (t < S_COUNT + C_COUNT) {
@@ -477,6 +526,9 @@
 	__threadfence_system();
 	if (t == 0) __hip_atomic_store(out_host + S_COUNT + C_COUNT, seq, __ATOMIC_RELEASE, __HIP_MEMORY_SCOPE_SYSTEM);
 }
+__global__ __launch_bounds__(64) void k_post_results(double *__restrict__ scal, double *__restrict__ out_host, double seq) {
+	post_results_wave(scal, out_host, seq);
+}
 void launch_post_results(hipStream_t st, double *scal, double *out_host, double seq) {
 	hipLaunchKernelGGL(k_post_results, dim3(1), dim3(64), 0, st, scal, out_host, seq);
 }
@@ -491,9 +543,9 @@
 }
 
 void launch_field_finalize(hipStream_t st, const AtomsDev &at, const Box &bx, int polar_ewald, const double *e_recip_part, const double *part,
-                           int n_split, double gamma, double *e_static, double *mu, double *e_real_out, double *mu_copy) {
-	hipLaunchKernelGGL(k_field_finalize, dim3(at.n_pad / kTile), dim3(kTile * kSlotGroups), 0, st, at, bx, polar_ewald, e_recip_part, part, n_split,
-	                   gamma, e_static, mu, e_real_out, recip_ksplit(at.n_pad), mu_copy);
+                           int n_split, double gamma, double *e_static, double *mu, double *e_real_out, double *mu_copy, double *moment_part) {
+	hipLaunchKernelGGL(k_field_finalize, dim3(at.n_pad / kTile), dim3(kTile * kSlotWaves), 0, st, at, bx, polar_ewald, e_recip_part, part, n_split,
+	                   gamma, e_static, mu, e_real_out, recip_ksplit(at.n_pad), mu_copy, moment_part);
 }
 
 __device__ __forceinline__ void iteration_verdict(int *__restrict__ ctl, int *__restrict__ host_flag, int it, bool lane_broke) {
@@ -518,7 +570,7 @@
                                                     int n_split, const double *__restrict__ mu_old, double *__restrict__ mu_new,
                                                     double *__restrict__ e_induced, int want_rrms, double *__restrict__ rrms_atom,
                                                     double allowed_sqerr, int *__restrict__ ctl, int *__restrict__ host_flag, int it,
-                                                    double *__restrict__ dk) {
+                                                    double *__restrict__ dk, const MomentOut mo) {
 	__shared__ double sh[kSlotGroups][kTile][3];
 	if (ctl && ctl[1] != 0) return;
 	const int a = threadIdx.x & 63, g = threadIdx.x >> 6;
@@ -535,8 +587,14 @@
 			nm[p] = al * (e_static[3 * (size_t)i + p] + f[p]);
 		}
 	}
+	double dp[3] = {0, 0, 0}, es[3] = {0, 0, 0};
+	if (mo.part) {
+		for (int p = 0; p < 3; ++p) es[p] = e_static[3 * (size_t)i + p];
+		if (mo.k > 1)
+			for (int p = 0; p < 3; ++p) dp[p] = mo.d_prev[3 * (size_t)i + p];
+	}
 	bool broke = false;
-	double acc = 0, nn = 0;
+	double acc = 0, nn = 0, dn[3];
 	for (int p = 0; p < 3; ++p) {
 		const double d = nm[p] - mu_old[3 * (size_t)i + p];
 		acc += d * d;
@@ -545,7 +603,9 @@
 		mu_new[3 * (size_t)i + p] = nm[p];
 		e_induced[3 * (size_t)i + p] = f[p];
 		if (dk) dk[3 * (size_t)i + p] = d;
-	}
+		dn[p] = d;
+	}
+	if (mo.part) moment_pair_store(mo, live, al, es, dp, dn, a, blockIdx.x);
 	if (want_rrms) {
 		double r = sqrt(acc / nn);
 		if (!isfinite(r)) r = 0.0;
@@ -557,8 +617,8 @@
                                                        int n_split, const double *__restrict__ mu_old, double *__restrict__ mu_new,
                                                        double *__restrict__ e_induced, int want_rrms, double *__restrict__ rrms_atom,
                                                        double allowed_sqerr, int *__restrict__ ctl, int *__restrict__ host_flag, int it,
-                                                       double *__restrict__ dk) {
-	dipole_update_block(at, e_static, part, n_split, mu_old, mu_new, e_induced, want_rrms, rrms_atom, allowed_sqerr, ctl, host_flag, it, dk);
+                                                       double *__restrict__ dk, const MomentOut mo) {
+	dipole_update_block(at, e_static, part, n_split, mu_old, mu_new, e_induced, want_rrms, rrms_atom, allowed_sqerr, ctl, host_flag, it, dk, mo);
 }
 
 __global__ __launch_bounds__(256) void k_dipole_reset(AtomsDev at, const double *__restrict__ e_static, double *__restrict__ mu) {
@@ -593,83 +653,27 @@
 	polar_energy_block(at, mu, e_static, rrms_atom, scal);
 }
 
-constexpr int kMomentsMax = 2 * (kMomentsMaxHalf + 1);
-constexpr int kMomentsOnePassHalf = 5;
-template <int H>
-__device__ __forceinline__ void polar_moments_one_pass(const AtomsDev &at, const double *__restrict__ dk, const double *__restrict__ e_static,
-                                                       double *__restrict__ sh, double *__restrict__ s_m) {
-	const size_t stride = 3 * (size_t)at.n_pad;
-	double acc[2 * H + 1] = {};
-#pragma unroll 2
-	for (int i = threadIdx.x; i < at.n; i += 256) {
-		const size_t b = 3 * (size_t)i;
-		const double al = at.alpha[i];
-		double d[H + 1][3], w[3];
+__device__ __forceinline__ void fold_moments_block(const double *__restrict__ moment_part, int n_tiles, int n_iter, double *__restrict__ scal) {
+	__shared__ double s_w[4][kMomentsMax];
+	__shared__ double s_m[kMomentsMax];
+	const int lane = threadIdx.x & 63, w = threadIdx.x >> 6;
+	constexpr int kChunk = 11;
+	for (int k0 = 0; k0 <= n_iter; k0 += kChunk) {
+		double v[kChunk] = {};
+		for (int t = threadIdx.x; t < n_tiles; t += 256) {
+			const double *__restrict__ q = moment_part + (size_t)t * kMomentsMax + k0;
 #pragma unroll
-		for (int a = 0; a <= H; ++a) {
-			const double *__restrict__ q = dk + (size_t)a * stride + b;
-			d[a][0] = q[0], d[a][1] = q[1], d[a][2] = q[2];
-		}
-		w[0] = e_static[b], w[1] = e_static[b + 1], w[2] = e_static[b + 2];
-		const double inv = (al != 0.0) ? 1.0 / al : 0.0;
+			for (int j = 0; j < kChunk; ++j) v[j] += (k0 + j <= n_iter) ? q[j] : 0.0;
+		}
 #pragma unroll
-		for (int a = 0; a <= H; ++a) {
-			if (a > 0) w[0] = d[a][0] * inv, w[1] = d[a][1] * inv, w[2] = d[a][2] * inv;
-			acc[2 * a] += ((w[0] * d[a][0]) + w[1] * d[a][1]) + w[2] * d[a][2];
-			if (a < H) acc[2 * a + 1] += ((w[0] * d[a + 1][0]) + w[1] * d[a + 1][1]) + w[2] * d[a + 1][2];
-		}
-	}
-#pragma unroll
-	for (int k = 0; k <= 2 * H; ++k) {
-		const double v = block_sum_256(acc[k], sh);
-		if (threadIdx.x == 0) s_m[k] = v;
-	}
-}
-__device__ __forceinline__ void polar_moments_block(const AtomsDev &at, const double *__restrict__ dk, const double *__restrict__ e_static, int n_iter,
-                                                    double *__restrict__ scal) {
-	__shared__ double sh[4];
-	__shared__ double s_m[kMomentsMax];
-	const size_t stride = 3 * (size_t)at.n_pad;
-	const int half = (n_iter + 1) / 2;
-	switch (half <= kMomentsOnePassHalf ? half : 0) {
-	case 1: polar_moments_one_pass<1>(at, dk, e_static, sh, s_m); break;
-	case 2: polar_moments_one_pass<2>(at, dk, e_static, sh, s_m); break;
-	case 3: polar_moments_one_pass<3>(at, dk, e_static, sh, s_m); break;
-	case 4: polar_moments_one_pass<4>(at, dk, e_static, sh, s_m); break;
-	case 5: polar_moments_one_pass<5>(at, dk, e_static, sh, s_m); break;
-	default: break;
-	}
-	for (int a = 0; a <= (half <= kMomentsOnePassHalf ? -1 : half); ++a) {
-		const double *__restrict__ da = dk + (size_t)a * stride;
-		const bool odd = 2 * a + 1 <= n_iter;
-		const double *__restrict__ db = odd ? da + stride : da;
-		double m0 = 0, m1 = 0;
-		if (a == 0) {
-#pragma unroll 4
-			for (int i = threadIdx.x; i < at.n; i += 256) {
-				const size_t b = 3 * (size_t)i;
-				const double w0 = e_static[b], w1 = e_static[b + 1], w2 = e_static[b + 2];
-				m0 += ((w0 * da[b]) + w1 * da[b + 1]) + w2 * da[b + 2];
-				m1 += ((w0 * db[b]) + w1 * db[b + 1]) + w2 * db[b + 2];
-			}
-		} else {
-#pragma unroll 4
-			for (int i = threadIdx.x; i < at.n; i += 256) {
-				const size_t b = 3 * (size_t)i;
-				const double al = at.alpha[i];
-				const double inv = (al != 0.0) ? 1.0 / al : 0.0;
-				const double w0 = da[b] * inv, w1 = da[b + 1] * inv, w2 = da[b + 2] * inv;
-				m0 += ((w0 * da[b]) + w1 * da[b + 1]) + w2 * da[b + 2];
-				m1 += ((w0 * db[b]) + w1 * db[b + 1]) + w2 * db[b + 2];
-			}
-		}
-		m0 = block_sum_256(m0, sh);
-		m1 = block_sum_256(m1, sh);
-		if (threadIdx.x == 0) {
-			s_m[2 * a] = m0;
-			s_m[2 * a + 1] = odd ? m1 : 0.0;
-		}
-	}
+		for (int j = 0; j < kChunk; ++j) {
+			const double r = wave_sum(v[j]);
+			if (lane == 0) s_w[w][k0 + j] = r;
+		}
+	}
+	__syncthreads();
+	if (threadIdx.x <= n_iter) s_m[threadIdx.x] = ((s_w[0][threadIdx.x] + s_w[1][threadIdx.x]) + s_w[2][threadIdx.x]) + s_w[3][threadIdx.x];
+	__syncthreads();
 	if (threadIdx.x == 0) {
 		double u = 0;
 		for (int k = 0; k <= n_iter; ++k) u += s_m[k];
@@ -677,22 +681,18 @@
 		scal[S_RRMS] = 0.0;
 	}
 }
-__global__ __launch_bounds__(256) void k_polar_moments(AtomsDev at, const double *__restrict__ dk, const double *__restrict__ e_static, int n_iter,
-                                                       double *__restrict__ scal) {
-	polar_moments_block(at, dk, e_static, n_iter, scal);
-}
-__global__ __launch_bounds__(256) void k_polar_moments_and_pairs(AtomsDev at, const double *__restrict__ dk, const double *__restrict__ e_static, int n_iter,
-                                                                 const double *__restrict__ block_part, const int *__restrict__ block_cnt, int nb,
-                                                                 double *__restrict__ scal, long long *__restrict__ cnt) {
-	if (blockIdx.x == 0) polar_moments_block(at, dk, e_static, n_iter, scal);
-	else reduce_pairs_block(block_part, block_cnt, nb, scal, cnt);
-}
-void launch_polar_moments(hipStream_t st, const AtomsDev &at, const double *dk, const double *e_static, int n_iter, double *scal) {
-	hipLaunchKernelGGL(k_polar_moments, dim3(1), dim3(256), 0, st, at, dk, e_static, n_iter, scal);
-}
-void launch_polar_moments_and_pairs(hipStream_t st, const AtomsDev &at, const double *dk, const double *e_static, int n_iter, const double *block_part,
-                                    const int *block_cnt, int nb, double *scal, long long *cnt) {
-	hipLaunchKernelGGL(k_polar_moments_and_pairs, dim3(2), dim3(256), 0, st, at, dk, e_static, n_iter, block_part, block_cnt, nb, scal, cnt);
+static_assert(kMomentsMax % 11 == 0 && kMomentsMaxIter < kMomentsMax && kMomentsMax <= 256, "fold_moments_block: chunks inside a tile's row, one thread per moment");
+__global__ __launch_bounds__(256) void k_moments_tail(const double *__restrict__ moment_part, int n_tiles, int n_iter, const double *__restrict__ block_part,
+                                                      const int *__restrict__ block_cnt, int nb, double *scal, double *out_host, double seq) {
+	fold_moments_block(moment_part, n_tiles, n_iter, scal);
+	if (block_part) reduce_pairs_block(block_part, block_cnt, nb, scal, reinterpret_cast<long long *>(scal + S_COUNT));
+	if (!out_host) return;
+	__syncthreads();
+	if (threadIdx.x < 64) post_results_wave(scal, out_host, seq);
+}
+void launch_moments_tail(hipStream_t st, const double *moment_part, int n_tiles, int n_iter, const double *block_part, const int *block_cnt, int nb,
+                         double *scal, double *out_host, double seq) {
+	hipLaunchKernelGGL(k_moments_tail, dim3(1), dim3(256), 0, st, moment_part, n_tiles, n_iter, block_part, block_cnt, nb, scal, out_host, seq);
 }
 
 __global__ __launch_bounds__(256) void k_polar_energy_and_pairs(AtomsDev at, const double *__restrict__ mu, const double *__restrict__ e_static,
@@ -705,9 +705,9 @@
 
 void launch_dipole_update(hipStream_t st, const AtomsDev &at, const double *e_static, const double *part, int n_split, const double *mu_old,
                           double *mu_new, double *e_induced, int want_rrms, double *rrms_atom, double allowed_sqerr, int *ctl, int *host_flag, int it,
-                          double *dk) {
+                          double *dk, const MomentOut &mo) {
 	hipLaunchKernelGGL(k_dipole_update, dim3(at.n_pad / kTile), dim3(kTile * kSlotGroups), 0, st, at, e_static, part, n_split, mu_old, mu_new,
-	                   e_induced, want_rrms, rrms_atom, allowed_sqerr, ctl, host_flag, it, dk);
+	                   e_induced, want_rrms, rrms_atom, allowed_sqerr, ctl, host_flag, it, dk, mo);
 }
 void launch_dipole_reset(hipStream_t st, const AtomsDev &at, const double *e_static, double *mu) {
 	hipLaunchKernelGGL(k_dipole_reset, dim3((at.n_pad + 255) / 256), dim3(256), 0, st, at, e_static, mu);
diff --git a/mpmcxx_amd/csrc/kernels_panel.hip b/mpmcxx_amd/csrc/kernels_panel.hip
--- a/mpmcxx_amd/csrc/kernels_panel.hip
+++ b/mpmcxx_amd/csrc/kernels_panel.hip
@@ -368,6 +368,7 @@
 	double allowed_sqerr;
 	int *ctl, *host_flag;
 	int nt, it, want_rrms;
+	MomentOut mo;
 };
 
 __device__ __forceinline__ void panel_update_tile(const AtomsDev &at, const PanelUpdate &u, const double *__restrict__ part, const double *__restrict__ gpart,
@@ -376,13 +377,15 @@
 	const int a = threadIdx.x & 63, w = __builtin_amdgcn_readfirstlane(threadIdx.x >> 6);
 	const int i = X * kTile + a;
 	const int nF = u.nt - X, wg0 = u.seg[X], nG = u.seg[X + 1] - wg0;
-	double al = 0.0, es[3] = {0, 0, 0}, mo[3] = {0, 0, 0};
+	double al = 0.0, es[3] = {0, 0, 0}, mo[3] = {0, 0, 0}, dp[3] = {0, 0, 0};
 	if (w == 0) {
 		al = at.alpha[i];
 		for (int p = 0; p < 3; ++p) {
 			es[p] = u.e_static[3 * (size_t)i + p];
 			mo[p] = mu_old[3 * (size_t)i + p];
 		}
+		if (u.mo.part && u.mo.k > 1)
+			for (int p = 0; p < 3; ++p) dp[p] = u.mo.d_prev[3 * (size_t)i + p];
 	}
 	double f[GW][3] = {};
 	const size_t n_pad = (size_t)at.n_pad;
@@ -436,7 +439,7 @@
 		}
 	}
 	bool broke = false;
-	double acc = 0, nn = 0;
+	double acc = 0, nn = 0, dn[3];
 	for (int p = 0; p < 3; ++p) {
 		const double d = nm[p] - mo[p];
 		acc += d * d;
@@ -445,7 +448,9 @@
 		u.mu_new[3 * (size_t)i + p] = nm[p];
 		if (u.e_induced) u.e_induced[3 * (size_t)i + p] = fo[p];
 		if (u.dk) u.dk[3 * (size_t)i + p] = d;
-	}
+		dn[p] = d;
+	}
+	if (u.mo.part) moment_pair_store(u.mo, live, al, es, dp, dn, a, X);
 	if (u.want_rrms) {
 		double r = sqrt(acc / nn);
 		if (!isfinite(r)) r = 0.0;
@@ -536,9 +541,10 @@
 
 void launch_dipole_update_panel(hipStream_t st, const AtomsDev &at, const double *e_static, const double *part, const double *gpart, const int *seg,
                                 const double *mu_old, double *mu_new, double *e_induced, int want_rrms, double *rrms_atom, double allowed_sqerr,
-                                int *ctl, int *host_flag, int it, double *dk) {
+                                int *ctl, int *host_flag, int it, double *dk, const MomentOut &mo) {
 	PanelUpdate u{};
 	u.dk = dk;
+	u.mo = mo;
 	u.e_static = e_static, u.seg = seg, u.mu_new = mu_new, u.e_induced = e_induced, u.rrms_atom = rrms_atom, u.allowed_sqerr = allowed_sqerr;
 	u.ctl = ctl, u.host_flag = host_flag, u.nt = at.n_pad / kTile, u.it = it, u.want_rrms = want_rrms;
 	hipLaunchKernelGGL(k_dipole_update_panel, dim3(at.n_pad / kTile), dim3(kTile * kUpdWaves), 0, st, at, part, gpart, mu_old, u);
diff --git a/mpmcxx_amd/csrc/trial.cpp b/mpmcxx_amd/csrc/trial.cpp
--- a/mpmcxx_amd/csrc/trial.cpp
+++ b/mpmcxx_amd/csrc/trial.cpp
@@ -145,7 +145,7 @@
 			c->mu_cur = 0;
 			if (polar_moments_apply(c) && (rc = reserve_dk_ring(c)) != MPMC_OK) return rc;
 			launch_field_finalize(st, at, c->box, o.polar_ewald, c->d_e_recip_part, c->d_e_real_trial, 1, o.polar_gamma, c->d_e_static, c->d_mu[0], nullptr,
-			                      polar_moments_apply(c) ? c->d_dk_ring.p : nullptr);
+			                      polar_moments_apply(c) ? c->d_dk_ring.p : nullptr, polar_moments_apply(c) ? c->d_moment_part.p : nullptr);
 		}
 		HIP_TRY(c, hipGetLastError());
 		c->trial_polar_delta = true;
```

After: 1957, median of 2. About the same (+0.2%).
